# HuiyangYu/TGSFilter

Hardware: AMD Instinct MI355X
Metric: filtered Gbases/sec (end-to-end, excl. gzip I/O) (higher is better)
Workload: dtype u8

## Files before the change

include/tgsf.h:

```cpp
#ifndef TGSF_H
#define TGSF_H

#include <stddef.h>
#include <stdint.h>

#ifdef __cplusplus
extern "C" {
#endif

#define TGSF_ABI_VERSION 3
#define TGSF_MAX_ADAPTERS 32
#define TGSF_MAX_ADAPTER_LEN 8192
#define TGSF_N_DROPINFO 17
#define TGSF_N_QBINS 256
#define TGSF_BIN_WIDTH 100

typedef enum tgsf_status {
    TGSF_OK = 0,
    TGSF_E_INVALID = -1,
    TGSF_E_NO_DEVICE = -2,
    TGSF_E_HIP = -3,
    TGSF_E_CAPACITY = -4,
    TGSF_E_UNSUPPORTED = -5,
    TGSF_E_DATA = -6
} tgsf_status;

typedef struct tgsf_params {
    uint32_t struct_size;
    int32_t  min_len;
    int32_t  max_len;
    float    min_q;
    float    max_q;
    int32_t  bc_len;
    int32_t  head_trim;
    int32_t  tail_trim;
    int32_t  end_len;
    int32_t  end_match_len;
    int32_t  mid_match_len;
    int32_t  extra_len;
    float    end_sim;
    float    mid_sim;
    int32_t  discard;
    int32_t  filter;
    int32_t  only_qc;
    int32_t  min_repeat;
    int32_t  kmer;
    int32_t  qtype;
    int32_t  n_adapters;
    const char* adapters[TGSF_MAX_ADAPTERS];
    int32_t  adapter_len[TGSF_MAX_ADAPTERS];
    uint64_t max_batch_bases;
    uint32_t max_batch_reads;
    uint32_t max_read_len;
    int32_t  no_qual;
    int32_t  reserved;
} tgsf_params;

typedef struct tgsf_batch_in {
    const uint8_t*  seq;
    const uint8_t*  qual;
    const uint64_t* offsets;
    const uint32_t* lengths;
    uint32_t        n_reads;
    uint32_t        reserved;
    uint64_t        n_bytes;
    const uint64_t* qual_offsets;
} tgsf_batch_in;

#define TGSF_RF_LOWQ       0x01u
#define TGSF_RF_AD5P       0x02u
#define TGSF_RF_AD3P       0x04u
#define TGSF_RF_ADMID      0x08u
#define TGSF_RF_DISCARDED  0x10u

typedef struct tgsf_read_result {
    uint64_t sum_q;
    uint32_t flags;
    uint32_t n_frags;
    uint32_t frag_begin;
    uint32_t trimmed;
    int32_t  reserved0;
    int32_t  reserved1;
} tgsf_read_result;

#define TGSF_FF_PASS    0x01u
#define TGSF_FF_REPEAT  0x02u

typedef struct tgsf_fragment {
    uint64_t sum_q;
    uint32_t read;
    int32_t  start;
    int32_t  len;
    uint32_t flags;
} tgsf_fragment;

typedef struct tgsf_batch_out {
    tgsf_read_result* reads;
    tgsf_fragment*    frags;
    uint32_t          frag_capacity;
    uint32_t          n_frags;
} tgsf_batch_out;

#define TGSF_CTR_DROPINFO    0
#define TGSF_CTR_RAW_DIFFQ   17
#define TGSF_CTR_CLEAN_DIFFQ 273
#define TGSF_CTR_ROWS        529
#define TGSF_CTR_END_TABLES  533

enum { TGSF_T_RAW5P_QUAL = 0, TGSF_T_RAW5P_CNT, TGSF_T_RAW3P_QUAL, TGSF_T_RAW3P_CNT,
       TGSF_T_CLEAN5P_QUAL, TGSF_T_CLEAN5P_CNT, TGSF_T_CLEAN3P_QUAL, TGSF_T_CLEAN3P_CNT };
enum { TGSF_B_RAW_QUAL = 0, TGSF_B_RAW_CNT, TGSF_B_CLEAN_QUAL, TGSF_B_CLEAN_CNT };

static inline size_t tgsf_ctr_end_table(int t, int bc_len) {
    return (size_t)TGSF_CTR_END_TABLES + (size_t)t * (size_t)bc_len * 5u;
}
static inline size_t tgsf_ctr_bin_table(int b, int bc_len, uint32_t n_bins) {
    return (size_t)TGSF_CTR_END_TABLES + 8u * (size_t)bc_len * 5u + (size_t)b * (size_t)n_bins * 5u;
}
static inline size_t tgsf_ctr_len(int bc_len, uint32_t n_bins) {
    return tgsf_ctr_bin_table(4, bc_len, n_bins);
}
static inline uint32_t tgsf_n_bins(uint32_t max_read_len) { return max_read_len / TGSF_BIN_WIDTH + 1u; }

typedef struct tgsf_ctx tgsf_ctx;

int tgsf_abi_version(void);

const char* tgsf_backend(void);

int tgsf_prepare_device(int device);

int tgsf_device_location(int device, char* bus_id, int len, int* numa_node);

int tgsf_create(const tgsf_params* params, int device, tgsf_ctx** out_ctx);
void tgsf_destroy(tgsf_ctx* ctx);

int tgsf_submit(tgsf_ctx* ctx, const tgsf_batch_in* in, tgsf_batch_out* out);
int tgsf_submit_async(tgsf_ctx* ctx, const tgsf_batch_in* in, tgsf_batch_out* out);

#define TGSF_MAX_ENQUEUED 64
#define TGSF_NFRAGS_NOT_FINAL 0xFFFFFFFFu
int tgsf_submit_device(tgsf_ctx* ctx, const tgsf_batch_in* in, tgsf_batch_out* out,
                       uint32_t* d_n_frags, void* hip_stream);

int tgsf_wait(tgsf_ctx* ctx);

int tgsf_counters_len(tgsf_ctx* ctx, uint64_t* n_words, int32_t* bc_len, uint32_t* n_bins);
int tgsf_counters(tgsf_ctx* ctx, uint64_t* dst, uint64_t n_words);
int tgsf_counters_used(tgsf_ctx* ctx, uint64_t* dst, uint64_t n_words, uint64_t rows[2]);
int tgsf_counters_merge(tgsf_ctx* dst, tgsf_ctx* src);
int tgsf_counters_device(tgsf_ctx* ctx, void** d_ptr, uint64_t* n_words);
int tgsf_reset_counters(tgsf_ctx* ctx);

#define TGSF_N_STAGES 12
int tgsf_profile(tgsf_ctx* ctx, int enable);
int tgsf_stage_times(tgsf_ctx* ctx, float ms[TGSF_N_STAGES], uint32_t* n_batches);
const char* tgsf_stage_name(int stage);

int tgsf_align_windows(tgsf_ctx* ctx, const uint8_t* seq, uint64_t n_bytes,
                       const uint64_t* win_off, const uint32_t* win_len,
                       const uint8_t* adapter_id, const int32_t* k, uint32_t n,
                       int32_t* res, int32_t* ends);

const char* tgsf_last_error(tgsf_ctx* ctx);

#ifdef __cplusplus
}
#endif
#endif
```

tgsfilter_amd/abi.py:

```python
from __future__ import annotations

import ctypes as C

import numpy as np

ABI_VERSION = 3
MAX_ADAPTERS = 32
MAX_ADAPTER_LEN = 8192
N_DROPINFO = 17
N_QBINS = 256
BIN_WIDTH = 100
N_STAGES = 12

OK, E_INVALID, E_NO_DEVICE, E_HIP, E_CAPACITY, E_UNSUPPORTED, E_DATA = 0, -1, -2, -3, -4, -5, -6

RF_LOWQ, RF_AD5P, RF_AD3P, RF_ADMID, RF_DISCARDED = 0x01, 0x02, 0x04, 0x08, 0x10
FF_PASS, FF_REPEAT = 0x01, 0x02
MAX_ENQUEUED = 64
NFRAGS_NOT_FINAL = 0xFFFFFFFF

CTR_DROPINFO, CTR_RAW_DIFFQ, CTR_CLEAN_DIFFQ, CTR_ROWS, CTR_END_TABLES = 0, 17, 273, 529, 533
(T_RAW5P_QUAL, T_RAW5P_CNT, T_RAW3P_QUAL, T_RAW3P_CNT,
 T_CLEAN5P_QUAL, T_CLEAN5P_CNT, T_CLEAN3P_QUAL, T_CLEAN3P_CNT) = range(8)
B_RAW_QUAL, B_RAW_CNT, B_CLEAN_QUAL, B_CLEAN_CNT = range(4)


class Params(C.Structure):
    _fields_ = [
        ("struct_size", C.c_uint32),
        ("min_len", C.c_int32), ("max_len", C.c_int32),
        ("min_q", C.c_float), ("max_q", C.c_float),
        ("bc_len", C.c_int32), ("head_trim", C.c_int32), ("tail_trim", C.c_int32),
        ("end_len", C.c_int32), ("end_match_len", C.c_int32), ("mid_match_len", C.c_int32),
        ("extra_len", C.c_int32),
        ("end_sim", C.c_float), ("mid_sim", C.c_float),
        ("discard", C.c_int32), ("filter", C.c_int32), ("only_qc", C.c_int32),
        ("min_repeat", C.c_int32), ("kmer", C.c_int32), ("qtype", C.c_int32),
        ("n_adapters", C.c_int32),
        ("adapters", C.c_char_p * MAX_ADAPTERS),
        ("adapter_len", C.c_int32 * MAX_ADAPTERS),
        ("max_batch_bases", C.c_uint64),
        ("max_batch_reads", C.c_uint32),
        ("max_read_len", C.c_uint32),
        ("no_qual", C.c_int32), ("reserved", C.c_int32),
    ]


class BatchIn(C.Structure):
    _fields_ = [
        ("seq", C.c_void_p), ("qual", C.c_void_p), ("offsets", C.c_void_p), ("lengths", C.c_void_p),
        ("n_reads", C.c_uint32), ("reserved", C.c_uint32), ("n_bytes", C.c_uint64),
        ("qual_offsets", C.c_void_p),
    ]


class BatchOut(C.Structure):
    _fields_ = [
        ("reads", C.c_void_p), ("frags", C.c_void_p),
        ("frag_capacity", C.c_uint32), ("n_frags", C.c_uint32),
    ]


READ_RESULT_DTYPE = np.dtype([
    ("sum_q", "<u8"), ("flags", "<u4"), ("n_frags", "<u4"), ("frag_begin", "<u4"),
    ("trimmed", "<u4"), ("reserved0", "<i4"), ("reserved1", "<i4"),
])
FRAGMENT_DTYPE = np.dtype([
    ("sum_q", "<u8"), ("read", "<u4"), ("start", "<i4"), ("len", "<i4"), ("flags", "<u4"),
])
assert READ_RESULT_DTYPE.itemsize == 32 and FRAGMENT_DTYPE.itemsize == 24


def ctr_end_table(t: int, bc_len: int) -> int:
    return CTR_END_TABLES + t * bc_len * 5


def ctr_bin_table(b: int, bc_len: int, n_bins: int) -> int:
    return CTR_END_TABLES + 8 * bc_len * 5 + b * n_bins * 5


def ctr_len(bc_len: int, n_bins: int) -> int:
    return ctr_bin_table(4, bc_len, n_bins)


def n_bins(max_read_len: int) -> int:
    return max_read_len // BIN_WIDTH + 1


_MID_SIM = {"hifi": 0.95, "clr": 0.9, "ont": 0.9}
# ... 35 lines not shown
```

tgsfilter_amd/capi.py:

```python
from __future__ import annotations

import ctypes as C
import os

import numpy as np

from . import abi

_HERE = os.path.dirname(os.path.abspath(__file__))
DEFAULT_LIB = os.path.join(_HERE, "libtgsf.so")
_LIBS = {}

SYMBOLS = [
    "tgsf_abi_version", "tgsf_backend", "tgsf_prepare_device", "tgsf_device_location", "tgsf_create", "tgsf_destroy", "tgsf_submit", "tgsf_submit_async", "tgsf_submit_device",
    "tgsf_wait",
    "tgsf_counters_len", "tgsf_counters", "tgsf_counters_used", "tgsf_counters_merge", "tgsf_counters_device", "tgsf_reset_counters", "tgsf_profile",
    "tgsf_stage_times", "tgsf_stage_name", "tgsf_align_windows", "tgsf_last_error",
]


class TgsfError(RuntimeError):
    def __init__(self, code, msg):
        super().__init__(f"tgsf error {code}: {msg}")
        self.code = code


def load(path: str | None = None):
    explicit = path is not None
    path = path or os.environ.get("TGSF_LIB") or DEFAULT_LIB
    if path in _LIBS:
        if not explicit and not _LIBS[path].tgsf_backend().startswith(b"hip"):
            raise RuntimeError(f"{path} is not the HIP build of libtgsf (there is no CPU fallback; is TGSF_LIB set by accident?)")
        return _LIBS[path]
    if not os.path.exists(path):
        raise FileNotFoundError(
            f"{path} not found: build the HIP extension first (python -c 'import __graft_entry__ as g; g.build()')")
    L = C.CDLL(path)
    vp, u32, u64, i32 = C.c_void_p, C.c_uint32, C.c_uint64, C.c_int32
    L.tgsf_abi_version.restype = C.c_int
    L.tgsf_backend.restype = C.c_char_p
    L.tgsf_prepare_device.argtypes = [C.c_int]
    L.tgsf_device_location.argtypes = [C.c_int, C.c_char_p, C.c_int, C.POINTER(C.c_int)]
    L.tgsf_create.argtypes = [C.POINTER(abi.Params), C.c_int, C.POINTER(vp)]
    L.tgsf_destroy.argtypes = [vp]
    L.tgsf_destroy.restype = None
    L.tgsf_submit.argtypes = [vp, C.POINTER(abi.BatchIn), C.POINTER(abi.BatchOut)]
    L.tgsf_submit_async.argtypes = [vp, C.POINTER(abi.BatchIn), C.POINTER(abi.BatchOut)]
    L.tgsf_submit_device.argtypes = [vp, C.POINTER(abi.BatchIn), C.POINTER(abi.BatchOut), vp, vp]
    L.tgsf_wait.argtypes = [vp]
    L.tgsf_counters_len.argtypes = [vp, C.POINTER(u64), C.POINTER(i32), C.POINTER(u32)]
    L.tgsf_counters.argtypes = [vp, vp, u64]
    L.tgsf_counters_used.argtypes = [vp, vp, u64, vp]
    L.tgsf_counters_merge.argtypes = [vp, vp]
    L.tgsf_counters_device.argtypes = [vp, C.POINTER(vp), C.POINTER(u64)]
    L.tgsf_reset_counters.argtypes = [vp]
    L.tgsf_profile.argtypes = [vp, C.c_int]
    L.tgsf_stage_times.argtypes = [vp, C.POINTER(C.c_float * abi.N_STAGES), C.POINTER(u32)]
    L.tgsf_stage_name.argtypes = [C.c_int]
    L.tgsf_stage_name.restype = C.c_char_p
    L.tgsf_align_windows.argtypes = [vp, vp, u64, vp, vp, vp, vp, u32, vp, vp]
    L.tgsf_last_error.argtypes = [vp]
    L.tgsf_last_error.restype = C.c_char_p
    if L.tgsf_abi_version() != abi.ABI_VERSION:
        raise RuntimeError("libtgsf ABI version mismatch")
    if not explicit and not L.tgsf_backend().startswith(b"hip"):
        raise RuntimeError(f"{path} is the {L.tgsf_backend().decode()!r} build of libtgsf, not the HIP build "
                           "(there is no CPU fallback; is TGSF_LIB set by accident?)")
    _LIBS[path] = L
    return L


class Context:

    def __init__(self, params: abi.Params, device: int = 0, lib_path: str | None = None):
        self.lib = load(lib_path)
        self.params = params
        h = C.c_void_p()
        rc = self.lib.tgsf_create(C.byref(params), device, C.byref(h))
        if rc != 0:
            raise TgsfError(rc, self.lib.tgsf_last_error(None).decode())
        self.h = h
        nw, bc, nb = C.c_uint64(), C.c_int32(), C.c_uint32()
        self._chk(self.lib.tgsf_counters_len(self.h, C.byref(nw), C.byref(bc), C.byref(nb)))
        self.ctr_words, self.bc_len, self.n_bins = nw.value, bc.value, nb.value

    def _chk(self, rc):
        if rc != 0:
            raise TgsfError(rc, self.lib.tgsf_last_error(self.h).decode())

    def close(self):
        if getattr(self, "h", None):
            self.lib.tgsf_destroy(self.h)
            self.h = None

    def __del__(self):
        try:
            self.close()
        except Exception:
            pass

    def submit(self, seq, qual, offsets, lengths=None, frag_capacity=None, qual_offsets=None):
        self.submit_async(seq, qual, offsets, lengths, frag_capacity, qual_offsets)
        return self.wait_result()

    def submit_async(self, seq, qual, offsets, lengths=None, frag_capacity=None, qual_offsets=None):
        seq = np.ascontiguousarray(seq, dtype=np.uint8)
        qual = np.ascontiguousarray(qual, dtype=np.uint8)
        offsets = np.ascontiguousarray(offsets, dtype=np.uint64)
        if lengths is not None:
            lengths = np.ascontiguousarray(lengths, dtype=np.uint32)
            n = len(lengths)
            total = int(lengths.sum())
        else:
            n = len(offsets) - 1
            total = int(offsets[-1] - offsets[0])
        if frag_capacity is None:
            frag_capacity = total // 100 + n + 16
        reads = np.zeros(n, dtype=abi.READ_RESULT_DTYPE)
        frags = np.zeros(frag_capacity, dtype=abi.FRAGMENT_DTYPE)
        if qual_offsets is not None:
            qual_offsets = np.ascontiguousarray(qual_offsets, dtype=np.uint64)
        same = qual is seq or (qual.ctypes.data == seq.ctypes.data)
        bi = abi.BatchIn(seq.ctypes.data, seq.ctypes.data if same else qual.ctypes.data, offsets.ctypes.data,
                         lengths.ctypes.data if lengths is not None else None, n, 0, seq.size,
                         qual_offsets.ctypes.data if qual_offsets is not None else None)
        bo = abi.BatchOut(reads.ctypes.data, frags.ctypes.data, frag_capacity, 0)
        self._pending = (reads, frags, bi, bo, seq, qual, offsets, lengths, qual_offsets)
        rc = self.lib.tgsf_submit_async(self.h, C.byref(bi), C.byref(bo))
        if rc != 0:
            self._pending = None
            self._chk(rc)

    def wait_result(self):
        pend, self._pending = self._pending, None
        if pend is None:
            raise RuntimeError("no batch pending")
        self._chk(self.lib.tgsf_wait(self.h))
        reads, frags, _, bo = pend[:4]
        return reads, frags[:bo.n_frags].copy()

    def submit_device(self, d_seq, d_qual, d_offsets, d_lengths, n_reads, n_bytes, d_reads, d_frags,
                      frag_capacity, d_nfrags=None, stream=None, d_qual_offsets=None):
        bi = abi.BatchIn(d_seq, d_qual, d_offsets, d_lengths, n_reads, 0, n_bytes, d_qual_offsets)
        bo = abi.BatchOut(d_reads, d_frags, frag_capacity, 0)
        self._chk(self.lib.tgsf_submit_device(self.h, C.byref(bi), C.byref(bo), d_nfrags, stream))

    def wait(self):
        self._chk(self.lib.tgsf_wait(self.h))

    def counters(self) -> np.ndarray:
        out = np.zeros(self.ctr_words, dtype=np.uint64)
        self._chk(self.lib.tgsf_counters(self.h, out.ctypes.data, self.ctr_words))
# ... 43 lines not shown
```

tgsfilter_amd/csrc/tgsf_lib.hip:

```cpp
#include <stdarg.h>
#include <stdio.h>
#include <stdlib.h>
#include <string.h>

#include <algorithm>
#include <string>
#include <vector>

#if defined(TGSF_EMUL)
#include "tgsf_kernels.h"
namespace tgsf_emul { thread_local Dim3 threadIdx, blockIdx, blockDim, gridDim; }
typedef void* rt_stream;
typedef int rt_error;
#else
#include <hip/hip_runtime.h>
#include "tgsf_kernels.h"
typedef hipStream_t rt_stream;
#endif

using namespace tgsf;

static thread_local std::string g_create_error;

static const char* knob(const char* name)
{
    static const bool on = [] { const char* e = getenv("TGSF_DEBUG_KNOBS"); return e && e[0] == '1'; }();
    return on ? getenv(name) : nullptr;
}

struct tgsf_ctx {
    tgsf_params params;
    std::vector<std::string> adapters;
    DevParams P;
    DevBatch B;
    int device;
    rt_stream stream;
    rt_stream last_stream;
    bool own_stream;
    std::string error;
    uint64_t cap_bases;
    uint32_t cap_reads, max_read_len, n_bins;
    static constexpr unsigned endtab_grid = 512;
    static constexpr unsigned stats_grid = 768;
    bool flat_scan = true;
    int suffix_filter = 2;
    bool no_hot32 = false;
    uint64_t ctr_words;
    int scratch_cols;
    uint8_t *d_seq, *d_qual;
    uint64_t* d_off;
    uint64_t* d_qoff;
    uint32_t* d_lenin;
    tgsf_read_result* d_out_reads;
    tgsf_fragment* d_out_frags;
    uint32_t* d_out_nfrags;
    std::vector<void*> allocs;
    bool profile;
    float stage_ms[TGSF_N_STAGES];
    uint32_t prof_batches;
#if !defined(TGSF_EMUL)
    static constexpr int kProfRing = 64;
    hipEvent_t ev[kProfRing][TGSF_N_STAGES + 1];
    hipEvent_t ev_aux[kProfRing][3];
    int prof_pending;
    hipStream_t aux;
    hipEvent_t ev_fork, ev_join;
    uint32_t* h_pinned = nullptr;
    static constexpr size_t kStageBytes = 32u << 20;
    uint8_t* stage[2] = {nullptr, nullptr};
    hipEvent_t stage_ev[2] = {nullptr, nullptr};
#endif
    uint32_t h_words_[8];
    uint32_t* h_status;
    uint32_t* pend_nf_p;
    tgsf_batch_out* pend_out = nullptr;
    struct Pending { tgsf_batch_in in; tgsf_read_result* reads; tgsf_fragment* frags; uint32_t fcap; uint32_t* nfrags; rt_stream st; };
    Pending pending[TGSF_MAX_ENQUEUED];
    uint32_t n_pending = 0;
    uint32_t* ovf_ring = nullptr;
    uint32_t* bp_ring = nullptr;
    uint32_t h_ovf[TGSF_MAX_ENQUEUED];
    uint32_t pool_regrown = 0;

};

static int fail(tgsf_ctx* c, int code, const char* fmt, ...)
{
    char buf[512];
    va_list ap;
    va_start(ap, fmt);
    vsnprintf(buf, sizeof buf, fmt, ap);
    va_end(ap);
    if (c) c->error = buf; else g_create_error = buf;
    return code;
}

#if defined(TGSF_EMUL)
#include "tgsf_emul_rt.h"
#else
static int rt_malloc(void** p, size_t n) { return (int)hipMalloc(p, n ? n : 1); }
static void rt_free(void* p) { (void)hipFree(p); }
static int rt_memset(void* p, int v, size_t n, rt_stream s) { return (int)hipMemsetAsync(p, v, n, s); }
static int rt_h2d(void* d, const void* s, size_t n, rt_stream st) { return (int)hipMemcpyAsync(d, s, n, hipMemcpyHostToDevice, st); }
static int rt_d2h(void* d, const void* s, size_t n, rt_stream st) { return (int)hipMemcpyAsync(d, s, n, hipMemcpyDeviceToHost, st); }
static int rt_sync(rt_stream s) { return (int)hipStreamSynchronize(s); }
static const char* rt_errstr(int e) { return hipGetErrorString((hipError_t)e); }
#define TGSF_LAUNCH(kernel, grid, block, stream, ...) hipLaunchKernelGGL(kernel, dim3(grid), dim3(block), 0, (stream), __VA_ARGS__)
#define TGSF_LAUNCH_COOP TGSF_LAUNCH
#define TGSF_LAUNCH_LDS(kernel, grid, block, lds, stream, ...) hipLaunchKernelGGL(kernel, dim3(grid), dim3(block), (lds), (stream), __VA_ARGS__)
static unsigned grid_cap(unsigned g) { return g; }
#endif

template <class T>
static int dev_alloc(tgsf_ctx* c, T** p, size_t count)
{
    void* v = nullptr;
    int e = rt_malloc(&v, count * sizeof(T) + 64);
    if (e) return fail(c, TGSF_E_HIP, "device allocation of %zu bytes failed: %s", count * sizeof(T), rt_errstr(e));
    c->allocs.push_back(v);
    *p = (T*)v;
    return 0;
}

static int build_tables(tgsf_ctx* c)
{
    const tgsf_params& p = c->params;
    DevParams& P = c->P;
    const int A = p.n_adapters;
    std::vector<uint8_t> ad((size_t)kMaxAdapters * kMaxQ, 0);
    const size_t per_ad = (size_t)256 * kPeqW;
    std::vector<uint64_t> fwd((size_t)kMaxAdapters * per_ad, 0), rev((size_t)kMaxAdapters * per_ad, 0),
        top((size_t)kMaxAdapters * 256, 0);
    P.max_nw = 1;
    P.min_Q = 1 << 30;
    for (int a = 0; a < A; a++) {
        const std::string& s = c->adapters[a];
        const int Q = (int)s.size();
        P.Q[a] = Q;
        if (Q > 64 && P.max_nw < 2) P.max_nw = 2;
        if (Q > 128 && P.max_nw < 4) P.max_nw = 4;
        if (Q > 256) P.max_nw = kWideNW;
        if (Q < P.min_Q) P.min_Q = Q;
        int km = Q - p.mid_match_len + 1;
        int ke = Q - p.end_match_len + 1;
        P.k_mid[a] = km > Q - 1 ? Q - 1 : km;
        P.k_end[a] = ke > Q - 1 ? Q - 1 : ke;
        P.w5[a] = p.end_len + (int)((float)Q / p.end_sim);
        P.need_end[a] = P.need_mid[a] = Q + 1;
        for (int m = Q; m >= 0; m--) {
            if (m >= p.end_match_len && (float)m / (float)Q >= p.end_sim) P.need_end[a] = m;
            if (m >= p.mid_match_len && (float)m / (float)Q >= p.mid_sim) P.need_mid[a] = m;
        }
        memcpy(&ad[(size_t)a * kMaxQ], s.data(), (size_t)Q);
        for (int r = 0; r < Q && r < 64 * kPeqW; r++) {
            uint8_t cf = (uint8_t)s[r], cr = (uint8_t)s[Q - 1 - r];
            fwd[(size_t)a * per_ad + (size_t)cf * kPeqW + (r >> 6)] |= 1ull << (r & 63);
            rev[(size_t)a * per_ad + (size_t)cr * kPeqW + (r >> 6)] |= 1ull << (r & 63);
        }
        if (Q <= 64) {
            const int sh = 64 - Q;
            const uint64_t pad = sh ? ((1ull << sh) - 1ull) : 0ull;
            for (int sym = 0; sym < 256; sym++)
                top[(size_t)a * 256 + sym] = (fwd[(size_t)a * per_ad + (size_t)sym * kPeqW] << sh) | pad;
        }
    }
    if (A == 0) P.min_Q = 1 << 30;
    uint8_t* d_ad; uint64_t *d_f, *d_r, *d_t;
    int e;
    if ((e = dev_alloc(c, &d_ad, ad.size()))) return e;
    if ((e = dev_alloc(c, &d_f, fwd.size()))) return e;
    if ((e = dev_alloc(c, &d_r, rev.size()))) return e;
    if ((e = dev_alloc(c, &d_t, top.size()))) return e;
    rt_h2d(d_ad, ad.data(), ad.size(), c->stream);
    rt_h2d(d_f, fwd.data(), fwd.size() * 8, c->stream);
    rt_h2d(d_r, rev.data(), rev.size() * 8, c->stream);
    rt_h2d(d_t, top.data(), top.size() * 8, c->stream);
    rt_sync(c->stream);
    P.adapter = d_ad; P.peq_fwd = d_f; P.peq_rev = d_r; P.peq_top = d_t;
    P.peq_fwd_w = P.peq_rev_w = nullptr;
    if (P.max_nw > 4) {
        const size_t per_w = (size_t)256 * kWideNW;
        std::vector<uint64_t> fw((size_t)A * per_w, 0), rw((size_t)A * per_w, 0);
        for (int a = 0; a < A; a++) {
            const std::string& s = c->adapters[a];
            const int Q = (int)s.size();
            for (int r = 0; r < Q; r++) {
                const uint8_t cf = (uint8_t)s[r], cr = (uint8_t)s[Q - 1 - r];
                fw[(size_t)a * per_w + (size_t)cf * kWideNW + (r >> 6)] |= 1ull << (r & 63);
                rw[(size_t)a * per_w + (size_t)cr * kWideNW + (r >> 6)] |= 1ull << (r & 63);
            }
        }
        uint64_t *d_fw, *d_rw;
        if ((e = dev_alloc(c, &d_fw, fw.size()))) return e;
        if ((e = dev_alloc(c, &d_rw, rw.size()))) return e;
        rt_h2d(d_fw, fw.data(), fw.size() * 8, c->stream);
        rt_h2d(d_rw, rw.data(), rw.size() * 8, c->stream);
        rt_sync(c->stream);
        P.peq_fwd_w = d_fw; P.peq_rev_w = d_rw;
    }
    return 0;
}

extern "C" int tgsf_abi_version(void) { return TGSF_ABI_VERSION; }
extern "C" const char* tgsf_backend(void) { return kTgsfEmul ? "emulation" : "hip:gfx950"; }

#if !defined(TGSF_EMUL)
__global__ void k_noop(int* p) { if (p) *p = 0; }
#endif
#if !defined(TGSF_EMUL)
static void set_wait_mode(int device)
{
    const char* e = getenv("TGSF_SYNC");
    if (!e || strcmp(e, "blocking") != 0) return;
    if (hipSetDevice(device) == hipSuccess) { (void)hipSetDeviceFlags(hipDeviceScheduleBlockingSync); (void)hipGetLastError(); }
}
#endif
extern "C" int tgsf_prepare_device(int device)
{
#if !defined(TGSF_EMUL)
    int ndev = 0;
    if (hipGetDeviceCount(&ndev) != hipSuccess || device < 0 || device >= ndev) return TGSF_E_NO_DEVICE;
    set_wait_mode(device);
    if (hipSetDevice(device) != hipSuccess) return TGSF_E_HIP;
    hipLaunchKernelGGL(k_noop, dim3(1), dim3(64), 0, 0, (int*)nullptr);
    if (hipDeviceSynchronize() != hipSuccess) return TGSF_E_HIP;
    {
        static const char a0[] = "GTTTTCGCATTTATCGTGAAACGCTTTCGCGTTTTTCGTGCGCCGCTTCA";
        static const char a1[] = "TGAAGCGGCGCACGAAAAACGCGAAAGCGTTTCACGATAAATGCGAAAAC";
        tgsf_params p;
        memset(&p, 0, sizeof p);
        p.struct_size = sizeof p;
        p.min_len = 100; p.max_len = 2147483647; p.min_q = 0; p.max_q = 255; p.bc_len = 150;
        p.end_len = 150; p.end_match_len = 4; p.mid_match_len = 35; p.extra_len = 50;
        p.end_sim = 0.75f; p.mid_sim = 0.9f; p.filter = 1; p.qtype = 33; p.kmer = 11;
        p.n_adapters = 2; p.adapters[0] = a0; p.adapters[1] = a1; p.adapter_len[0] = p.adapter_len[1] = 50;
        p.max_batch_bases = 1 << 16; p.max_batch_reads = 16; p.max_read_len = 1 << 14;
        tgsf_ctx* c = nullptr;
        if (tgsf_create(&p, device, &c) == TGSF_OK) {
            std::vector<uint8_t> seq(8192), qual(8192, (uint8_t)'5');
            for (size_t i = 0; i < seq.size(); i++) seq[i] = "ACGT"[(i * 2654435761u >> 13) & 3];
            memcpy(&seq[4096 + 1000], a0, 50);
            const uint64_t off[2] = {0, 4096};
            const uint32_t len[2] = {3000, 4000};
            tgsf_read_result res[2];
            tgsf_fragment fr[64];
            tgsf_batch_in in;
            memset(&in, 0, sizeof in);
            in.seq = seq.data(); in.qual = qual.data(); in.offsets = off; in.lengths = len; in.n_reads = 2; in.n_bytes = seq.size();
            tgsf_batch_out out{res, fr, 64, 0};
            (void)tgsf_submit(c, &in, &out);
            tgsf_destroy(c);
        }
    }
#else
    (void)device;
#endif
    return TGSF_OK;
}

extern "C" int tgsf_device_location(int device, char* bus_id, int len, int* numa_node)
{
    if (numa_node) *numa_node = -1;
    if (bus_id && len > 0) bus_id[0] = 0;
#if !defined(TGSF_EMUL)
    int ndev = 0;
    if (hipGetDeviceCount(&ndev) != hipSuccess || device < 0 || device >= ndev) return TGSF_E_NO_DEVICE;
    char id[64] = {0};
    if (hipDeviceGetPCIBusId(id, (int)sizeof id, device) != hipSuccess) return TGSF_E_HIP;
    for (char* p = id; *p; p++) if (*p >= 'A' && *p <= 'F') *p = (char)(*p - 'A' + 'a');
    if (bus_id && len > 0) { strncpy(bus_id, id, (size_t)len - 1); bus_id[len - 1] = 0; }
    if (numa_node) {
        const std::string path = std::string("/sys/bus/pci/devices/") + id + "/numa_node";
        if (FILE* f = fopen(path.c_str(), "r")) {
            int v = -1;
            if (fscanf(f, "%d", &v) == 1) *numa_node = v;
            fclose(f);
        }
    }
    return TGSF_OK;
#else
    if (bus_id && len > 0) snprintf(bus_id, (size_t)len, "emul:%d", device);
    if (numa_node)
        if (const char* e = knob("TGSF_EMUL_NUMA")) {
            int k = 0;
            for (const char* c = e; *c; k++) {
                if (k == device) { *numa_node = atoi(c); break; }
                while (*c && *c != ',') c++;
                if (*c == ',') c++;
            }
        }
    return TGSF_OK;
#endif
}

extern "C" const char* tgsf_last_error(tgsf_ctx* ctx) { return ctx ? ctx->error.c_str() : g_create_error.c_str(); }

extern "C" void tgsf_destroy(tgsf_ctx* c)
{
    if (!c) return;
    if (c->B.bp_allowed && c->B.bp_state && knob("TGSF_TRACE_BP")) {
        uint32_t w[4] = {0, 0, 0, 0};
        uint64_t pl[4] = {0, 0, 0, 0};
        uint32_t sg[4] = {0, 0, 0, 0};
        if (!rt_d2h(w, c->B.bp_state, sizeof w, c->stream) && !rt_d2h(pl, c->B.plan, sizeof pl, c->stream) && !rt_d2h(sg, c->B.seg_info, sizeof sg, c->stream) && !rt_sync(c->stream))
            fprintf(stderr, "tgsf: clean tables as a by-product of the raw pass: %u batches speculated; the next would%s; the last batch: %llu bases a direct clean pass scans, "
                            "%llu bases its own did, %u work items in that pass\n", w[1], w[0] ? "" : " not", (unsigned long long)pl[2], (unsigned long long)pl[3], sg[2]);
    }
#if !defined(TGSF_EMUL)
    (void)hipSetDevice(c->device);
    (void)hipStreamSynchronize(c->stream);
    for (int k = 0; k < tgsf_ctx::kProfRing; k++) {
        for (int i = 0; i <= TGSF_N_STAGES; i++) if (c->ev[k][i]) (void)hipEventDestroy(c->ev[k][i]);
        for (int i = 0; i < 3; i++) if (c->ev_aux[k][i]) (void)hipEventDestroy(c->ev_aux[k][i]);
    }
    if (c->h_pinned) (void)hipHostFree(c->h_pinned);
    for (int i = 0; i < 2; i++) {
        if (c->stage[i]) (void)hipHostFree(c->stage[i]);
        if (c->stage_ev[i]) (void)hipEventDestroy(c->stage_ev[i]);
    }
    if (c->ev_fork) (void)hipEventDestroy(c->ev_fork);
    if (c->ev_join) (void)hipEventDestroy(c->ev_join);
    if (c->aux) (void)hipStreamDestroy(c->aux);
    if (c->own_stream && c->stream) (void)hipStreamDestroy(c->stream);
#endif
    for (void* p : c->allocs) rt_free(p);
    delete c;
}

extern "C" int tgsf_create(const tgsf_params* p, int device, tgsf_ctx** out)
{
    if (!p || !out) return fail(nullptr, TGSF_E_INVALID, "null argument");
    *out = nullptr;
    if (p->struct_size != sizeof(tgsf_params))
        return fail(nullptr, TGSF_E_INVALID, "tgsf_params.struct_size %u != %zu (ABI mismatch)", p->struct_size, sizeof(tgsf_params));
    if (p->n_adapters < 0 || p->n_adapters > TGSF_MAX_ADAPTERS)
        return fail(nullptr, TGSF_E_INVALID, "n_adapters %d outside [0,%d]", p->n_adapters, TGSF_MAX_ADAPTERS);
    if (p->min_repeat > 0 && (p->kmer < 1 || p->kmer > 32))
        return fail(nullptr, TGSF_E_UNSUPPORTED, "-k %d: the repeat gate supports k-mer sizes 1..32 (the reference's k-mers are 64 bits)", p->kmer);
    if (p->qtype != 33 && p->qtype != 64) return fail(nullptr, TGSF_E_INVALID, "qtype must be 33 or 64");
    if (p->bc_len < 0 || p->bc_len > kMaxBcLenTotal) return fail(nullptr, TGSF_E_INVALID, "bc_len (-e) outside [0,%d]", kMaxBcLenTotal);
    if (p->filter && p->n_adapters > 0) {
        if (!(p->end_sim > 0.f) || !(p->mid_sim > 0.f)) return fail(nullptr, TGSF_E_INVALID, "similarities must be > 0");
        if (p->end_len < 0 || p->extra_len < 0) return fail(nullptr, TGSF_E_INVALID, "end_len / extra_len must be >= 0");
        if (p->end_match_len < 1 || p->mid_match_len < 1)
            return fail(nullptr, TGSF_E_INVALID, "match lengths must be >= 1");
    }
    for (int a = 0; a < p->n_adapters; a++) {
        if (!p->adapters[a] || p->adapter_len[a] < 1 || p->adapter_len[a] > TGSF_MAX_ADAPTER_LEN)
            return fail(nullptr, TGSF_E_UNSUPPORTED, "adapter %d: length %d outside [1,%d]", a, p->adapter_len[a], TGSF_MAX_ADAPTER_LEN);
    }
    if (!p->max_batch_bases || !p->max_batch_reads || !p->max_read_len)
        return fail(nullptr, TGSF_E_INVALID, "max_batch_bases / max_batch_reads / max_read_len must be set");
    if (p->max_read_len > (1u << 28)) return fail(nullptr, TGSF_E_INVALID, "max_read_len above 2^28");

    tgsf_ctx* c = new tgsf_ctx();
    c->params = *p;
    c->device = device;
    c->profile = false;
    c->prof_batches = 0;
    memset(c->stage_ms, 0, sizeof c->stage_ms);
    memset(c->h_words_, 0, sizeof c->h_words_);
    c->h_status = c->h_words_;
    c->pend_nf_p = c->h_words_ + 4;
    for (int a = 0; a < p->n_adapters; a++) {
        c->adapters.emplace_back(p->adapters[a], (size_t)p->adapter_len[a]);
        c->params.adapters[a] = c->adapters.back().data();
    }
    for (int a = 0; a < p->n_adapters; a++) c->params.adapters[a] = c->adapters[a].data();
#if !defined(TGSF_EMUL)
    memset(c->ev, 0, sizeof c->ev);
    memset(c->ev_aux, 0, sizeof c->ev_aux);
    c->aux = nullptr; c->ev_fork = c->ev_join = nullptr;
    int ndev = 0;
    hipError_t he = hipGetDeviceCount(&ndev);
    if (he != hipSuccess || ndev <= 0) {
        delete c;
        return fail(nullptr, TGSF_E_NO_DEVICE, "no HIP device available (%s); libtgsf has no CPU fallback", hipGetErrorString(he));
    }
    if (device < 0 || device >= ndev) { delete c; return fail(nullptr, TGSF_E_NO_DEVICE, "device %d out of range (%d devices)", device, ndev); }
    set_wait_mode(device);
    if ((he = hipSetDevice(device)) != hipSuccess) { delete c; return fail(nullptr, TGSF_E_HIP, "hipSetDevice: %s", hipGetErrorString(he)); }
    if ((he = hipStreamCreateWithFlags(&c->stream, hipStreamNonBlocking)) != hipSuccess) {
        delete c; return fail(nullptr, TGSF_E_HIP, "hipStreamCreate: %s", hipGetErrorString(he));
    }
    c->own_stream = true;
    c->prof_pending = 0;
    {
        uint32_t* pw = nullptr;
        if (hipHostMalloc((void**)&pw, 64, hipHostMallocDefault) == hipSuccess && pw) {
            memset(pw, 0, 64);
            c->h_pinned = pw; c->h_status = pw; c->pend_nf_p = pw + 4;
        }
    }
    {
        int lo = 0, hi = 0;
        (void)hipDeviceGetStreamPriorityRange(&lo, &hi);
        he = hipStreamCreateWithPriority(&c->aux, hipStreamNonBlocking, hi);
    }
    if (he != hipSuccess ||
        (he = hipEventCreateWithFlags(&c->ev_fork, hipEventDisableTiming)) != hipSuccess ||
        (he = hipEventCreateWithFlags(&c->ev_join, hipEventDisableTiming)) != hipSuccess) {
        tgsf_destroy(c); return fail(nullptr, TGSF_E_HIP, "auxiliary stream: %s", hipGetErrorString(he));
    }
#else
    c->stream = nullptr; c->own_stream = false;
#endif
    c->last_stream = c->stream;
#if !defined(TGSF_EMUL)
    if (p->max_batch_bases > (8u << 20)) {
        for (int i = 0; i < 2; i++)
            if (hipHostMalloc((void**)&c->stage[i], tgsf_ctx::kStageBytes, hipHostMallocDefault) != hipSuccess ||
                hipEventCreateWithFlags(&c->stage_ev[i], hipEventDisableTiming) != hipSuccess) {
                tgsf_destroy(c); return fail(nullptr, TGSF_E_HIP, "pinned staging buffers: allocation failed");
            }
    }
#endif
    DevParams& P = c->P;
    memset(&P, 0, sizeof P);
    P.min_len = p->min_len; P.max_len = p->max_len; P.min_q = p->min_q; P.max_q = p->max_q;
    P.bc_len = p->bc_len; P.head_trim = p->head_trim; P.tail_trim = p->tail_trim; P.end_len = p->end_len;
    P.end_match_len = p->end_match_len; P.mid_match_len = p->mid_match_len; P.extra_len = p->extra_len;
    P.end_sim = p->end_sim; P.mid_sim = p->mid_sim; P.discard = p->discard; P.filter = p->filter;
    P.only_qc = p->only_qc; P.qtype = p->qtype; P.n_adapters = p->n_adapters;
    P.no_qual = p->no_qual ? 1 : 0;
    P.min_repeat = p->min_repeat; P.kmer = p->kmer;
    c->cap_bases = p->max_batch_bases;
    c->cap_reads = p->max_batch_reads;
    c->max_read_len = p->max_read_len;
    c->n_bins = tgsf_n_bins(p->max_read_len);
    P.n_bins = c->n_bins;
    c->ctr_words = tgsf_ctr_len(p->bc_len, c->n_bins);
    P.seg_cols = kSegCols;
    if (const char* e = knob("TGSF_NO_HOT32")) c->no_hot32 = atoi(e) > 0;
    if (const char* e = knob("TGSF_SEG_COLS")) { int v = atoi(e); if (v >= 256 && v <= 65536) P.seg_cols = v & ~15; }
    if (const char* e = knob("TGSF_MID_FLAT")) c->flat_scan = atoi(e) > 0;
    if (const char* e = knob("TGSF_MID_FILTER")) { int v = atoi(e); if (v >= 0 && v <= 2) c->suffix_filter = v; }

    int e = build_tables(c);
    DevBatch& B = c->B;
    memset(&B, 0, sizeof B);
    B.flat_pmax = 256; B.flat_pmin = 16; B.flat_f0 = 224;
    if (const char* e = knob("TGSF_FLAT_PMIN")) { int v = atoi(e); if (v >= 1 && v <= (1 << 20)) B.flat_pmin = (uint32_t)v; }
    if (const char* e = knob("TGSF_FLAT_PMAX")) { int v = atoi(e); if (v >= 1 && v <= (1 << 20)) B.flat_pmax = (uint32_t)v; }
    if (const char* e = knob("TGSF_FLAT_F0")) { int v = atoi(e); if (v >= 0 && v <= 256) B.flat_f0 = (uint32_t)v; }
    B.flat_pmin = 1u << flat_log2(B.flat_pmin); B.flat_pmax = 1u << flat_log2(B.flat_pmax);
    if (B.flat_pmax < B.flat_pmin) B.flat_pmax = B.flat_pmin;
    const size_t n = c->cap_reads;
    const int A = p->n_adapters > 0 ? p->n_adapters : 1;
    const uint64_t cap_bytes = c->cap_bases + 16ull * n + 64;
    const int min_len = p->min_len > 0 ? p->min_len : 1;
    uint64_t fcap64 = p->filter ? (c->cap_bases / (uint64_t)min_len + 16) : (uint64_t)n + 16;
    if (fcap64 > c->cap_bases + 16) fcap64 = c->cap_bases + 16;
    if (fcap64 < n + 16 && !p->filter) fcap64 = n + 16;
    B.fcap = (uint32_t)std::min<uint64_t>(fcap64, 0x7FFFFFF0ull);
    B.max_tiles = (c->max_read_len + kTileBases - 1) / kTileBases;
    uint64_t pool = c->cap_bases / 64 + 65536 + (uint64_t)n * 16u * (uint64_t)std::max(p->n_adapters, 1);
    B.pool_cap = (uint32_t)std::min<uint64_t>(pool, 1ull << 28);
    if (const char* e = knob("TGSF_POOL_CAP")) { const long long v = atoll(e); if (v >= 1 && v < (1ll << 28)) B.pool_cap = (uint32_t)v; }
    const size_t nitems = n + (size_t)B.fcap;
    if (!e) e = dev_alloc(c, &c->d_seq, cap_bytes);
    if (!e) e = dev_alloc(c, &c->d_qual, cap_bytes);
    if (!e) e = dev_alloc(c, &c->d_off, n + 1);
    if (!e) e = dev_alloc(c, &c->d_qoff, n + 1);
    if (!e) e = dev_alloc(c, &c->d_lenin, n);
    if (!e) e = dev_alloc(c, &B.len, n);
    if (!e) e = dev_alloc(c, &B.sumq, n);
    if (!e) e = dev_alloc(c, &B.flags, n);
    if (!e) e = dev_alloc(c, &B.clip5, n * A);
    if (!e) e = dev_alloc(c, &B.clip3, n * A);
    if (!e) e = dev_alloc(c, &B.mid_head, n);
    if (!e) e = dev_alloc(c, &B.mid_best, n * A);
    if (!e) e = dev_alloc(c, &B.mid_cnt, n);
    if (!e) e = dev_alloc(c, &B.mid_gate, n * A);
    if (!e) e = dev_alloc(c, &B.pool, (size_t)B.pool_cap);
    if (!e) e = dev_alloc(c, &B.pool_n, 4);
    if (!e) e = dev_alloc(c, &B.seg_cnt, n + 1);
    if (!e) e = dev_alloc(c, &B.chk_cnt, n + 1);
    if (c->cap_bases / 16u + n >= 0xFFFFFFF0ull) c->flat_scan = false;
    if (c->cap_bases / 16u + n >= (1ull << 30) || !c->flat_scan) c->suffix_filter = 0;
    {
        bool any = false;
        for (int a = 0; a < p->n_adapters; a++) any |= c->P.Q[a] > 32 && c->P.Q[a] <= 64 && c->P.k_mid[a] >= 0 && c->P.k_mid[a] <= kSuffixMaxK;
        if (!any || !p->filter) c->suffix_filter = 0;
    }
    if (!e && c->suffix_filter) e = dev_alloc(c, &B.chk_mark, (size_t)4 * (size_t)((c->cap_bases / 16u + n) / 32u + 8u));
    if (c->suffix_filter) {
        B.rc_cap = (uint32_t)std::min<uint64_t>((c->cap_bases / 16u + n) / 25u + 4096u, 1ull << 24);
        if (const char* e2 = knob("TGSF_RECHECK_CAP")) { int v = atoi(e2); if (v >= 0) B.rc_cap = (uint32_t)v; }
        if (!e) e = dev_alloc(c, &B.rc_list, (size_t)B.rc_cap + 1);
        if (!e) e = dev_alloc(c, &B.rc_n, 4);
    }
    if (!e) e = dev_alloc(c, &B.nfr, n + 1);
    if (!e) e = dev_alloc(c, &B.scan_part, n / kScanTile + 2);
    if (!e) e = dev_alloc(c, &B.trimmed, n);
    B.rep_long_cap = (uint32_t)std::min<uint64_t>(c->cap_bases / kRepShare + 16, (uint64_t)B.fcap + 16);
    if (!e) e = dev_alloc(c, &B.rep_next, 2 + (size_t)B.rep_long_cap);
    if (p->min_repeat > 0 && p->kmer >= 12 && p->kmer <= 31) {
        B.rep_tab_log2 = 4;
        while (B.rep_tab_log2 < 40 && (1ull << B.rep_tab_log2) < 2ull * c->max_read_len) B.rep_tab_log2++;
        if (!e) e = dev_alloc(c, &B.rep_tab, (size_t)1 << B.rep_tab_log2);
        if (!e) e = dev_alloc(c, &B.rep_lock, 4);
        if (!e) rt_memset(B.rep_lock, 0, 16, c->stream);
        B.rep_max_plog = kRepMaxPlog;
        if (const char* ev = knob("TGSF_REP_MAX_PLOG")) { int v = atoi(ev); if (v >= 0 && v <= 20) B.rep_max_plog = (uint32_t)v; }
    }
    if (!e) e = dev_alloc(c, &B.tile_hist, 2 * ((size_t)B.max_tiles + 2));
    if (!e) e = dev_alloc(c, &B.tile_cnt, 2 * ((size_t)B.max_tiles + 2));
    if (!e) e = dev_alloc(c, &B.tile_base, 2 * ((size_t)B.max_tiles + 2));
    if (!e) e = dev_alloc(c, &B.tile_fill, 2 * ((size_t)B.max_tiles + 2));
    if (!e) e = dev_alloc(c, &B.seg_info, 4);
    if (!e) e = dev_alloc(c, &B.perm, nitems);
    B.work_cap = (uint32_t)std::min<uint64_t>(2 * (c->cap_bases / kTileBases) + nitems + 16, 0x7FFFFFF0ull);
    if (!e) e = dev_alloc(c, &B.work, 2 * (size_t)B.work_cap);
    if (!e) e = dev_alloc(c, &B.frag_off, (size_t)B.fcap);
    if (!e) e = dev_alloc(c, &B.frag_qoff, (size_t)B.fcap);
    if (!e) e = dev_alloc(c, &B.frag_len, (size_t)B.fcap);
    if (!e) e = dev_alloc(c, &B.frag_sum, (size_t)B.fcap);
    if (!e) e = dev_alloc(c, &B.frag_read, (size_t)B.fcap);
    if (!e) e = dev_alloc(c, &B.frag_start, (size_t)B.fcap);
    if (!e) e = dev_alloc(c, &B.frag_flags, (size_t)B.fcap);
    if (!e) e = dev_alloc(c, &B.raw_tab, 2 * (size_t)c->n_bins * 5);
    if (!e) e = dev_alloc(c, &B.whole, n);
    if (!e) e = dev_alloc(c, &B.plan, 4);
    B.clean_force = p->only_qc ? 1u : 0u;
    B.bp_allowed = (p->filter && !p->only_qc && (p->head_trim > 0 || p->tail_trim > 0) &&
                    p->head_trim >= 0 && p->tail_trim >= 0) ? 1u : 0u;
    static_assert(kTileBases < (1 << 13), "staged bytes of a tile fit the work list's 13 bits");
    if (const char* f = knob("TGSF_CLEAN_TABLES")) {
        if (!strcmp(f, "direct")) { B.clean_force = 1; B.bp_allowed = 0; }
        else if (!strcmp(f, "difference") && !p->only_qc) { B.clean_force = 2; B.bp_allowed = 0; }
        else if (!strcmp(f, "byproduct") && B.bp_allowed) B.clean_force = 3;
    }
    if (B.bp_allowed) {
        if (!e) e = dev_alloc(c, &B.spec, n);
        if (!e) e = dev_alloc(c, &B.spec_sum, n);
        if (!e) e = dev_alloc(c, &B.bp_state, 4);
        if (!e) e = dev_alloc(c, &c->bp_ring, TGSF_MAX_ENQUEUED);
    }
    {
        int maxcols = 1;
        for (int a = 0; a < p->n_adapters; a++) {
            int kmax = std::max(std::max(P.k_end[a], P.k_mid[a]), 0);
            maxcols = std::max(maxcols, P.Q[a] + std::min(P.Q[a], kmax) + 1);
        }
        c->scratch_cols = maxcols;
        int col_words = P.max_nw;
        if (P.max_nw > 4) { col_words = 1; for (int a = 0; a < p->n_adapters; a++) col_words = std::max(col_words, (P.Q[a] + 63) / 64); }
        size_t lane_words = (size_t)(maxcols + 1) * 2 * (size_t)col_words;
        if (P.max_nw > 4) lane_words = std::min<size_t>(lane_words, (1u << 17) + 2 * (size_t)col_words) + 4 * (size_t)col_words + 64;
        B.scratch_wave_words = lane_words * 64;
        B.scratch_mid_wave0 = ((size_t)n * A * 2 + 63) / 64 + 1;
        const size_t waves = B.scratch_mid_wave0 + ((size_t)n * A + 63) / 64 + 1;
        if (!e) e = dev_alloc(c, &B.scratch, waves * B.scratch_wave_words);
    }
    if (!e) e = dev_alloc(c, &B.ctr, (size_t)c->ctr_words);
    if (!e) e = dev_alloc(c, &B.status, 4);
    if (!e) e = dev_alloc(c, &c->ovf_ring, TGSF_MAX_ENQUEUED);
    if (!e) e = dev_alloc(c, &c->d_out_reads, n);
    if (!e) e = dev_alloc(c, &c->d_out_frags, (size_t)B.fcap);
    if (!e) e = dev_alloc(c, &c->d_out_nfrags, 4);
    if (e) {
        g_create_error = c->error;
        tgsf_destroy(c);
        return e;
    }
    rt_memset(B.ctr, 0, c->ctr_words * 8, c->stream);
    rt_memset(B.status, 0, 16, c->stream);
    rt_memset(c->ovf_ring, 0, TGSF_MAX_ENQUEUED * 4, c->stream);
    B.ovf = c->ovf_ring;
    if (B.bp_allowed) {
        const uint32_t init[4] = {1u, 0u, 0u, 0u};
        rt_memset(c->bp_ring, 0, TGSF_MAX_ENQUEUED * 4, c->stream);
        (void)rt_h2d(B.bp_state, init, sizeof init, c->stream);
        B.bp_used = c->bp_ring;
    }
    rt_memset(B.raw_tab, 0, 2 * (size_t)c->n_bins * 5 * 8, c->stream);
    rt_sync(c->stream);
    *out = c;
    return TGSF_OK;
}

static const char* kStageNames[TGSF_N_STAGES] = {
    "prepare+sort", "stats_raw", "gate_reads", "end_tables_raw", "end_windows", "mid_scan",
    "mid_resolve", "regions", "repeat_gate", "stats_clean", "gate_frags+end_tables_clean", "finalize"};

extern "C" const char* tgsf_stage_name(int s) { return (s >= 0 && s < TGSF_N_STAGES) ? kStageNames[s] : ""; }

static unsigned blocks_for(uint64_t n, unsigned block) { return (unsigned)std::max<uint64_t>(1, (n + block - 1) / block); }

#if !defined(TGSF_EMUL)
static int harvest_profile(tgsf_ctx* c, rt_stream st)
{
    if (!c->prof_pending) return TGSF_OK;
    hipError_t he = hipStreamSynchronize(st);
    if (he != hipSuccess) return fail(c, TGSF_E_HIP, "stream synchronize failed: %s", hipGetErrorString(he));
    (void)hipStreamSynchronize(c->aux);
    for (int k = 0; k < c->prof_pending; k++)
        for (int i = 0; i < TGSF_N_STAGES; i++) {
            float ms = 0.f;
            hipError_t e = (i == 3 || i == 4) ? hipEventElapsedTime(&ms, c->ev_aux[k][i - 3], c->ev_aux[k][i - 2])
                                              : hipEventElapsedTime(&ms, c->ev[k][i], c->ev[k][i + 1]);
            if (e == hipSuccess) c->stage_ms[i] += ms;
        }
    c->prof_pending = 0;
    return TGSF_OK;
}
#endif

static void scan_u32(const DevBatch& B, uint32_t* a, uint32_t n, rt_stream st, uint32_t* part = nullptr)
{
    if (!part) part = B.scan_part;
    const unsigned nb = (n + kScanTile - 1) / kScanTile;
    TGSF_LAUNCH_COOP(k_scan_tiles, nb, 256, st, a, n, part);
    TGSF_LAUNCH_COOP(k_scan_top, 1, 64, st, part, (uint32_t)nb, a + n);
    TGSF_LAUNCH_COOP(k_scan_add, nb, 256, st, a, n, (const uint32_t*)part);
}

static int drain_pending(tgsf_ctx* c, bool implicit = false);

static int run_pipeline(tgsf_ctx* c, const tgsf_batch_in* in, tgsf_read_result* d_reads, tgsf_fragment* d_frags,
                        uint32_t out_fcap, uint32_t* d_nfrags, rt_stream st, bool redo = false, uint32_t slot = 0)
{
    if (!redo) {
        if (c->n_pending == TGSF_MAX_ENQUEUED) { int e = drain_pending(c, true); if (e) return e; }
        slot = c->n_pending++;
        tgsf_ctx::Pending& pd = c->pending[slot];
        pd.in = *in; pd.reads = d_reads; pd.frags = d_frags; pd.fcap = out_fcap; pd.nfrags = d_nfrags; pd.st = st;
    }
    const bool profile = c->profile && !redo;
    (void)profile;
    DevBatch B = c->B;
    B.ovf = c->ovf_ring + slot;
    B.bp_used = c->bp_ring + slot;
    B.replay = redo ? 1u : 0u;
    const DevParams& P = c->P;
    B.seq = in->seq; B.qual = in->qual; B.off = in->offsets; B.len_in = in->lengths;
    B.qoff = in->qual_offsets ? in->qual_offsets : in->offsets;
    B.n = in->n_reads; B.n_bytes = in->n_bytes;
    const uint32_t n = B.n;
    const int A = P.n_adapters;
    const unsigned T = 256;
    static_assert(kMidThreads == 256, "k_mid_flat / k_mid_scan1 are launched with T lanes a workgroup");
    c->last_stream = st;
    const unsigned gsmall = grid_cap(std::min(blocks_for(n, T), 2048u));
    const unsigned gstats = grid_cap(c->stats_grid);
    const size_t tl = 2 * ((size_t)B.max_tiles + 2) * 4;
    const unsigned gfold = grid_cap(std::min(blocks_for((uint64_t)P.n_bins * 5, T), 1024u));
    int stage = 0;
#if !defined(TGSF_EMUL)
    if (profile && c->prof_pending == tgsf_ctx::kProfRing) { int e = harvest_profile(c, st); if (e) return e; }
    hipEvent_t* evs = c->ev[profile ? c->prof_pending : 0];
    hipEvent_t* evx = c->ev_aux[profile ? c->prof_pending : 0];
    if (profile) {
        for (int i = 0; i <= TGSF_N_STAGES; i++) if (!evs[i]) (void)hipEventCreate(&evs[i]);
        for (int i = 0; i < 3; i++) if (!evx[i]) (void)hipEventCreate(&evx[i]);
    }
    hipStream_t ax = c->aux;
#define STAGE_MARK() do { if (profile) (void)hipEventRecord(evs[stage], st); stage++; } while (0)
#else
#define STAGE_MARK() do { stage++; } while (0)
#endif
// ... 60 lines not shown
                gflat = grid_cap(blocks_for((uint64_t)S.d0[S.nph] + 128ull * (B.flat_pmax / B.flat_pmin) + 512u, T));
            }
        }
        const uint64_t max_segs = in->n_bytes / (uint64_t)P.seg_cols + 2ull * n + 1;
        const unsigned gseg = blocks_for(max_segs, T);
        const unsigned gmid = gseg;
        rt_stream ms = st;
        (void)ms;
        auto launch_scans = [&](uint32_t mode) {
            DevBatch Bm = B;
            Bm.mid_mode = mode;
            int a = 0;
            while (a < A) {
                if (P.Q[a] > 256) { TGSF_LAUNCH(k_mid_scan_wide, gseg, T, ms, P, Bm, a); a++; continue; }
                if (P.Q[a] > 192) { TGSF_LAUNCH(k_mid_scanw<4>, gseg, T, ms, P, Bm, a); a++; continue; }
                if (P.Q[a] > 128) { TGSF_LAUNCH(k_mid_scanw<3>, gseg, T, ms, P, Bm, a); a++; continue; }
                if (P.Q[a] > 64) { TGSF_LAUNCH(k_mid_scanw<2>, gseg, T, ms, P, Bm, a); a++; continue; }
                auto cls = [&](int x) {
                    if (P.Q[x] <= 32 && !c->no_hot32) return 0;
                    if (flat && mode == 0 && c->suffix_filter && P.Q[x] > 32 && P.k_mid[x] >= 0 && P.k_mid[x] <= kSuffixMaxK) return 2;
                    return 1;
                };
                const int kind = cls(a);
                const bool narrow = kind == 0;
                const int width = narrow ? 2 : 4;
                int na = 0;
                while (a + na < A && na < width && P.Q[a + na] <= 64 && cls(a + na) == kind) na++;
                if (kind == 2) {
                    const unsigned lp = 0;
                    Bm.mark_stride = (uint32_t)((flat_chunks / 32u + 7u) & ~3ull);
                    rt_memset(Bm.chk_mark, 0, (size_t)na * Bm.mark_stride * 4u, ms);
                    rt_memset(Bm.rc_n, 0, 4, ms);
                    if (c->suffix_filter == 1) switch (na) {
                    case 1: TGSF_LAUNCH_LDS((k_mid_flat<1, Hot32, 1>), gflat, T, lp, ms, P, Bm, a, na); break;
                    case 2: TGSF_LAUNCH_LDS((k_mid_flat<2, Hot32, 1>), gflat, T, lp, ms, P, Bm, a, na); break;
                    case 3: TGSF_LAUNCH_LDS((k_mid_flat<3, Hot32, 1>), gflat, T, lp, ms, P, Bm, a, na); break;
                    default: TGSF_LAUNCH_LDS((k_mid_flat<4, Hot32, 1>), gflat, T, lp, ms, P, Bm, a, na); break;
                    }
                    else switch (na) {
                    case 1: TGSF_LAUNCH_LDS((k_mid_flat<1, Hot32, 2>), gflat, T, lp, ms, P, Bm, a, na); break;
                    case 2: TGSF_LAUNCH_LDS((k_mid_flat<2, Hot32, 2>), gflat, T, lp, ms, P, Bm, a, na); break;
                    case 3: TGSF_LAUNCH_LDS((k_mid_flat<3, Hot32, 2>), gflat, T, lp, ms, P, Bm, a, na); break;
                    default: TGSF_LAUNCH_LDS((k_mid_flat<4, Hot32, 2>), gflat, T, lp, ms, P, Bm, a, na); break;
                    }
                    const unsigned grc = grid_cap(blocks_for(flat_chunks / 32u + 1u, (unsigned)kRecheckWords));
                    TGSF_LAUNCH_COOP(k_mid_marks, grc, T, ms, P, Bm, a, na);
                    TGSF_LAUNCH(k_mid_recheck, grid_cap(2048u), T, ms, P, Bm, a, na);
                    a += na;
                    continue;
                }
                if (flat && mode == 0) {
                    const unsigned lp = 0;
                    if (narrow) switch (na) {
                    case 1: TGSF_LAUNCH_LDS((k_mid_flat<1, Hot32>), gflat, T, lp, ms, P, Bm, a, na); break;
                    default: TGSF_LAUNCH_LDS((k_mid_flat<2, Hot32>), gflat, T, lp, ms, P, Bm, a, na); break;
                    }
                    else switch (na) {
                    case 1: TGSF_LAUNCH_LDS((k_mid_flat<1, Hot>), gflat, T, lp, ms, P, Bm, a, na); break;
                    case 2: TGSF_LAUNCH_LDS((k_mid_flat<2, Hot>), gflat, T, lp, ms, P, Bm, a, na); break;
                    case 3: TGSF_LAUNCH_LDS((k_mid_flat<3, Hot>), gflat, T, lp, ms, P, Bm, a, na); break;
                    default: TGSF_LAUNCH_LDS((k_mid_flat<4, Hot>), gflat, T, lp, ms, P, Bm, a, na); break;
                    }
                    a += na;
                    continue;
                }
                if (narrow) switch (na) {
                case 1: TGSF_LAUNCH((k_mid_scan1<1, Hot32>), gmid, T, ms, P, Bm, a, na); break;
                default: TGSF_LAUNCH((k_mid_scan1<2, Hot32>), gmid, T, ms, P, Bm, a, na); break;
                }
                else switch (na) {
                case 1: TGSF_LAUNCH((k_mid_scan1<1, Hot>), gmid, T, ms, P, Bm, a, na); break;
                case 2: TGSF_LAUNCH((k_mid_scan1<2, Hot>), gmid, T, ms, P, Bm, a, na); break;
                case 3: TGSF_LAUNCH((k_mid_scan1<3, Hot>), gmid, T, ms, P, Bm, a, na); break;
                default: TGSF_LAUNCH((k_mid_scan1<4, Hot>), gmid, T, ms, P, Bm, a, na); break;
                }
                a += na;
            }
        };
        launch_scans(0);
        if (redo) {
            const uint64_t cells = max_segs * (uint64_t)A + 1;
            if (cells > 0xFFFFFFF0ull) return fail(c, TGSF_E_CAPACITY, "middle scan: too many (segment, adapter) cells for the position-ordered pass");
            uint32_t *seg_n = nullptr, *part = nullptr;
            if (rt_malloc((void**)&seg_n, (size_t)(cells + 1) * 4 + 64) || rt_malloc((void**)&part, (size_t)(cells / kScanTile + 4) * 4 + 64)) {
                if (seg_n) rt_free(seg_n);
                return fail(c, TGSF_E_CAPACITY, "middle scan: no device memory for the position-ordered pass (%.1f GB)", (double)cells * 4e-9);
            }
            B.seg_n = seg_n;
            int rc = TGSF_OK;
            do {
                rt_memset(seg_n, 0, (size_t)(cells + 1) * 4, ms);
                TGSF_LAUNCH(k_mid_reset, gsmall, T, ms, B, A);
                launch_scans(1);
                scan_u32(B, seg_n, (uint32_t)cells, ms, part);
                uint32_t need = 0;
                int he = rt_d2h(&need, seg_n + cells, 4, ms);
                if (!he) he = rt_sync(ms);
                if (he) { rc = fail(c, TGSF_E_HIP, "middle scan (counting pass) failed: %s", rt_errstr(he)); break; }
                if (need > B.pool_cap) {
                    const uint64_t want = (uint64_t)need + 1024;
                    if (want > 0x7FFFFFF0ull) { rc = fail(c, TGSF_E_CAPACITY, "middle-adapter candidates: %u columns tie their reads' minima, more than one batch can list", need); break; }
                    void* np = nullptr;
                    if (rt_malloc(&np, (size_t)want * sizeof(MidCand) + 64)) {
                        rc = fail(c, TGSF_E_CAPACITY, "middle-adapter candidates: no device memory for %llu slots (%.1f GB)", (unsigned long long)want, (double)want * sizeof(MidCand) * 1e-9);
                        break;
                    }
                    for (void*& q : c->allocs) if (q == (void*)c->B.pool) q = np;
                    rt_free(c->B.pool);
                    c->B.pool = (MidCand*)np; c->B.pool_cap = (uint32_t)want;
                    B.pool = c->B.pool; B.pool_cap = c->B.pool_cap;
                    c->pool_regrown++;
                }
                if (knob("TGSF_TRACE_POOL"))
                    fprintf(stderr, "tgsf: candidate pool overflow (or a read with a long candidate list): %u columns at their reads' minima, pool of %u slots%s; scanning again in position order\n", need, B.pool_cap,
                            c->pool_regrown ? " (grown)" : "");
                rt_memset(B.ovf, 0, 4, ms);
                launch_scans(2);
                TGSF_LAUNCH(k_mid_link, gsmall, T, ms, B, A);
                DevBatch Bm = B;
                Bm.mid_mode = 2;
                if (P.max_nw > 4) TGSF_LAUNCH(k_mid_resolve<kWideNW>, blocks_for((uint64_t)n * A, 64), 64, ms, P, Bm);
                else if (P.max_nw > 2) TGSF_LAUNCH(k_mid_resolve<4>, blocks_for((uint64_t)n * A, 64), 64, ms, P, Bm);
                else TGSF_LAUNCH(k_mid_resolve<2>, blocks_for((uint64_t)n * A, 64), 64, ms, P, Bm);
                const unsigned geach = grid_cap(std::min(blocks_for(need, 64), 65536u));
                if (need) {
                    if (P.max_nw > 4) TGSF_LAUNCH(k_mid_resolve_each<kWideNW>, geach, 64, ms, P, Bm);
                    else if (P.max_nw > 2) TGSF_LAUNCH(k_mid_resolve_each<4>, geach, 64, ms, P, Bm);
                    else TGSF_LAUNCH(k_mid_resolve_each<2>, geach, 64, ms, P, Bm);
                }
                he = rt_sync(ms);
                if (he) rc = fail(c, TGSF_E_HIP, "middle scan (position-ordered pass) failed: %s", rt_errstr(he));
            } while (0);
            rt_free(seg_n);
            rt_free(part);
            B.seg_n = nullptr;
            if (rc) return rc;
        }
    }
    STAGE_MARK();
    if (P.filter && A > 0 && !redo) {
        if (P.max_nw > 4) TGSF_LAUNCH(k_mid_resolve<kWideNW>, blocks_for((uint64_t)n * A, 64), 64, st, P, B);
        else if (P.max_nw > 2) TGSF_LAUNCH(k_mid_resolve<4>, blocks_for((uint64_t)n * A, 64), 64, st, P, B);
        else TGSF_LAUNCH(k_mid_resolve<2>, blocks_for((uint64_t)n * A, 64), 64, st, P, B);
    }
    STAGE_MARK();
#if !defined(TGSF_EMUL)
    (void)hipStreamWaitEvent(st, c->ev_join, 0);
#endif
    TGSF_LAUNCH(k_regions<false>, gsmall, T, st, P, B);
    scan_u32(B, B.nfr, n, st);
    TGSF_LAUNCH(k_regions<true>, gsmall, T, st, P, B);
    STAGE_MARK();
    if (P.min_repeat > 0 && !P.only_qc) {
        rt_memset(B.rep_next, 0, 2 * sizeof(uint32_t), st);
        const int keys_from = 12;
        if (P.kmer < keys_from && P.kmer <= 13) TGSF_LAUNCH(k_repeat, grid_cap(256u), kRepThreads, st, P, B);
        else {
            TGSF_LAUNCH(k_repeat_long, gsmall, T, st, P, B);
            if (P.kmer <= 15) TGSF_LAUNCH(k_repeat_keys<false>, grid_cap(256u), kRepThreads, st, P, B);
            else TGSF_LAUNCH(k_repeat_keys<true>, grid_cap(256u), kRepThreads, st, P, B);
        }
    }
    STAGE_MARK();
    rt_memset(B.tile_hist, 0, tl, st);
    rt_memset(B.tile_fill, 0, tl, st);
    const unsigned gfr = grid_cap(std::min(blocks_for((uint64_t)B.fcap + n, T), 2048u));
    TGSF_LAUNCH(k_clean_plan, gsmall, T, st, P, B);
    if (B.bp_allowed && !redo) TGSF_LAUNCH(k_clean_plan_next, 1, 64, st, B);
    TGSF_LAUNCH(k_fold_raw<true>, gfold, T, st, P, B);
    TGSF_LAUNCH(k_frag_prepare, gfr, T, st, P, B);
    TGSF_LAUNCH_COOP(k_tile_scan, 1, 64, st, B, 2u);
    TGSF_LAUNCH(k_tile_scatter<true>, gfr, T, st, P, B);
    TGSF_LAUNCH(k_build_work<true>, gwork, T, st, P, B);
    TGSF_LAUNCH((k_stats<true, true>), gstats, 64 * kStatsWaves, st, P, B);
    STAGE_MARK();
    TGSF_LAUNCH(k_gate_frags, gfr, T, st, P, B);
    for (uint32_t slab = 0; slab * (uint32_t)kMaxBcLen < (uint32_t)P.bc_len; slab++)
        TGSF_LAUNCH(k_end_tables<true>, grid_cap(c->endtab_grid), 64 * kEndWaves, st, P, B, slab);
    STAGE_MARK();
    TGSF_LAUNCH(k_finalize, gsmall, T, st, B, d_reads, d_frags, out_fcap, d_nfrags);
    STAGE_MARK();
#if !defined(TGSF_EMUL)
    hipError_t he = hipGetLastError();
    if (he != hipSuccess) return fail(c, TGSF_E_HIP, "kernel launch failed: %s", hipGetErrorString(he));
    if (profile) { c->prof_batches++; c->prof_pending++; }
#endif
    return TGSF_OK;
}

static int text_h2d(tgsf_ctx* c, uint8_t* dst, const uint8_t* src, uint64_t n, rt_stream st)
{
#if !defined(TGSF_EMUL)
    hipPointerAttribute_t at;
    const bool known = hipPointerGetAttributes(&at, src) == hipSuccess && at.type != hipMemoryTypeUnregistered;
    (void)hipGetLastError();
    if (!known && c->stage[0] && n > (1u << 20)) {
        int he = 0, k = 0;
        for (uint64_t o = 0; o < n; o += tgsf_ctx::kStageBytes, k ^= 1) {
            const size_t m = (size_t)std::min<uint64_t>(tgsf_ctx::kStageBytes, n - o);
            (void)hipEventSynchronize(c->stage_ev[k]);
            memcpy(c->stage[k], src + o, m);
            he |= (int)hipMemcpyAsync(dst + o, c->stage[k], m, hipMemcpyHostToDevice, st);
            he |= (int)hipEventRecord(c->stage_ev[k], st);
        }
        return he;
    }
#endif
    (void)c;
    return rt_h2d(dst, src, n, st);
}

static int check_batch(tgsf_ctx* c, const tgsf_batch_in* in)
{
    if (!in || !in->seq || (!in->qual && !c->P.no_qual) || !in->offsets) return fail(c, TGSF_E_INVALID, "null batch pointer");
    if (in->n_reads == 0) return fail(c, TGSF_E_INVALID, "empty batch");
    if (in->n_reads > c->cap_reads) return fail(c, TGSF_E_CAPACITY, "batch has %u reads, context was sized for %u", in->n_reads, c->cap_reads);
    if (in->qual_offsets && !in->lengths) return fail(c, TGSF_E_INVALID, "qual_offsets requires explicit lengths");
// ... 190 lines not shown
        const uint64_t r = used[b >> 1];
        if (r) he = rt_d2h(dst + at, c->B.ctr + at, (size_t)r * 5 * 8, c->stream);
    }
    if (!he) he = rt_sync(c->stream);
    if (rows) { rows[0] = used[0]; rows[1] = used[1]; }
    return he ? fail(c, TGSF_E_HIP, "device to host copy failed") : TGSF_OK;
}

extern "C" int tgsf_counters_merge(tgsf_ctx* dst, tgsf_ctx* src)
{
    if (!dst || !src || dst == src) return TGSF_E_INVALID;
    if (dst->ctr_words != src->ctr_words || dst->P.bc_len != src->P.bc_len || dst->device != src->device)
        return fail(dst, TGSF_E_INVALID, "tgsf_counters_merge: the contexts differ in tally layout or device");
    int e = tgsf_wait(src);
    if (e) return fail(dst, e, "%s", src->error.c_str());
    if ((e = tgsf_wait(dst))) return e;
    TGSF_LAUNCH(k_ctr_merge, grid_cap(blocks_for(dst->ctr_words, 256)), 256, dst->stream, dst->B.ctr, (const uint64_t*)src->B.ctr, dst->ctr_words);
    const int he = rt_sync(dst->stream);
    return he ? fail(dst, TGSF_E_HIP, "tgsf_counters_merge failed") : TGSF_OK;
}

extern "C" int tgsf_counters_device(tgsf_ctx* c, void** d_ptr, uint64_t* n_words)
{
    if (!c || !d_ptr) return TGSF_E_INVALID;
    *d_ptr = c->B.ctr;
    if (n_words) *n_words = c->ctr_words;
    return TGSF_OK;
}

extern "C" int tgsf_reset_counters(tgsf_ctx* c)
{
    if (!c) return TGSF_E_INVALID;
    int he = rt_memset(c->B.ctr, 0, c->ctr_words * 8, c->stream);
    if (!he) he = rt_memset(c->B.raw_tab, 0, 2 * (size_t)c->n_bins * 5 * 8, c->stream);
    if (!he) he = rt_sync(c->stream);
    return he ? fail(c, TGSF_E_HIP, "memset failed") : TGSF_OK;
}

extern "C" int tgsf_profile(tgsf_ctx* c, int enable)
{
    if (!c) return TGSF_E_INVALID;
#if !defined(TGSF_EMUL)
    { int e = harvest_profile(c, c->last_stream); if (e) return e; }
#endif
    c->profile = enable != 0;
    memset(c->stage_ms, 0, sizeof c->stage_ms);
    c->prof_batches = 0;
    return TGSF_OK;
}

extern "C" int tgsf_stage_times(tgsf_ctx* c, float ms[TGSF_N_STAGES], uint32_t* n_batches)
{
    if (!c || !ms) return TGSF_E_INVALID;
#if !defined(TGSF_EMUL)
    { int e = harvest_profile(c, c->last_stream); if (e) return e; }
#endif
    memcpy(ms, c->stage_ms, sizeof c->stage_ms);
    if (n_batches) *n_batches = c->prof_batches;
    return TGSF_OK;
}

extern "C" int tgsf_align_windows(tgsf_ctx* c, const uint8_t* seq, uint64_t n_bytes, const uint64_t* win_off,
                                  const uint32_t* win_len, const uint8_t* adapter_id, const int32_t* k, uint32_t n,
                                  int32_t* res, int32_t* ends)
{
    if (!c || !seq || !win_off || !win_len || !adapter_id || !k || !res || !ends) return TGSF_E_INVALID;
    if (!n) return TGSF_OK;
    for (uint32_t i = 0; i < n; i++) {
        if (adapter_id[i] >= c->P.n_adapters) return fail(c, TGSF_E_INVALID, "problem %u: adapter id out of range", i);
        if (win_len[i] == 0 || win_off[i] + win_len[i] > n_bytes) return fail(c, TGSF_E_INVALID, "problem %u: window outside the buffer", i);
        if (k[i] < 0) return fail(c, TGSF_E_INVALID, "problem %u: k < 0", i);
        const int Q = c->P.Q[adapter_id[i]];
        if (Q + std::min(Q, (int)k[i]) + 1 > c->scratch_cols)
            return fail(c, TGSF_E_CAPACITY, "problem %u: k larger than the context's thresholds allow for", i);
    }
    if ((size_t)n > (size_t)c->cap_reads * std::max(c->P.n_adapters, 1) * 2)
        return fail(c, TGSF_E_CAPACITY, "more alignment problems than the context was sized for");
#if !defined(TGSF_EMUL)
    (void)hipSetDevice(c->device);
#endif
    uint8_t *d_seq = nullptr, *d_aid = nullptr; uint64_t* d_off = nullptr; uint32_t* d_len = nullptr;
    int32_t *d_k = nullptr, *d_res = nullptr, *d_ends = nullptr;
    int e = 0;
    e |= rt_malloc((void**)&d_seq, n_bytes + 16);
    e |= rt_malloc((void**)&d_aid, n);
    e |= rt_malloc((void**)&d_off, (size_t)n * 8);
    e |= rt_malloc((void**)&d_len, (size_t)n * 4);
    e |= rt_malloc((void**)&d_k, (size_t)n * 4);
    e |= rt_malloc((void**)&d_res, (size_t)n * 16);
    e |= rt_malloc((void**)&d_ends, (size_t)n * 8);
    rt_stream st = c->stream;
    if (!e) {
        e |= rt_h2d(d_seq, seq, n_bytes, st);
        e |= rt_h2d(d_aid, adapter_id, n, st);
        e |= rt_h2d(d_off, win_off, (size_t)n * 8, st);
        e |= rt_h2d(d_len, win_len, (size_t)n * 4, st);
        e |= rt_h2d(d_k, k, (size_t)n * 4, st);
    }
    if (!e) {
        if (c->P.max_nw > 4)
            TGSF_LAUNCH(k_align_windows<kWideNW>, blocks_for(n, 64), 64, st, c->P, c->B, (const uint8_t*)d_seq, (const uint64_t*)d_off,
                        (const uint32_t*)d_len, (const uint8_t*)d_aid, (const int32_t*)d_k, n, d_res, d_ends);
        else if (c->P.max_nw > 2)
            TGSF_LAUNCH(k_align_windows<4>, blocks_for(n, 64), 64, st, c->P, c->B, (const uint8_t*)d_seq, (const uint64_t*)d_off,
                        (const uint32_t*)d_len, (const uint8_t*)d_aid, (const int32_t*)d_k, n, d_res, d_ends);
        else
            TGSF_LAUNCH(k_align_windows<2>, blocks_for(n, 64), 64, st, c->P, c->B, (const uint8_t*)d_seq, (const uint64_t*)d_off,
                        (const uint32_t*)d_len, (const uint8_t*)d_aid, (const int32_t*)d_k, n, d_res, d_ends);
        e |= rt_d2h(res, d_res, (size_t)n * 16, st);
        e |= rt_d2h(ends, d_ends, (size_t)n * 8, st);
        e |= rt_sync(st);
    }
    rt_free(d_seq); rt_free(d_aid); rt_free(d_off); rt_free(d_len); rt_free(d_k); rt_free(d_res); rt_free(d_ends);
    return e ? fail(c, TGSF_E_HIP, "tgsf_align_windows: device operation failed") : TGSF_OK;
}
```

tgsfilter_amd/host/api.cpp:

```cpp
#include "api.h"
#include "cputime.h"
#include "fatal.h"

#include <dlfcn.h>
#include <unistd.h>

#include <chrono>
#include <cstdio>
#include <cstdlib>
#include <iostream>
#include <string>
#include <thread>

#ifndef TGSF_LIB_REL
#define TGSF_LIB_REL "../libtgsf.so"
#endif
#ifndef TGSF_EXPECT_BACKEND
#define TGSF_EXPECT_BACKEND "hip"
#endif

namespace host {

namespace {
Api g_api;
std::thread g_thread;
std::string g_error;
double g_load_s = 0, g_device_s = 0;
bool g_started = false;

double now_s() { return std::chrono::duration<double>(std::chrono::steady_clock::now().time_since_epoch()).count(); }

std::string lib_path()
{
    if (const char* e = getenv("TGSF_LIB")) return e;
    char exe[4096];
    const ssize_t n = readlink("/proc/self/exe", exe, sizeof exe - 1);
    std::string dir = n > 0 ? std::string(exe, (size_t)n) : std::string(".");
    const size_t slash = dir.rfind('/');
    dir = slash == std::string::npos ? "." : dir.substr(0, slash);
    return dir + "/" + TGSF_LIB_REL;
}

void load(std::vector<int> devices)
{
    CpuScope cpu(CPU_LOADER);
    const double t0 = now_s();
    const std::string path = lib_path();
    void* h = dlopen(path.c_str(), RTLD_NOW | RTLD_LOCAL);
    if (!h) { g_error = std::string("cannot load ") + path + ": " + dlerror() + " (there is no CPU fallback)"; return; }
#define BIND(field, sym) \
    g_api.field = reinterpret_cast<decltype(g_api.field)>(dlsym(h, sym)); \
    if (!g_api.field) { g_error = std::string("symbol ") + sym + " missing in " + path; return; }
    BIND(abi_version, "tgsf_abi_version")
    BIND(backend, "tgsf_backend")
    BIND(prepare_device, "tgsf_prepare_device")
    BIND(create, "tgsf_create")
    BIND(destroy, "tgsf_destroy")
    BIND(submit, "tgsf_submit")
    BIND(wait, "tgsf_wait")
    BIND(counters_len, "tgsf_counters_len")
    BIND(counters, "tgsf_counters")
    BIND(counters_used, "tgsf_counters_used")
    BIND(align_windows, "tgsf_align_windows")
    BIND(last_error, "tgsf_last_error")
    BIND(profile, "tgsf_profile")
    BIND(stage_times, "tgsf_stage_times")
    BIND(stage_name, "tgsf_stage_name")
    BIND(device_location, "tgsf_device_location")
    BIND(counters_merge, "tgsf_counters_merge")
#undef BIND
    if (g_api.abi_version() != TGSF_ABI_VERSION) { g_error = path + ": ABI version mismatch"; return; }
    {
        const char* b = g_api.backend();
        const std::string want = TGSF_EXPECT_BACKEND;
        if (!b || std::string(b).compare(0, want.size(), want) != 0) {
            g_error = path + " is the \"" + (b ? b : "?") + "\" build of the library; this program runs on the \"" + want +
                      "\" build only (there is no CPU fallback; is TGSF_LIB set by accident?)";
            return;
        }
    }
    g_load_s = now_s() - t0;
    std::vector<std::thread> up;
    for (size_t i = 1; i < devices.size(); i++) {
        bool seen = false;
        for (size_t j = 0; j < i; j++) seen = seen || devices[j] == devices[i];
        if (!seen) up.emplace_back([d = devices[i]] { CpuScope c2(CPU_LOADER); (void)g_api.prepare_device(d); });
    }
    if (!devices.empty()) (void)g_api.prepare_device(devices[0]);
    for (std::thread& t : up) t.join();
    g_device_s = now_s() - t0 - g_load_s;
}
}

void lib_start(const std::vector<int>& devices)
{
    g_started = true;
    g_thread = std::thread(load, devices);
}

const Api& lib()
{
    if (!g_started) lib_start({});
    if (g_thread.joinable()) g_thread.join();
    if (!g_error.empty()) {
        std::cerr << "Error: " << g_error << std::endl;
        quit(255);
    }
    return g_api;
}

namespace {
RcclApi g_rccl;
bool g_rccl_ok = false, g_rccl_started = false;
std::thread g_rccl_thread;

void load_rccl()
{
    std::string path = lib_path();
    const size_t slash = path.rfind('/');
    path = (slash == std::string::npos ? std::string(".") : path.substr(0, slash)) + "/libtgsf_rccl.so";
    void* h = dlopen(path.c_str(), RTLD_NOW | RTLD_LOCAL);
    if (!h) return;
#define BIND(field, sym) g_rccl.field = reinterpret_cast<decltype(g_rccl.field)>(dlsym(h, sym)); if (!g_rccl.field) return;
    BIND(unique_id, "tgsf_rccl_unique_id")
    BIND(comm_init, "tgsf_rccl_comm_init")
    BIND(comm_count, "tgsf_rccl_comm_count")
    BIND(comm_destroy, "tgsf_rccl_comm_destroy")
    BIND(allreduce_counters, "tgsf_rccl_allreduce_counters")
    BIND(last_error, "tgsf_rccl_last_error")
#undef BIND
    g_rccl_ok = true;
}
}

void rccl_start()
{
    if (g_rccl_started) return;
    g_rccl_started = true;
    g_rccl_thread = std::thread(load_rccl);
}

const RcclApi* rccl_lib()
{
    rccl_start();
    if (g_rccl_thread.joinable()) g_rccl_thread.join();
    return g_rccl_ok ? &g_rccl : nullptr;
}

void lib_times(double& load_s, double& device_s) { load_s = g_load_s; device_s = g_device_s; }

}
```

tgsfilter_amd/host/api.h:

```cpp
#pragma once
#include <vector>

#include "tgsf.h"
#include "tgsf_rccl.h"

namespace host {

struct Api {
    decltype(&tgsf_abi_version) abi_version;
    decltype(&tgsf_backend) backend;
    decltype(&tgsf_prepare_device) prepare_device;
    decltype(&tgsf_create) create;
    decltype(&tgsf_destroy) destroy;
    decltype(&tgsf_submit) submit;
    decltype(&tgsf_wait) wait;
    decltype(&tgsf_counters_len) counters_len;
    decltype(&tgsf_counters) counters;
    decltype(&tgsf_counters_used) counters_used;
    decltype(&tgsf_align_windows) align_windows;
    decltype(&tgsf_last_error) last_error;
    decltype(&tgsf_profile) profile;
    decltype(&tgsf_stage_times) stage_times;
    decltype(&tgsf_stage_name) stage_name;
    decltype(&tgsf_device_location) device_location;
    decltype(&tgsf_counters_merge) counters_merge;
};

struct RcclApi {
    decltype(&tgsf_rccl_unique_id) unique_id;
    decltype(&tgsf_rccl_comm_init) comm_init;
    decltype(&tgsf_rccl_comm_count) comm_count;
    decltype(&tgsf_rccl_comm_destroy) comm_destroy;
    decltype(&tgsf_rccl_allreduce_counters) allreduce_counters;
    decltype(&tgsf_rccl_last_error) last_error;
};
void rccl_start();
const RcclApi* rccl_lib();

void lib_start(const std::vector<int>& devices);
const Api& lib();
void lib_times(double& load_s, double& device_s);

}
```

tgsfilter_amd/host/prepass.cpp:

```cpp
#include "prepass.h"
#include <chrono>
#include <cstdio>

#include <unistd.h>

#include <algorithm>
#include <cstdlib>
#include <cstring>
#include <iostream>
#include <thread>
#include <unordered_map>
#include <vector>

#include "api.h"
#include "fatal.h"

namespace host {

const char* const kAdapterLib[22] = {
    "ATCTCTCTCTTTTCCTCCTCCTCCGTTGTTGTTGTTGAGAGAGAT",
    "ATCTCTCTCAACAACAACAACGGAGGAGGAGGAAAAGAGAGAGAT",
    "AAAAAAAAAAAAAAAAAATTAACGGAGGAGGAGGA",
    "TCCTCCTCCTCCGTTAATTTTTTTTTTTTTTTTTT",
    "AATGTACTTCGTTCAGTTACGTATTGCT",
    "AGCAATACGTAACTGAACGAAGTACATT",
    "GCAATACGTAACTGAACGAAGT",
    "ACTTCGTTCAGTTACGTATTGC",
    "GTTTTCGCATTTATCGTGAAACGCTTTCGCGTTTTTCGTGCGCCGCTTCA",
    "TGAAGCGGCGCACGAAAAACGCGAAAGCGTTTCACGATAAATGCGAAAAC",
    "GGCGTCTGCTTGGGTGTTTAACCTTTTTGTCAGAGAGGTTCCAAGTCAGAGAGGTTCCT",
    "AGGAACCTCTCTGACTTGGAACCTCTCTGACAAAAAGGTTAAACACCCAAGCAGACGCC",
    "GGAACCTCTCTGACTTGGAACCTCTCTGACAAAAAGGTTAAACACCCAAGCAGACGCCAGCAAT",
    "ATTGCTGGCGTCTGCTTGGGTGTTTAACCTTTTTGTCAGAGAGGTTCCAAGTCAGAGAGGTTCC",
    "TTTTTTTTCCTGTACTTCGTTCAGTTACGTATTGCT",
    "AGCAATACGTAACTGAACGAAGTACAGGAAAAAAAA",
    "GCAATACGTAACTGAACGAAGTACAGG",
    "CCTGTACTTCGTTCAGTTACGTATTGC",
    "ACGTAACTGAACGAAGTACAGG",
    "CCTGTACTTCGTTCAGTTACGT",
    "CTTGCGGGCGGCGGACTCTCCTCTGAAGATAGAGCGACAGGCAAG",
    "CTTGCCTGTCGCTCTATCTTCAGAGGAGAGTCCGCCGCCCGCAAG",
};

std::string rev_comp(const std::string& s)
{
    static char comp[256];
    static bool init = false;
    if (!init) {
        memset(comp, 'N', sizeof comp);
        const char* a = "AGCTagctMRWSYKmrwsyk";
        const char* b = "TCGAtcgaKYWSRMkywsrm";
        for (int i = 0; a[i]; i++) comp[(unsigned char)a[i]] = b[i];
        init = true;
    }
    std::string r;
    r.reserve(s.size());
    for (size_t i = s.size(); i-- > 0;) r += comp[(unsigned char)s[i]];
    return r;
}

static int check_base_content(const std::vector<std::string>& ends, int check_len, int seq_num, float end_bias)
{
    static const struct Col { uint8_t of[256]; Col() { memset(of, 4, sizeof of); of['A'] = of['a'] = 0; of['T'] = of['t'] = 1; of['G'] = of['g'] = 2; of['C'] = of['c'] = 3; } } col;
    std::vector<int> cnt5((size_t)check_len * 5, 0);
    for (const std::string& s : ends) {
        const size_t n = std::min(s.size(), (size_t)check_len);
        for (size_t i = 0; i < n; i++) cnt5[i * 5 + col.of[(unsigned char)s[i]]]++;
    }
    std::vector<int> cnt((size_t)check_len * 4, 0);
    for (int i = 0; i < check_len; i++) for (int j = 0; j < 4; j++) cnt[(size_t)i * 4 + j] = cnt5[(size_t)i * 5 + j];
    const int max_diff = (int)((seq_num * end_bias) / 100);
    int trim = 0;
    for (int i = 1; i < check_len - 1; i++) {
        const int ld = std::min(i, 5), rd = std::min(check_len - i - 1, 5);
        bool left = false, right = false;
        for (int j = 0; j < 4; j++) {
            for (int x = 1; x <= ld; x++)
                if (abs(cnt[(size_t)i * 4 + j] - cnt[(size_t)(i - x) * 4 + j]) > max_diff) { left = true; break; }
            for (int x = 1; x <= rd; x++)
                if (abs(cnt[(size_t)(i + x) * 4 + j] - cnt[(size_t)i * 4 + j]) > max_diff) { right = true; break; }
        }
        if (left && right) trim = i + 1;
    }
    return trim;
}

static double pp_now() { return std::chrono::duration<double>(std::chrono::steady_clock::now().time_since_epoch()).count(); }
static double g_pp_create = 0, g_pp_align = 0; static int g_pp_calls = 0;

static void adapter_search(const Options& o, const std::vector<std::string>& ends, std::string& adapter, float& depth)
{
    adapter.clear(); depth = 0.f;
    float min_sim = o.mid_sim;
    if (min_sim < 0.9) min_sim = 0.9f;
    if (ends.empty()) return;

    tgsf_params p;
    memset(&p, 0, sizeof p);
    p.struct_size = sizeof p;
    p.min_len = 100; p.max_len = 2147483647; p.min_q = 0; p.max_q = 255; p.bc_len = 0;
    p.end_len = 0; p.extra_len = 0; p.end_sim = 0.75f; p.mid_sim = 0.9f; p.filter = 1; p.qtype = 33;
    p.n_adapters = 22;
    int k[22];
    size_t max_q = 0;
    for (int a = 0; a < 22; a++) {
        p.adapters[a] = kAdapterLib[a];
        p.adapter_len[a] = (int)strlen(kAdapterLib[a]);
        k[a] = (int)((1 - min_sim) * p.adapter_len[a]) + 1;
        max_q = std::max(max_q, (size_t)p.adapter_len[a]);
    }
    p.end_match_len = 2; p.mid_match_len = (int)max_q;
    const size_t per_call = 4096;
    p.max_batch_reads = (uint32_t)(per_call * 22 / (22 * 2) + 64);
    p.max_batch_bases = 1 << 20; p.max_read_len = 1 << 16;
    tgsf_ctx* ctx = nullptr;
    const double c0 = pp_now();
    if (lib().create(&p, o.devices.empty() ? o.device : o.devices[0], &ctx) != TGSF_OK) { std::cerr << "Error: " << lib().last_error(nullptr) << std::endl; quit(255); }

    g_pp_create += pp_now() - c0;
    std::unordered_map<int, int> maps;
    std::vector<uint8_t> buf; std::vector<uint64_t> off; std::vector<uint32_t> len; std::vector<uint8_t> aid;
    std::vector<int32_t> kk, res, eds;
    for (size_t b = 0; b < ends.size(); b += per_call) {
        const size_t e = std::min(ends.size(), b + per_call);
        buf.clear(); off.clear(); len.clear(); aid.clear(); kk.clear();
        for (size_t i = b; i < e; i++) {
            const uint64_t o0 = buf.size();
            buf.insert(buf.end(), ends[i].begin(), ends[i].end());
            if (ends[i].empty()) continue;
            for (int a = 0; a < 22; a++) { off.push_back(o0); len.push_back((uint32_t)ends[i].size()); aid.push_back((uint8_t)a); kk.push_back(k[a]); }
        }
        const uint32_t n = (uint32_t)off.size();
        if (!n) continue;
        res.assign((size_t)n * 4, 0); eds.assign((size_t)n * 2, 0);
        const double a0 = pp_now();
        if (lib().align_windows(ctx, buf.data(), buf.size(), off.data(), len.data(), aid.data(), kk.data(), n, res.data(), eds.data()) != TGSF_OK) {
            std::cerr << "Error: " << lib().last_error(ctx) << std::endl; quit(255);
        }
        g_pp_align += pp_now() - a0; g_pp_calls++;
        for (uint32_t i = 0; i < n; i++)
            if (res[(size_t)i * 4 + 1] > 0)
                maps[(int)aid[i]] += res[(size_t)i * 4 + 2] - res[(size_t)i * 4 + 0];
    }
    lib().destroy(ctx);
    std::vector<std::pair<int, int>> vec(maps.begin(), maps.end());
    std::sort(vec.begin(), vec.end(), [](const std::pair<int, int>& a, const std::pair<int, int>& b) { return a.second > b.second; });
    if (vec.empty()) return;
    const int best = vec.front().first;
    const std::string cand = kAdapterLib[best];
    const float mean_dep = (float)maps[best] / (float)cand.size();
    if (mean_dep >= 2 * min_sim) { adapter = cand; depth = mean_dep; }
}

PrepassResult run_prepass(Options& o, const std::function<bool(Rec&)>& next_record)
{
    PrepassResult R;
    const double t0 = pp_now();
    int check_len = std::max(std::max(o.end_len, o.bc_len), 100);
    int min_len = std::max(o.min_len, 2 * check_len);
    const int max_seq = std::max(o.ad_num, o.bc_num);
    std::vector<std::string> ends5, ends3;
    const bool need5 = o.filter && (o.head_trim < 0 || o.adapter_file.empty());
    const bool need3 = o.filter && (o.tail_trim < 0 || o.adapter_file.empty());
    int seq_num = 0, min_qc = 255, max_qc = 0;
    {
        Rec r;
        const bool has_qual = o.in_type != 0;
        while (next_record(r)) {
            const int L = (int)r.len;
            if (L < min_len) continue;
            if (seq_num >= max_seq) break;
            seq_num++;
            if (need5) ends5.emplace_back(r.seq, (size_t)check_len);
            if (need3) ends3.emplace_back(rev_comp(std::string(r.seq + (L - check_len), (size_t)check_len)));
            if (has_qual)
                for (int i = 0; i < check_len; i++) { const char c = r.qual[i]; if (min_qc > c) min_qc = c; if (max_qc < c) max_qc = c; }
        }
    }
    const double t_read = pp_now() - t0;
    if (o.in_type == 1 || o.in_type == 2) {
        if (min_qc >= 33 && min_qc <= 78 && max_qc >= 33 && max_qc <= 127) R.qtype = 33;
        else if (min_qc >= 64 && min_qc <= 108 && max_qc >= 64 && max_qc <= 127) R.qtype = 64;
        else R.qtype = min_qc < 55 ? 33 : 64;
        std::cerr << "INFO: base quality scoring: Phred" << R.qtype << std::endl;
        const int maxq = max_qc - R.qtype;
        if (o.min_q >= 0) {
            if (o.min_q >= maxq) {
                std::cerr << "Warning: max base quality score was: " << maxq << std::endl;
                std::cerr << "INFO: Please reset -q parameter." << std::endl;
                quit(255);
            }
        } else {
            if (maxq > 10 && o.read_type == "clr") o.min_q = 10;
            else if (maxq > 20 && o.read_type == "hifi") o.min_q = 20;
            else if (maxq > 10 && o.read_type == "ont") o.min_q = 10;
            else o.min_q = 0;
        }
    }
    const double t1 = pp_now();
    double t_bc = 0;
    if (o.filter) {
        {
            std::thread t3;
            if (o.tail_trim < 0) t3 = std::thread([&] { R.trim3p = check_base_content(ends3, check_len, seq_num, o.end_bias); });
            if (o.head_trim < 0) R.trim5p = check_base_content(ends5, check_len, seq_num, o.end_bias);
            if (t3.joinable()) t3.join();
        }
        if (o.head_trim < 0 && o.tail_trim < 0 && R.trim5p > o.bc_len) R.trim5p = o.bc_len;
        t_bc = pp_now() - t1;
        if (o.adapter_file.empty()) {
            adapter_search(o, ends5, R.adapter5p, R.depth5p);
            adapter_search(o, ends3, R.adapter3p, R.depth3p);
        }
    }
    if (getenv("TGSF_TIMING"))
        fprintf(stderr, "PREPASS: %d reads looked at in %.3f s | base content %.3f | adapter search %.3f (contexts %.3f, %d alignment calls %.3f)\n",
                seq_num, t_read, t_bc, pp_now() - t1 - t_bc, g_pp_create, g_pp_calls, g_pp_align);
    return R;
}

}
```

tgsfilter_amd/host/run.h:

```cpp
#pragma once
#include <memory>

#include "api.h"
#include "pipeline.h"
#include "prepass.h"
#include "report.h"
#include "shard.h"

namespace host {

int cpu_budget();
[[noreturn]] void leave(int code);
bool detached();

struct Run {
    explicit Run(Options& opts) : o(opts) {}

    int set_up_ranks();
    int check_file_types();
    void open_input();
    void open_output_early();
    void prepass();
    void make_contexts();
    void filter_pass();
    void downsample();
    void sum_tallies();
    void report();
    void timing_lines();

    Options& o;
    RankLink link;
    bool shard_may_use_rccl = false;
    bool sharded = false;
    bool timing = false;
    double t_epoch0 = 0, t_start = 0;
    double t_drain = 0, t_prepass = 0, t_pipe = 0, t_parse = 0, t_gpu = 0, t_write = 0, t_widle = 0, t_first = 0;

    std::string html;
    bool fasta_in = false;
    InputBytes in;
    bool streaming = false;
    size_t chunk_bytes = 64u << 20;
    int scan_threads = 1;
    size_t text_off = 0, text_size = 0;
    const char* text = nullptr;
    std::unique_ptr<RecordIndex> records_p;
    std::unique_ptr<ChunkReader> open_stream();

    std::string out_path;
    MappedSink sink;
    std::atomic<bool> early_stop{false};
    std::thread early;
    void end_early() { if (early.joinable()) { early_stop = true; early.join(); } }
    Output out;
    bool fastq_out = false, run_filter_pass = true;

    PrepassResult pp;
    std::vector<std::string> adapters;

    uint64_t batch_text = 0;
    uint32_t batch_reads = 1u << 16;
    const Api* api = nullptr;
    double t_load = 0, t_dev = 0, t_libwait = 0;
    const RcclApi* R = nullptr;
    struct RcclUp { std::atomic<int> done{0}; int rc = TGSF_OK; std::string err; void* comm = nullptr; };
    std::shared_ptr<RcclUp> rccl_state = std::make_shared<RcclUp>();
    std::thread rccl_up;
    bool use_rccl = false;
    bool ranks_own_gpus = false;
    tgsf_params p;
    std::vector<int> ctx_dev;
    std::vector<tgsf_ctx*> ctxs;
    double t_p0 = 0;

    std::unique_ptr<Channel<std::shared_ptr<Batch>>> to_gpu, to_writer;
    std::vector<int> raw_lens, clean_lens;
    uint64_t raw_bases = 0, clean_bases = 0;
    uint64_t own_raw_bases = 0;
    std::vector<CleanRec> clean_recs;
    BatchStore store;
    std::atomic<uint64_t> stream_text{0};
    std::atomic<double> stream_share{0.0};
    std::mutex gpu_time_m;
    bool numa_bind = false;
    std::vector<int> dev_node;
    std::vector<double> dev_submit_s;
    std::vector<uint64_t> dev_bytes, dev_batches;
    int fill_threads = 1, populate_threads = 1;
    uint64_t fill_min = 1u << 20, stride_bytes = 2ull << 30;
    std::unique_ptr<Pool> pool, populate;
    std::unique_ptr<Reserver> reserver;
    bool release_input = false, release_output = false;
    std::unique_ptr<Channel<std::pair<const char*, uint64_t>>> to_release;
    bool mapped_out = false;
    double t_f0 = 0, t_busy = 0, t_fill_tail = 0, t_close = 0;
    void reader_body();
    void feed(size_t k);
    void bind_to_node_of(size_t k);
    void writer_body();
    void fill_job(const std::shared_ptr<Batch>& b, size_t lo, size_t hi);
    void batch_done(std::shared_ptr<Batch> b);

    std::unique_ptr<MappedSink> dsink;
    std::unique_ptr<Pool> dpop;
    std::unique_ptr<Reserver> dres;
    bool open_dsink(uint64_t capacity, uint64_t speculative);
    uint64_t down_bases = 0, down_job_recs = 0, down_job_bases = 0;
    std::vector<int> down_lens;
    std::vector<uint64_t> down_t;
    double t_dsel = 0, t_dcreate = 0, t_dqc = 0, t_dwrite = 0, t_dclose = 0, t_dsubmit = 0, t_dfirst = 0, d_kept = 0, d_span = 0;
    int n_dsubmit = 0;
    bool d_in_place = false, d_mapped = false;
    std::vector<char> select_kept();
    void second_pass(const std::vector<char>& keep);

    uint64_t nw = 0;
    int32_t bc = 0;
    uint32_t nbins = 0;
    std::vector<uint64_t> t;
    double t_x0 = 0, t_rccl_wait = 0, t_allreduce = 0;
    int rccl_ranks = 0;
    std::string tally_route;
    bool reports() const { return !sharded || link.rank == 0; }
};

std::vector<uint64_t> pack_rows(const std::vector<uint64_t>& v, int32_t bc, uint32_t nbins);
void add_rows(std::vector<uint64_t>& v, const std::vector<uint64_t>& ru, int32_t bc, uint32_t nbins);

}
```

tgsfilter_amd/host/run_contexts.cpp:

```cpp
#include "run.h"

namespace host {

void Run::prepass()
{
    std::unique_ptr<CpuScope> cpu_prepass(new CpuScope(CPU_PREPASS));
    if (sharded && link.rank > 0) {
    } else if (streaming) {
        std::unique_ptr<ChunkReader> cr = open_stream();
        std::shared_ptr<Chunk> ch;
        size_t at = 0;
        bool over = false;
        pp = run_prepass(o, [&](Rec& r) {
            while (!over && (!ch || at >= ch->recs.size())) {
                if (ch && !ch->message.empty()) std::cerr << ch->message << std::endl;
                if (ch && ch->last) { over = true; break; }
                ch = cr->next(o.in_file);
                at = 0;
                if (!ch) over = true;
            }
            if (over) return false;
            r = ch->recs[at++];
            return true;
        });
    } else if (sharded && link.world > 1) {
        RecordIndex whole(in.data(), in.size(), !fasta_in, std::max(scan_threads, std::min(8, cpu_budget() / 2)), 1u << 14);
        RecordIndex::Cursor cur(whole);
        pp = run_prepass(o, [&](Rec& r) { return cur.next(r); });
    } else {
        RecordIndex::Cursor cur(*records_p);
        pp = run_prepass(o, [&](Rec& r) { return cur.next(r); });
    }
    if (sharded) {
        BlobOut b;
        if (link.rank == 0) { b.pod(pp.qtype); b.pod(pp.trim5p); b.pod(pp.trim3p); b.pod(pp.depth5p); b.pod(pp.depth3p); b.pod(o.min_q); b.str(pp.adapter5p); b.str(pp.adapter3p); }
        link.bcast(b.s);
        BlobIn r(b.s);
        r.pod(pp.qtype); r.pod(pp.trim5p); r.pod(pp.trim3p); r.pod(pp.depth5p); r.pod(pp.depth3p); r.pod(o.min_q); r.str(pp.adapter5p); r.str(pp.adapter3p);
    }
    cpu_prepass.reset();
    t_prepass = now_s() - t_start;
    if (o.filter) {
        if (o.head_trim < 0) o.head_trim = pp.trim5p;
        if (o.tail_trim < 0) o.tail_trim = pp.trim3p;
        std::cerr << "INFO: trim 5' end length: " << o.head_trim << std::endl;
        std::cerr << "INFO: trim 3' end length: " << o.tail_trim << std::endl;
        std::cerr << "INFO: min output reads length: " << o.min_len << std::endl;
        if (!fasta_in) std::cerr << "INFO: min Phred average quality score: " << o.min_q << std::endl;
        auto add = [&](const std::string& a) { if (std::find(adapters.begin(), adapters.end(), a) == adapters.end()) adapters.push_back(a); };
        if (!o.adapter_file.empty()) {
            InputBytes af;
            if (af.open(o.adapter_file)) {
                const int ft = file_type(o.adapter_file);
                FastxReader rd(af.data(), af.size(), ft == 1);
                Record r;
                while (rd.next(r)) { add(std::string(r.seq)); add(rev_comp(std::string(r.seq))); }
            }
            int num = 0;
            for (const std::string& a : adapters) std::cerr << "INFO: input adapter " << ++num << " :" << a << std::endl;
        } else {
            std::string a5 = pp.adapter5p, a3 = pp.adapter3p;
            float d5 = pp.depth5p, d3 = pp.depth3p;
            if (d5 > 5 * d3) { a3.clear(); d3 = 0; } else if (d3 > 5 * d5) { a5.clear(); d5 = 0; }
            std::cerr << "INFO: 5' adapter: " << a5 << std::endl;
            std::cerr << "INFO: 3' adapter: " << a3 << std::endl;
            std::cerr << "INFO: mean depth of 5' adapter: " << d5 << std::endl;
            std::cerr << "INFO: mean depth of 3' adapter: " << d3 << std::endl;
            if (o.only_adapters) leave(0);
            if (!a5.empty()) { add(a5); add(rev_comp(a5)); }
            if (!a3.empty()) { add(a3); add(rev_comp(a3)); }
            if (a5.empty() && a3.empty()) {
                if (o.read_type == "hifi" || o.read_type == "clr") {
                    add(kAdapterLib[0]); add(kAdapterLib[1]);
                    std::cerr << "INFO: set PacBio blunt adapter to trim: " << kAdapterLib[0] << std::endl;
                } else if (o.read_type == "ont") {
                    add(kAdapterLib[8]); add(kAdapterLib[9]);
                    std::cerr << "INFO: set NanoPore rapid adapter to trim: " << kAdapterLib[8] << std::endl;
                }
            }
        }
    }
}

void Run::make_contexts()
{
    batch_text = streaming ? std::min<uint64_t>(256ull << 20, chunk_bytes)
                                    : std::min<uint64_t>(256ull << 20, std::max<uint64_t>(text_size / 8 + 4096, 1 << 16));
    if (const char* e = knob("TGSF_BATCH_BYTES")) { const long long v = atoll(e); if (v > 0) batch_text = (uint64_t)v; }
    batch_reads = 1u << 16;
    {
        uint64_t per_read = 0, cols = 0, words = 1;
        for (const std::string& a : adapters) {
            const int Q = (int)a.size();
            const int kmax = std::max(0, std::min(Q - 1, std::max(Q - o.end_match_len + 1, Q - o.mid_match_len + 1)));
            cols = std::max<uint64_t>(cols, (uint64_t)(Q + kmax + 2));
            words = std::max<uint64_t>(words, Q > 256 ? (uint64_t)(Q + 63) / 64 : Q > 128 ? 4 : Q > 64 ? 2 : 1);
        }
        per_read = cols * 2 * words * 8;
        if (words > 4) per_read = std::min<uint64_t>(per_read, (1ull << 20) + 16 * words) + 32 * words + 512;
        per_read *= 3 * std::max<size_t>(adapters.size(), 1);
        if (per_read) batch_reads = (uint32_t)std::min<uint64_t>(batch_reads, std::max<uint64_t>(256, (4ull << 30) / per_read));
    }
    fastq_out = o.out_type == 1;
    run_filter_pass = o.filter || o.only_qc;
    {
        const char* w = getenv("TGSF_WRITER");
        const bool may_map = !o.only_qc && !o.out_gz && !o.downsample && run_filter_pass && !o.out_file.empty() &&
                             !(w && !strcmp(w, "writev"));
        if (may_map && !sink.is_open()) sink.open(out_path, streaming ? std::max<uint64_t>(64ull << 30, 64ull * in.size())
                                                                      : 4 * (uint64_t)text_size + (1ull << 30));
        Options oo = o;
        oo.out_file = out_path;
        if (!o.only_qc && !sink.is_open() && !out.open(oo)) leave(1);
    }
    api = &lib();
    const Api& L = *api;
    lib_times(t_load, t_dev);
    t_libwait = now_s() - t_start - t_prepass;
    if (sharded) {
        const char* ex = getenv("TGSF_SHARD_EXCHANGE");
        if (shard_may_use_rccl) R = rccl_lib();
        char bus[64] = {0};
        int node = -1;
        if (L.device_location(o.device, bus, (int)sizeof bus, &node) != TGSF_OK) snprintf(bus, sizeof bus, "device%d", o.device);
        BlobOut mine;
        mine.str(bus);
        mine.pod<int>(R ? 1 : 0);
        const std::vector<std::string> all = link.gather(mine.s);
        std::string verdict(2, '0');
        if (link.rank == 0) {
            std::vector<std::string> seen;
            bool ok = R != nullptr, own = true;
            for (const std::string& a : all) {
                BlobIn in2(a);
                std::string b2; int have = 0;
                in2.str(b2); in2.pod(have);
                own = own && std::find(seen.begin(), seen.end(), b2) == seen.end();
                ok = ok && have;
                seen.push_back(b2);
            }
            ok = ok && own;
            verdict[0] = own ? '1' : '0';
            if (ok) {
                char id[TGSF_RCCL_ID_BYTES];
                if (R->unique_id(id) == TGSF_OK) { verdict[1] = '1'; verdict.append(id, sizeof id); }
                else if (ex && !strcmp(ex, "rccl")) die(std::string("TGSF_SHARD_EXCHANGE=rccl: ") + R->last_error());
            } else if (ex && !strcmp(ex, "rccl")) die("TGSF_SHARD_EXCHANGE=rccl: ranks share a GPU, or libtgsf_rccl.so does not load on every rank");
        }
        link.bcast(verdict);
        ranks_own_gpus = verdict.size() >= 2 && verdict[0] == '1';
        use_rccl = verdict.size() == 2 + TGSF_RCCL_ID_BYTES && verdict[1] == '1';
        if (use_rccl)
            rccl_up = std::thread([R = R, up = rccl_state, verdict, device = o.device, rank = link.rank, world = link.world] {
                if (const char* e = knob("TGSF_RCCL_STALL_S")) usleep((useconds_t)(atof(e) * 1e6));
                up->rc = R->comm_init(device, verdict.data() + 2, rank, world, &up->comm);
                if (up->rc != TGSF_OK) up->err = R->last_error();
                up->done.store(1, std::memory_order_release);
            });
    }
    memset(&p, 0, sizeof p);
    p.struct_size = sizeof p;
    p.min_len = o.min_len; p.max_len = o.max_len; p.min_q = o.min_q < 0 ? 0.f : o.min_q; p.max_q = o.max_q;
    p.bc_len = o.bc_len; p.head_trim = o.head_trim < 0 ? 0 : o.head_trim; p.tail_trim = o.tail_trim < 0 ? 0 : o.tail_trim;
    p.end_len = o.end_len; p.end_match_len = o.end_match_len; p.mid_match_len = o.mid_match_len; p.extra_len = o.extra_len;
    p.end_sim = o.end_sim; p.mid_sim = o.mid_sim; p.discard = o.discard; p.filter = o.filter; p.only_qc = o.only_qc;
    p.min_repeat = o.min_repeat; p.kmer = o.kmer; p.qtype = pp.qtype ? pp.qtype : 33;
    p.no_qual = fasta_in ? 1 : 0;
    if (adapters.size() > TGSF_MAX_ADAPTERS) die("more than " + std::to_string(TGSF_MAX_ADAPTERS) + " adapter sequences");
    p.n_adapters = (int)adapters.size();
    for (size_t a = 0; a < adapters.size(); a++) { p.adapters[a] = adapters[a].data(); p.adapter_len[a] = (int)adapters[a].size(); }
    p.max_batch_reads = batch_reads;
    if (streaming) p.max_read_len = 1u << 26;
    else if (sharded) {
        if (in.size() <= (1ull << 30)) { records_p->wait_complete(); p.max_read_len = (uint32_t)std::max<uint64_t>(link.max_u64(records_p->longest()), 1024); }
        else p.max_read_len = (uint32_t)std::min<uint64_t>(std::max<uint64_t>(in.size() / 2, 1024), 1u << 26);
    }
    else if (records_p->complete()) p.max_read_len = std::max<uint32_t>(records_p->longest(), 1024);
    else p.max_read_len = (uint32_t)std::min<uint64_t>(std::max<uint64_t>(in.size() / 2, 1024), 1u << 26);
    p.max_batch_bases = std::max<uint64_t>(batch_text, 2ull * p.max_read_len + (1u << 16)) + (1 << 20);
    int per_dev = (streaming || text_size > (64u << 20)) ? 3 : 1;
    if (const char* e = getenv("TGSF_CTX_PER_DEVICE")) { const int v = atoi(e); if (v >= 1 && v <= 8) per_dev = v; }
    for (int d : o.devices) for (int k = 0; k < per_dev; k++) ctx_dev.push_back(d);
    ctxs.assign(ctx_dev.size(), nullptr);
    t_p0 = now_s();
}

}
```

tgsfilter_amd/host/run_pipeline.cpp:

```cpp
#include "run.h"

#include <sched.h>

namespace host {

void Run::reader_body()
{
    CpuScope cpu(CPU_BATCHER);
    if (!run_filter_pass) { for (size_t d = 0; d < ctxs.size(); d++) to_gpu->put(nullptr); return; }
    std::unique_ptr<RecordIndex::Cursor> rd;
    if (!streaming) rd.reset(new RecordIndex::Cursor(*records_p));
    std::unique_ptr<ChunkReader> cr;
    if (streaming) cr = open_stream();
    std::shared_ptr<Chunk> ch;
    size_t ch_at = 0;
    bool over = false;
    Rec r;
    auto fresh = [&] { return store.get(); };
    std::shared_ptr<Batch> b = fresh();
    const double t0 = now_s();
    double waited = 0;
    uint64_t next_id = 0;
    auto flush = [&] {
        if (b->recs.empty()) return;
// ... 13 lines not shown
            ch_at = 0;
            if (!ch) { over = true; break; }
            stream_text.store(cr->text_bytes());
            stream_share.store(cr->consumed());
        }
        if (over) return false;
        r = ch->recs[ch_at++];
        return true;
    };
    auto bad_cut = [&](size_t at) {
        die("--ranks / --shard: the input cannot be cut near byte " + std::to_string(at) + " the way one sequential reader would read it "
            "(lines the reader skips, or a malformed record, near there): run it without --ranks / --shard");
    };
    const char* last_end = nullptr;
    while (next_record()) {
        const size_t L = r.len;
        if (L > p.max_read_len) die("read longer than the supported maximum");
        const char* rec_end = (fasta_in ? r.seq : r.qual) + L;
        if (sharded && !last_end && link.rank > 0 && r.name != text + 1) bad_cut(text_off);
        last_end = rec_end;
        if (!b->recs.empty() && ((uint64_t)(rec_end - b->base) > batch_text || b->recs.size() >= batch_reads)) flush();
        if (b->recs.empty()) { b->base = r.name; b->hold = ch; }
        b->off.push_back((uint64_t)(r.seq - b->base));
        b->qoff.push_back(fasta_in ? b->off.back() : (uint64_t)(r.qual - b->base));
        b->len.push_back((uint32_t)L); b->recs.push_back(r);
        b->span = (uint64_t)(rec_end - b->base);
        if (b->span > p.max_batch_bases) die("record larger than a batch");
        b->bases += L;
        raw_bases += L; raw_lens.push_back((int)L);
    }
    if (sharded && link.rank + 1 < link.world) {
        const char* e = last_end ? last_end : text;
        const char* const end = text + text_size;
        if (e < end && *e == '\r') e++;
        if (e < end && *e == '\n') e++;
        if (e != end || !records_p->end_message().empty()) bad_cut(text_off + text_size);
    }
    flush();
    for (size_t d = 0; d < ctxs.size(); d++) to_gpu->put(nullptr);
    t_parse = now_s() - t0 - waited;
    std::sort(raw_lens.begin(), raw_lens.end());
}

void Run::bind_to_node_of(size_t k)
{
    const Api& L = *api;
    int node = -1;
    char bus[64];
    if (L.device_location(ctx_dev[k], bus, (int)sizeof bus, &node) == TGSF_OK && node >= 0) {
        const char* sysfs = knob("TGSF_SYSFS_NODES");
        std::ifstream f(std::string(sysfs ? sysfs : "/sys/devices/system/node") + "/node" + std::to_string(node) + "/cpulist");
        std::string list;
        cpu_set_t set;
        CPU_ZERO(&set);
        int n_set = 0;
        if (f && std::getline(f, list)) {
            size_t i = 0;
            while (i < list.size()) {
                const int a = atoi(list.c_str() + i);
                int b = a;
                size_t j = list.find_first_of(",-", i);
                if (j != std::string::npos && list[j] == '-') { b = atoi(list.c_str() + j + 1); j = list.find(',', j); }
                for (int c2 = a; c2 <= b && c2 < CPU_SETSIZE; c2++) { CPU_SET(c2, &set); n_set++; }
                i = j == std::string::npos ? list.size() : j + 1;
            }
        }
        cpu_set_t allowed;
        if (n_set > 0 && sched_getaffinity(0, sizeof allowed, &allowed) == 0) {
            n_set = 0;
            for (int c2 = 0; c2 < CPU_SETSIZE; c2++) {
                if (CPU_ISSET(c2, &set) && !CPU_ISSET(c2, &allowed)) CPU_CLR(c2, &set);
                if (CPU_ISSET(c2, &set)) n_set++;
            }
        }
        if (n_set > 0 && sched_setaffinity(0, sizeof set, &set) == 0) dev_node[k] = node;
    }
}

void Run::feed(size_t k)
{
    CpuScope cpu(CPU_FEEDER);
    const Api& L = *api;
    if (numa_bind) bind_to_node_of(k);
    if (L.create(&p, ctx_dev[k], &ctxs[k]) != TGSF_OK) die(L.last_error(nullptr));
    tgsf_ctx* fctx = ctxs[k];
    if (timing) (void)L.profile(fctx, 1);
    for (;;) {
        std::shared_ptr<Batch> b = to_gpu->get();
        if (!b) break;
        const double g0 = now_s();
        if (b->res.size() < b->recs.size()) b->res.resize(b->recs.size());
        const size_t fneed = (size_t)(b->bases / (uint64_t)std::max(p.min_len, 1)) + b->recs.size() + 16;
        if (b->frags.size() < fneed) b->frags.resize(fneed);
        const uint8_t* btext = reinterpret_cast<const uint8_t*>(b->base);
        tgsf_batch_in bi;
        memset(&bi, 0, sizeof bi);
        bi.seq = btext; bi.qual = btext;
        bi.offsets = b->off.data(); bi.qual_offsets = b->qoff.data(); bi.lengths = b->len.data();
        bi.n_reads = (uint32_t)b->recs.size(); bi.n_bytes = b->span;
        tgsf_batch_out bo{b->res.data(), b->frags.data(), (uint32_t)b->frags.size(), 0};
        if (L.submit(fctx, &bi, &bo) != TGSF_OK) die(L.last_error(fctx));
        { std::lock_guard<std::mutex> l(gpu_time_m); t_gpu += now_s() - g0; if (t_first == 0) t_first = now_s() - t_p0; }
        dev_submit_s[k] += now_s() - g0; dev_bytes[k] += b->span; dev_batches[k]++;
        b->n_frags = bo.n_frags;
        to_writer->put(std::move(b));
    }
    to_writer->put(nullptr);
}

void Run::batch_done(std::shared_ptr<Batch> b)
{
    if (b->out_bytes && release_output) to_release->put({b->dst, b->out_bytes});
    if (release_input) to_release->put({b->base, b->span});
    store.put(std::move(b));
}

void Run::filter_pass()
{
    to_gpu.reset(new Channel<std::shared_ptr<Batch>>(2 + ctxs.size()));
    to_writer.reset(new Channel<std::shared_ptr<Batch>>(256));
    if (!run_filter_pass) {
        RecordIndex::Cursor rd(*records_p);
        Rec r;
        while (rd.next(r)) {
            clean_recs.push_back({std::string_view(r.name, r.name_len), 1, r.seq, r.qual, r.len});
            clean_bases += r.len;
        }
    }

    std::thread reader([this] { reader_body(); });

    numa_bind = o.devices.size() > 1 || (link.world > 1 && ranks_own_gpus);
    if (const char* e = getenv("TGSF_NUMA")) numa_bind = atoi(e) > 0;
    dev_node.assign(ctx_dev.size(), -1);
    dev_submit_s.assign(ctx_dev.size(), 0.0);
    dev_bytes.assign(ctx_dev.size(), 0);
    dev_batches.assign(ctx_dev.size(), 0);
    std::vector<std::thread> feeders;
    for (size_t k = 0; k < ctxs.size(); k++) feeders.emplace_back([this, k] { feed(k); });

    fill_threads = std::max(1, std::min(o.n_thread, 16));
    fill_min = 1u << 20;
    if (const char* e = knob("TGSF_FILL_MIN_BYTES")) { const long long v = atoll(e); if (v > 0) fill_min = (uint64_t)v; }
    pool.reset(new Pool(sink.is_open() ? fill_threads : 1));
    populate_threads = std::max(1, std::min(o.n_thread, 32));
    if (const char* e = knob("TGSF_POPULATE_THREADS")) { const int v = atoi(e); if (v >= 1 && v <= 64) populate_threads = v; }
    populate.reset(new Pool(sink.is_open() ? populate_threads : 0, CPU_POPULATE));
    stride_bytes = streaming ? (128ull << 20) : (2ull << 30);
    if (const char* e = knob("TGSF_STRIDE_BYTES")) { const long long v = atoll(e); if (v > 0) stride_bytes = (uint64_t)v; }
    end_early();
    reserver.reset(new Reserver(sink, *populate, stride_bytes, false));
    if (sink.is_open())
        reserver->start((!streaming && text_size > (256u << 20)) ? (uint64_t)text_size / 4 : 0);
    {
        uint64_t early_min = 1ull << 30;
        if (const char* e = knob("TGSF_DOWN_EARLY_MIN")) early_min = strtoull(e, nullptr, 10);
        if (o.downsample && !streaming && in.mapped() && (uint64_t)text_size >= early_min) {
            uint64_t spec = (uint64_t)text_size / 4;
            if (o.genome_size > 0 && o.desired_depth > 0) spec = std::min<uint64_t>(spec, (2 * o.genome_size * (uint64_t)o.desired_depth) / (uint64_t)link.world + (uint64_t)text_size / 64);
            open_dsink(4 * (uint64_t)text_size + (1ull << 30), spec);
        }
    }
    const bool sync_exit = !detached();
    release_input = sync_exit && !streaming && in.mapped() && !o.downsample;
    release_output = sync_exit || streaming;
    const uint64_t release_piece = 16u << 20;
    to_release.reset(new Channel<std::pair<const char*, uint64_t>>(1 << 16));
// ... 28 lines not shown
```

tgsfilter_amd/host/run_report.cpp:

```cpp
#include "run.h"

#include <sys/stat.h>

namespace host {

std::vector<uint64_t> pack_rows(const std::vector<uint64_t>& v, int32_t bc2, uint32_t nb2)
{
    const size_t head = tgsf_ctr_bin_table(0, bc2, nb2);
    std::vector<uint64_t> out(v.begin(), v.begin() + (long)head);
    for (int b = 0; b < 4; b++) {
        const size_t at = tgsf_ctr_bin_table(b, bc2, nb2), n = (size_t)std::min<uint64_t>(v[TGSF_CTR_ROWS + (b >> 1)], nb2) * 5;
        out.insert(out.end(), v.begin() + (long)at, v.begin() + (long)(at + n));
    }
    return out;
}

void add_rows(std::vector<uint64_t>& v, const std::vector<uint64_t>& ru, int32_t bc2, uint32_t nb2)
{
    const size_t head = tgsf_ctr_bin_table(0, bc2, nb2);
    if (ru.size() < head) die("a rank of the job sent a tally vector of another layout");
    uint64_t rows[4];
    for (int q = 0; q < 4; q++) rows[q] = std::max(v[TGSF_CTR_ROWS + q], ru[TGSF_CTR_ROWS + q]);
    for (size_t i = 0; i < head; i++) v[i] += ru[i];
    size_t from = head;
// ... 161 lines not shown
        const uint64_t* d = &t[TGSF_CTR_DROPINFO];
        std::cerr << "INFO: " << raw_lens.size() << " reads with a total of " << raw_bases << " bases were input." << std::endl;
        if (!o.only_qc) {
            std::cerr << "INFO: " << d[0] << " reads were discarded with " << d[1] << " bases due to low quality." << std::endl;
            std::cerr << "INFO: " << d[2] << " reads have adapter at 5', 3' and middle." << std::endl;
            std::cerr << "INFO: " << d[3] << " reads have adapter at 5' and middle." << std::endl;
            std::cerr << "INFO: " << d[4] << " reads have adapter at 3' and middle." << std::endl;
            std::cerr << "INFO: " << d[5] << " reads have adapter at 5' and 3' end." << std::endl;
            std::cerr << "INFO: " << d[6] << " reads only have adapter at middle." << std::endl;
            std::cerr << "INFO: " << d[7] << " reads only have adapter at 5' end." << std::endl;
            std::cerr << "INFO: " << d[8] << " reads only have adapter at 3' end." << std::endl;
            std::cerr << "INFO: " << d[9] << " reads didn't have any adapter." << std::endl;
            std::cerr << "INFO: " << d[10] << " bases were trimmed due to the adapter or base content bias." << std::endl;
            std::cerr << "INFO: " << d[11] << " reads were discarded with " << d[12] << " bases due to the short length." << std::endl;
            std::cerr << "INFO: " << d[13] << " reads were discarded with " << d[14] << " bases due to low quality after split." << std::endl;
            if (o.min_repeat > 0)
                std::cerr << "INFO: " << d[15] << " reads were discarded with " << d[16] << " bases due to short repeat length." << std::endl;
            std::cerr << "INFO: " << clean_num << " reads with a total of " << clean_bases << " bases after filtering." << std::endl;
            if (!o.downsample && !o.out_file.empty()) {
                if (!sharded) std::cerr << "INFO: Filtered reads were written to: " << o.out_file << "." << std::endl;
                else std::cerr << "INFO: Filtered reads were written to: " << o.out_file << ".part0 ... " << o.out_file << ".part" << link.world - 1
                               << " (" << link.world << " parts; concatenated in this order they are the reads in input order)." << std::endl;
            }
        }
    }
    if (reports() && sharded && !o.out_file.empty() && !o.only_qc && !o.only_adapters) {
        const std::string list = o.out_file + ".parts";
        std::vector<std::string> earlier;
        {
            std::ifstream f(list);
            std::string line;
            if (f && std::getline(f, line) && line == "# tgsfilter parts, in order")
                while (std::getline(f, line)) if (!line.empty()) earlier.push_back(line);
        }
        std::vector<std::string> mine;
        for (int k = 0; k < link.world; k++) mine.push_back(o.out_file + ".part" + std::to_string(k));
        for (const std::string& e : earlier) {
            if (std::find(mine.begin(), mine.end(), e) != mine.end()) continue;
            const std::string stem = o.out_file + ".part";
            if (e.compare(0, stem.size(), stem) != 0 || e.size() == stem.size() || e.find_first_not_of("0123456789", stem.size()) != std::string::npos) continue;
            struct stat st;
            if (lstat(e.c_str(), &st) == 0 && S_ISREG(st.st_mode) && unlink(e.c_str()) == 0)
                std::cerr << "Warning: " << e << ", a part of an earlier job with more ranks, was removed." << std::endl;
        }
        for (int k = link.world; k < link.world + 1024; k++) {
            const std::string other = o.out_file + ".part" + std::to_string(k);
            struct stat st;
            if (lstat(other.c_str(), &st) != 0) { if (k >= link.world + 64) break; else continue; }
            std::cerr << "Warning: " << other << " exists and is not a part of this job (nor of an earlier one this tool listed): `cat " << o.out_file
                      << ".part*` would take it in -- the parts of this job are listed in " << list << "." << std::endl;
        }
        std::ofstream f(list, std::ios::trunc);
        f << "# tgsfilter parts, in order\n";
        for (const std::string& m : mine) f << m << "\n";
    }
    if (o.downsample && reports()) {
        if (down_lens.empty()) die("no reads to downsample");
        std::sort(down_lens.begin(), down_lens.end());
        side_stats(bc, down_lens, down_bases, tables(down_t, false), clean);
        clean.tab[8] = limit_decimals(std::round(clean.mean_qual * 1000) / 1000.0, 2);
        if (!o.filter)
            std::cerr << "INFO: " << (sharded ? down_job_recs : clean_recs.size()) << " reads with a total of " << (sharded ? down_job_bases : clean_bases) << " bases were input." << std::endl;
        std::cerr << "INFO: " << down_lens.size() << " reads with a total of " << down_bases << " bases after downsampling." << std::endl;
        if (!o.out_file.empty()) {
            if (!sharded) std::cerr << "INFO: Downsampled reads were written to: " << o.out_file << "." << std::endl;
            else std::cerr << "INFO: Downsampled reads were written to: " << o.out_file << ".part0 ... " << o.out_file << ".part" << link.world - 1
                           << " (" << link.world << " parts; concatenated in this order they are the reads in input order)." << std::endl;
        }
    }
    std::string qc = fasta_in ? "0" : "1";
    qc += o.only_qc ? "0" : ((!o.filter && o.downsample) ? "1" : "2");
    if (reports()) {
        std::ofstream ofs(html);
        write_report(ofs, qc, raw, clean);
        ofs.close();
        std::cerr << "INFO: Quality control report was written to: " << html << "." << std::endl;
    }
}

void Run::timing_lines()
{
    const Api& L = *api;
    if (timing) {
        fprintf(stderr, "POOL: %zu jobs, busy %.3f, freeing job state %.3f, longest job %.3f, first job at %.3f, last job done at %.3f (pipeline start = 0, planner done at %.3f)\n",
                pool->jobs_, t_busy, pool->destroy_, pool->longest_, pool->first_ - t_p0, pool->last_ - t_p0, t_f0 - t_p0);
        fprintf(stderr, "TIMING: total %.3f s | index+prepass %.3f | waiting for the library %.3f (load %.3f + device %.3f, beside the pre-pass) | "
                        "pipeline %.3f (batching %.3f, tgsf_submit summed over %zu feeders %.3f, plan+write %.3f, planner waiting %.3f, "
                        "first batch filtered after %.3f, fill tail %.3f, closing the output %.3f; stages overlap) | stats+report %.3f | %s (fallocate %.3f, mapping the reserved pages %.3f, fill threads busy %.3f summed)\n",
                now_s() - t_start, t_prepass, t_libwait, t_load, t_dev, t_pipe, t_parse, ctxs.size(), t_gpu, t_write, t_widle, t_first,
                t_fill_tail, t_close, now_s() - t_p0 - t_pipe, mapped_out ? "output: fallocate + mapped fill" : "output: writev", sink.t_falloc, reserver->t_populate_wait, t_busy);
        fprintf(stderr, "RESERVE: planner waited %.3f s for pages of the output file\n", t_drain);
    }
    if (timing) {
        float tot[TGSF_N_STAGES] = {0};
        uint32_t nb = 0;
        for (tgsf_ctx* c : ctxs) {
            float ms[TGSF_N_STAGES]; uint32_t n1 = 0;
            if (c && L.stage_times(c, ms, &n1) == TGSF_OK) { nb += n1; for (int i = 0; i < TGSF_N_STAGES; i++) tot[i] += ms[i]; }
        }
        double sum = 0;
        for (int i = 0; i < TGSF_N_STAGES; i++) sum += tot[i];
        char piece[256];
        snprintf(piece, sizeof piece, "GPU: kernels %.3f s summed over %zu contexts and %u batches (upper bound of the busy time: contexts overlap) = %.4f of the run |", sum * 1e-3, ctxs.size(), nb,
                 sum * 1e-3 / std::max(1e-9, now_s() - t_start));
        std::string line = piece;
        for (int i = 0; i < TGSF_N_STAGES; i++) if (tot[i] > 0) { snprintf(piece, sizeof piece, " %s %.1f ms", L.stage_name(i), tot[i]); line += piece; }
        line += "\n";
        fputs(line.c_str(), stderr);
    }
    if (timing) {
        for (size_t di = 0; di < o.devices.size(); di++) {
            if (std::find(o.devices.begin(), o.devices.begin() + (long)di, o.devices[di]) != o.devices.begin() + (long)di) continue;
            double sub = 0; uint64_t by = 0, nb2 = 0; int nf2 = 0, node = -1;
            for (size_t k = 0; k < ctx_dev.size(); k++)
                if (ctx_dev[k] == o.devices[di]) { sub += dev_submit_s[k]; by += dev_bytes[k]; nb2 += dev_batches[k]; nf2++; node = std::max(node, dev_node[k]); }
            fprintf(stderr, "DEVICE %d: %llu batches, %.2f GB of text through %d feeders, tgsf_submit %.3f s summed = %.1f GB/s per feeder, %.1f GB/s for the device over the pipeline's %.3f s%s\n",
                    o.devices[di], (unsigned long long)nb2, by * 1e-9, nf2, sub, sub > 0 ? by * 1e-9 / sub : 0.0, t_pipe > 0 ? by * 1e-9 / t_pipe : 0.0, t_pipe,
                    node >= 0 ? (" (feeders bound to NUMA node " + std::to_string(node) + ")").c_str() : "");
        }
    }
    if (timing) {
        const double proc = process_cpu_s();
        double own = 0;
        std::string line;
        char piece[160];
        for (int s = 0; s < CPU_N; s++) {
            double v = (double)cpu_ns()[s].load() * 1e-9;
            if (s == CPU_MAIN) v += (double)thread_cpu_ns() * 1e-9 - (double)cpu_ns()[CPU_PREPASS].load() * 1e-9;
            own += v;
            if (v >= 0.0005) { snprintf(piece, sizeof piece, "%s %s %.3f", line.empty() ? "" : ",", cpu_stage_name(s), v); line += piece; }
        }
        snprintf(piece, sizeof piece, "CPU: %.3f s of CPU time (user + system) for %.3f Gbases = %.4f CPU-s per Gbase |", proc, (double)own_raw_bases * 1e-9,
                 own_raw_bases ? proc / ((double)own_raw_bases * 1e-9) : 0.0);
        std::string head = piece;
        snprintf(piece, sizeof piece, " | threads of the runtime and others %.3f\n", proc - own);
        fputs((head + line + piece).c_str(), stderr);
    }
    if (timing && o.downsample)
        fprintf(stderr, "DOWN: selection %.3f | QC pass over the kept reads (%s, %.2f GB of them in %.2f GB of text): context %.3f, batches + submits %.3f (its own thread; %d submits %.3f, the first %.3f) | writing them %.3f (%s) | closing the output %.3f\n",
                t_dsel, d_in_place ? "read in place" : "packed", d_kept * 1e-9, d_span * 1e-9, t_dcreate, t_dqc, n_dsubmit, t_dsubmit, t_dfirst, t_dwrite, d_mapped ? "fallocate + threads into a mapping" : "writev", t_dclose);
    if (timing) {
        struct timespec ts; clock_gettime(CLOCK_REALTIME, &ts);
        fprintf(stderr, "CLOCK: main entered at %.6f, leaving at %.6f (epoch seconds)\n", t_epoch0, (double)ts.tv_sec + ts.tv_nsec * 1e-9);
    }
}

}
```

tgsfilter_amd/host/run_setup.cpp:

```cpp
#include "run.h"

#include <sched.h>
#include <sys/stat.h>

namespace host {

int Run::set_up_ranks()
{
    if (o.ranks >= 1 && o.shard_world > 0) { std::cerr << "Error: --ranks starts the ranks itself; --shard is for a rank started by another launcher" << std::endl; return 1; }
    if (o.ranks >= 1 || o.shard_world >= 1) {
        const int world = o.ranks >= 1 ? o.ranks : o.shard_world;
        const char* why = nullptr;
        if (o.out_file.empty() && !o.only_qc && !o.only_adapters) why = "every rank writes a part file of its own: -o is needed";
        else if (file_type(o.in_file) == 2 || (o.in_file.size() > 3 && o.in_file.compare(o.in_file.size() - 3, 3, ".gz") == 0))
            why = "the ranks take byte ranges of a plain FASTQ / FASTA text";
        if (why) { std::cerr << "Error: --ranks / --shard: " << why << std::endl; return 1; }
        if (world > 1024) { std::cerr << "Error: --ranks " << world << std::endl; return 1; }
        {
            std::vector<int> dv;
            for (int r = 0; r < world && o.ranks >= 1; r++) dv.push_back(o.devices.empty() ? r : o.devices[(size_t)r % o.devices.size()]);
            std::sort(dv.begin(), dv.end());
            shard_may_use_rccl = o.ranks < 1 || std::adjacent_find(dv.begin(), dv.end()) == dv.end();
            const char* ex = getenv("TGSF_SHARD_EXCHANGE");
            if (ex && !strcmp(ex, "socket")) shard_may_use_rccl = false;
        }
        if (o.ranks >= 1) {
            fork_ranks(world, link);
            o.device = o.devices.empty() ? link.rank : o.devices[(size_t)link.rank % o.devices.size()];
        } else {
            if (o.rendezvous.empty()) { std::cerr << "Error: --shard needs --rendezvous <path>: where the ranks of the job meet (a unix socket)" << std::endl; return 1; }
            setenv("HSA_ENABLE_IPC_MODE_LEGACY", "0", 0);
            link.rendezvous(o.shard_rank, world, o.rendezvous);
        }
        o.devices.assign(1, o.device);
        o.n_thread = std::max(2, std::min(o.n_thread, std::max(o.n_thread / world, cpu_budget() / world)));
    }
    sharded = o.ranks >= 1 || o.shard_world >= 1;
    return 0;
}

int Run::check_file_types()
{
    o.in_type = file_type(o.in_file);
    const std::string prefix = file_prefix(o.in_file);
    html = prefix + ".html";
    if (!o.out_file.empty() && !o.only_qc) {
        html = file_prefix(o.out_file) + ".html";
        o.out_type = file_type(o.out_file);
        if (file_extension(o.out_file) == "gz") o.out_gz = true;
    } else {
        o.out_type = o.fasta_out ? 0 : (o.in_type == 2 ? 1 : o.in_type);
    }
    if (o.in_type == 3 || o.out_type == 3) {
        std::cerr << "Error: The file name suffix should be '.[fastq|fq|fasta|fa][.gz] or .[sam|bam]'" << std::endl;
        if (o.in_type == 3) std::cerr << "Error: Please check your input file name: " << o.in_file << std::endl;
        else std::cerr << "Error: Please check your output file name: " << o.out_file << std::endl;
        return 1;
    }
    if (o.in_type == 0 && o.out_type == 1) { std::cerr << "Error: Fasta format input file can't output fastq format file" << std::endl; return 1; }
    fasta_in = o.in_type == 0;
    return 0;
}

std::unique_ptr<ChunkReader> Run::open_stream()
{
    std::string err;
    std::unique_ptr<TextSource> src = open_text(in.data(), in.size(), o.in_type == 2, err);
    if (!src) { std::cerr << "Error: " << err << " (" << o.in_file << ")" << std::endl; fflush(nullptr); _exit(255); }
    return std::unique_ptr<ChunkReader>(new ChunkReader(std::move(src), !fasta_in, chunk_bytes, 20));
}

void Run::open_input()
{
    if (o.devices.empty()) o.devices.push_back(o.device);
    lib_start(o.devices);
    if (sharded && shard_may_use_rccl) rccl_start();

    const bool coded = o.in_type == 2 || (o.in_file.size() > 3 && o.in_file.compare(o.in_file.size() - 3, 3, ".gz") == 0);
    uint64_t stream_min = 256ull << 20;
    if (const char* e = knob("TGSF_STREAM_MIN_BYTES")) stream_min = strtoull(e, nullptr, 10);
    if (coded && !o.downsample) {
        if (!in.open_raw(o.in_file)) leave(1);
        streaming = in.size() >= stream_min;
    }
    if (!streaming && !in.open(o.in_file, o.in_type == 2)) leave(1);
    chunk_bytes = [] { const char* e = knob("TGSF_CHUNK_BYTES"); return e ? (size_t)strtoull(e, nullptr, 10) : (size_t)(64u << 20); }();
    const int budget = std::max(1, cpu_budget() / link.world);
    scan_threads = std::max(1, std::min({o.n_thread, 32, std::max(2, budget / 2)}));
    text_off = 0; text_size = in.size();
    if (sharded) {
        if (streaming || (in.size() > 0 && !in.mapped())) die("--ranks / --shard: the input is not a plain text file");
        const size_t lo = find_record_start(in.data(), in.size(), (size_t)((unsigned __int128)in.size() * (unsigned)link.rank / (unsigned)link.world), !fasta_in);
        const size_t hi = link.rank + 1 == link.world ? in.size()
                        : find_record_start(in.data(), in.size(), (size_t)((unsigned __int128)in.size() * (unsigned)(link.rank + 1) / (unsigned)link.world), !fasta_in);
        text_off = lo; text_size = hi > lo ? hi - lo : 0;
    }
    text = in.data() + text_off;
    if (!streaming) records_p.reset(new RecordIndex(text, text_size, !fasta_in, scan_threads));
}

void Run::open_output_early()
{
    out_path = sharded && !o.out_file.empty() ? o.out_file + ".part" + std::to_string(link.rank) : o.out_file;
    {
        const char* w = getenv("TGSF_WRITER");
        uint64_t early_min = 256ull << 20;
        if (const char* e = knob("TGSF_EARLY_OPEN_MIN")) early_min = strtoull(e, nullptr, 10);
        const bool may_map_early = !o.only_qc && !o.out_gz && !o.downsample && (o.filter || o.only_qc) && !o.out_file.empty() &&
                                   !(w && !strcmp(w, "writev")) && !o.only_adapters && !streaming && in.mapped() &&
                                   (uint64_t)text_size >= early_min;
        if (may_map_early && sink.open(out_path, 4 * (uint64_t)text_size + (1ull << 30), true))
            early = std::thread([this] {
                CpuScope cpu(CPU_FALLOCATE);
                const uint64_t limit = (uint64_t)text_size / 4;
                while (!early_stop.load() && sink.reserved() < limit)
                    if (!sink.reserve_to(std::min<uint64_t>(limit, sink.reserved() + (256u << 20)), false)) break;
            });
    }
}

}
```

Measured before the change: 6.670.

## Reserve device contexts ahead of time and carve allocations from one block

Adds tgsf_reserve/tgsf_release_reserved so that streams, events, pinned buffers and one large device block per context are allocated during the pre-pass, using upper-bound parameters. tgsf_create can then take a reserved resource set instead of calling the allocator many times. Per-context allocations are carved from a single block, and table build is split from table upload. The aim is to keep context creation latency out of the critical path, at the cost of possibly over-allocating memory from the upper-bound estimate and some added complexity.

New measurement: 6.675, median of 2. Within noise of the previous version (+0.1%).

```diff
diff --git a/include/tgsf.h b/include/tgsf.h
--- a/include/tgsf.h
+++ b/include/tgsf.h
@@ -8,7 +8,7 @@
 extern "C" {
 #endif
 
-#define TGSF_ABI_VERSION 3
+#define TGSF_ABI_VERSION 4
 #define TGSF_MAX_ADAPTERS 32
 #define TGSF_MAX_ADAPTER_LEN 8192
 #define TGSF_N_DROPINFO 17
@@ -135,6 +135,10 @@
 int tgsf_create(const tgsf_params* params, int device, tgsf_ctx** out_ctx);
 void tgsf_destroy(tgsf_ctx* ctx);
 
+int tgsf_reserve(const tgsf_params* upper, int device, int n_contexts);
+int tgsf_release_reserved(int device);
+int tgsf_alloc_stats(uint64_t out[5]);
+
 int tgsf_submit(tgsf_ctx* ctx, const tgsf_batch_in* in, tgsf_batch_out* out);
 int tgsf_submit_async(tgsf_ctx* ctx, const tgsf_batch_in* in, tgsf_batch_out* out);
 
diff --git a/tgsfilter_amd/abi.py b/tgsfilter_amd/abi.py
--- a/tgsfilter_amd/abi.py
+++ b/tgsfilter_amd/abi.py
@@ -4,7 +4,7 @@
 
 import numpy as np
 
-ABI_VERSION = 3
+ABI_VERSION = 4
 MAX_ADAPTERS = 32
 MAX_ADAPTER_LEN = 8192
 N_DROPINFO = 17
diff --git a/tgsfilter_amd/capi.py b/tgsfilter_amd/capi.py
--- a/tgsfilter_amd/capi.py
+++ b/tgsfilter_amd/capi.py
@@ -12,7 +12,7 @@
 _LIBS = {}
 
 SYMBOLS = [
-    "tgsf_abi_version", "tgsf_backend", "tgsf_prepare_device", "tgsf_device_location", "tgsf_create", "tgsf_destroy", "tgsf_submit", "tgsf_submit_async", "tgsf_submit_device",
+    "tgsf_abi_version", "tgsf_backend", "tgsf_prepare_device", "tgsf_device_location", "tgsf_create", "tgsf_destroy", "tgsf_reserve", "tgsf_release_reserved", "tgsf_alloc_stats", "tgsf_submit", "tgsf_submit_async", "tgsf_submit_device",
     "tgsf_wait",
     "tgsf_counters_len", "tgsf_counters", "tgsf_counters_used", "tgsf_counters_merge", "tgsf_counters_device", "tgsf_reset_counters", "tgsf_profile",
     "tgsf_stage_times", "tgsf_stage_name", "tgsf_align_windows", "tgsf_last_error",
@@ -44,6 +44,9 @@
     L.tgsf_create.argtypes = [C.POINTER(abi.Params), C.c_int, C.POINTER(vp)]
     L.tgsf_destroy.argtypes = [vp]
     L.tgsf_destroy.restype = None
+    L.tgsf_reserve.argtypes = [C.POINTER(abi.Params), C.c_int, C.c_int]
+    L.tgsf_release_reserved.argtypes = [C.c_int]
+    L.tgsf_alloc_stats.argtypes = [C.POINTER(u64 * 5)]
     L.tgsf_submit.argtypes = [vp, C.POINTER(abi.BatchIn), C.POINTER(abi.BatchOut)]
     L.tgsf_submit_async.argtypes = [vp, C.POINTER(abi.BatchIn), C.POINTER(abi.BatchOut)]
     L.tgsf_submit_device.argtypes = [vp, C.POINTER(abi.BatchIn), C.POINTER(abi.BatchOut), vp, vp]
@@ -68,6 +71,24 @@
                            "(there is no CPU fallback; is TGSF_LIB set by accident?)")
     _LIBS[path] = L
     return L
+
+
+def reserve(upper: abi.Params, device: int = 0, n_contexts: int = 1, lib_path: str | None = None):
+    L = load(lib_path)
+    rc = L.tgsf_reserve(C.byref(upper), device, n_contexts)
+    if rc != 0:
+        raise TgsfError(rc, L.tgsf_last_error(None).decode())
+
+
+def release_reserved(device: int = 0, lib_path: str | None = None) -> int:
+    return int(load(lib_path).tgsf_release_reserved(device))
+
+
+def alloc_stats(lib_path: str | None = None) -> dict:
+    out = (C.c_uint64 * 5)()
+    load(lib_path).tgsf_alloc_stats(C.byref(out))
+    return {"allocations_made": int(out[0]), "allocations_live": int(out[1]), "contexts_created": int(out[2]), "reserved_held": int(out[3]),
+            "contexts_from_reserve": int(out[4])}
 
 
 class Context:
diff --git a/tgsfilter_amd/csrc/tgsf_lib.hip b/tgsfilter_amd/csrc/tgsf_lib.hip
--- a/tgsfilter_amd/csrc/tgsf_lib.hip
+++ b/tgsfilter_amd/csrc/tgsf_lib.hip
@@ -4,6 +4,9 @@
 #include <string.h>
 
 #include <algorithm>
+#include <atomic>
+#include <map>
+#include <mutex>
 #include <string>
 #include <vector>
 
@@ -54,7 +57,11 @@
     tgsf_read_result* d_out_reads;
     tgsf_fragment* d_out_frags;
     uint32_t* d_out_nfrags;
-    std::vector<void*> allocs;
+    struct ctx_resources* res = nullptr;
+    void* pool_own = nullptr;
+    uint8_t* aw_buf = nullptr;
+    size_t aw_cap = 0;
+    struct host_tables* tab = nullptr;
     bool profile;
     float stage_ms[TGSF_N_STAGES];
     uint32_t prof_batches;
@@ -111,26 +118,125 @@
 static unsigned grid_cap(unsigned g) { return g; }
 #endif
 
-template <class T>
-static int dev_alloc(tgsf_ctx* c, T** p, size_t count)
-{
-    void* v = nullptr;
-    int e = rt_malloc(&v, count * sizeof(T) + 64);
-    if (e) return fail(c, TGSF_E_HIP, "device allocation of %zu bytes failed: %s", count * sizeof(T), rt_errstr(e));
-    c->allocs.push_back(v);
-    *p = (T*)v;
+static std::atomic<uint64_t> g_allocs_made{0}, g_allocs_live{0}, g_ctx_created{0}, g_ctx_from_reserve{0};
+static int dev_malloc(void** p, size_t n)
+{
+    const int e = rt_malloc(p, n);
+    if (e) return e;
+    g_allocs_made++; g_allocs_live++;
+#if defined(TGSF_EMUL)
+    if (const char* fill = knob("TGSF_EMUL_FILL")) memset(*p, (int)strtol(fill, nullptr, 0), n ? n : 1);
+#endif
     return 0;
 }
-
-static int build_tables(tgsf_ctx* c)
+static void dev_free(void* p)
+{
+    if (!p) return;
+    rt_free(p);
+    g_allocs_live--;
+}
+
+struct ctx_resources {
+    int device = 0;
+    void* block = nullptr;
+    size_t bytes = 0;
+    bool staging = false;
+    uint8_t* pinned = nullptr;
+#if !defined(TGSF_EMUL)
+    static constexpr size_t kStageBytes = tgsf_ctx::kStageBytes;
+    hipStream_t stream = nullptr, aux = nullptr;
+    hipEvent_t ev_fork = nullptr, ev_join = nullptr, stage_ev[2] = {nullptr, nullptr};
+#endif
+};
+
+static void res_release(ctx_resources* r)
+{
+    if (!r) return;
+#if !defined(TGSF_EMUL)
+    (void)hipSetDevice(r->device);
+    if (r->pinned) (void)hipHostFree(r->pinned);
+    for (int i = 0; i < 2; i++) if (r->stage_ev[i]) (void)hipEventDestroy(r->stage_ev[i]);
+    if (r->ev_fork) (void)hipEventDestroy(r->ev_fork);
+    if (r->ev_join) (void)hipEventDestroy(r->ev_join);
+    if (r->aux) (void)hipStreamDestroy(r->aux);
+    if (r->stream) (void)hipStreamDestroy(r->stream);
+#endif
+    dev_free(r->block);
+    delete r;
+}
+
+static ctx_resources* res_acquire(int device, size_t bytes, bool staging, int* code, std::string* err)
+{
+    ctx_resources* r = new ctx_resources();
+    r->device = device; r->staging = staging;
+    char buf[256];
+#define RES_FAIL(c, ...) do { snprintf(buf, sizeof buf, __VA_ARGS__); *err = buf; *code = (c); res_release(r); return nullptr; } while (0)
+#if !defined(TGSF_EMUL)
+    hipError_t he;
+    if ((he = hipSetDevice(device)) != hipSuccess) RES_FAIL(TGSF_E_HIP, "hipSetDevice: %s", hipGetErrorString(he));
+    if ((he = hipStreamCreateWithFlags(&r->stream, hipStreamNonBlocking)) != hipSuccess) RES_FAIL(TGSF_E_HIP, "hipStreamCreate: %s", hipGetErrorString(he));
+    {
+        const size_t pb = 256 + (staging ? 2 * ctx_resources::kStageBytes : 0);
+        if (hipHostMalloc((void**)&r->pinned, pb, hipHostMallocDefault) != hipSuccess || !r->pinned) {
+            r->pinned = nullptr;
+            (void)hipGetLastError();
+            if (staging) RES_FAIL(TGSF_E_HIP, "pinned staging buffers: allocation failed");
+        } else memset(r->pinned, 0, 64);
+    }
+    {
+        int lo = 0, hi = 0;
+        (void)hipDeviceGetStreamPriorityRange(&lo, &hi);
+        he = hipStreamCreateWithPriority(&r->aux, hipStreamNonBlocking, hi);
+    }
+    if (he != hipSuccess ||
+        (he = hipEventCreateWithFlags(&r->ev_fork, hipEventDisableTiming)) != hipSuccess ||
+        (he = hipEventCreateWithFlags(&r->ev_join, hipEventDisableTiming)) != hipSuccess)
+        RES_FAIL(TGSF_E_HIP, "auxiliary stream: %s", hipGetErrorString(he));
+    for (int i = 0; i < 2 && staging; i++)
+        if (hipEventCreateWithFlags(&r->stage_ev[i], hipEventDisableTiming) != hipSuccess) RES_FAIL(TGSF_E_HIP, "pinned staging buffers: allocation failed");
+#endif
+    {
+        const int e = dev_malloc(&r->block, bytes);
+        if (e) RES_FAIL(TGSF_E_HIP, "device allocation of %zu bytes failed: %s", bytes, rt_errstr(e));
+        r->bytes = bytes;
+    }
+#undef RES_FAIL
+    return r;
+}
+
+static std::mutex g_reserve_m;
+static std::map<int, std::vector<ctx_resources*>> g_reserved;
+
+struct Carver {
+    uintptr_t base;
+    size_t off = 0;
+    template <class T> void take(T** p, size_t count)
+    {
+        off = (off + 255) & ~(size_t)255;
+        *p = (T*)(base + off);
+        off += count * sizeof(T) + 64;
+    }
+};
+
+struct host_tables {
+    std::vector<uint8_t> ad;
+    std::vector<uint64_t> fwd, rev, top, fw, rw;
+    uint8_t* d_ad = nullptr;
+    uint64_t *d_f = nullptr, *d_r = nullptr, *d_t = nullptr, *d_fw = nullptr, *d_rw = nullptr;
+};
+
+static void build_tables(tgsf_ctx* c)
 {
     const tgsf_params& p = c->params;
     DevParams& P = c->P;
     const int A = p.n_adapters;
-    std::vector<uint8_t> ad((size_t)kMaxAdapters * kMaxQ, 0);
+    host_tables& H = *c->tab;
+    std::vector<uint8_t>& ad = H.ad;
+    std::vector<uint64_t>&fwd = H.fwd, &rev = H.rev, &top = H.top;
+    ad.assign((size_t)kMaxAdapters * kMaxQ, 0);
     const size_t per_ad = (size_t)256 * kPeqW;
-    std::vector<uint64_t> fwd((size_t)kMaxAdapters * per_ad, 0), rev((size_t)kMaxAdapters * per_ad, 0),
-        top((size_t)kMaxAdapters * 256, 0);
+    fwd.assign((size_t)kMaxAdapters * per_ad, 0); rev.assign((size_t)kMaxAdapters * per_ad, 0);
+    top.assign((size_t)kMaxAdapters * 256, 0);
     P.max_nw = 1;
     P.min_Q = 1 << 30;
     for (int a = 0; a < A; a++) {
@@ -165,40 +271,36 @@
         }
     }
     if (A == 0) P.min_Q = 1 << 30;
-    uint8_t* d_ad; uint64_t *d_f, *d_r, *d_t;
-    int e;
-    if ((e = dev_alloc(c, &d_ad, ad.size()))) return e;
-    if ((e = dev_alloc(c, &d_f, fwd.size()))) return e;
-    if ((e = dev_alloc(c, &d_r, rev.size()))) return e;
-    if ((e = dev_alloc(c, &d_t, top.size()))) return e;
-    rt_h2d(d_ad, ad.data(), ad.size(), c->stream);
-    rt_h2d(d_f, fwd.data(), fwd.size() * 8, c->stream);
-    rt_h2d(d_r, rev.data(), rev.size() * 8, c->stream);
-    rt_h2d(d_t, top.data(), top.size() * 8, c->stream);
-    rt_sync(c->stream);
-    P.adapter = d_ad; P.peq_fwd = d_f; P.peq_rev = d_r; P.peq_top = d_t;
-    P.peq_fwd_w = P.peq_rev_w = nullptr;
     if (P.max_nw > 4) {
         const size_t per_w = (size_t)256 * kWideNW;
-        std::vector<uint64_t> fw((size_t)A * per_w, 0), rw((size_t)A * per_w, 0);
+        H.fw.assign((size_t)A * per_w, 0); H.rw.assign((size_t)A * per_w, 0);
         for (int a = 0; a < A; a++) {
             const std::string& s = c->adapters[a];
             const int Q = (int)s.size();
             for (int r = 0; r < Q; r++) {
                 const uint8_t cf = (uint8_t)s[r], cr = (uint8_t)s[Q - 1 - r];
-                fw[(size_t)a * per_w + (size_t)cf * kWideNW + (r >> 6)] |= 1ull << (r & 63);
-                rw[(size_t)a * per_w + (size_t)cr * kWideNW + (r >> 6)] |= 1ull << (r & 63);
+                H.fw[(size_t)a * per_w + (size_t)cf * kWideNW + (r >> 6)] |= 1ull << (r & 63);
+                H.rw[(size_t)a * per_w + (size_t)cr * kWideNW + (r >> 6)] |= 1ull << (r & 63);
             }
         }
-        uint64_t *d_fw, *d_rw;
-        if ((e = dev_alloc(c, &d_fw, fw.size()))) return e;
-        if ((e = dev_alloc(c, &d_rw, rw.size()))) return e;
-        rt_h2d(d_fw, fw.data(), fw.size() * 8, c->stream);
-        rt_h2d(d_rw, rw.data(), rw.size() * 8, c->stream);
-        rt_sync(c->stream);
-        P.peq_fwd_w = d_fw; P.peq_rev_w = d_rw;
-    }
-    return 0;
+    }
+}
+
+static void upload_tables(tgsf_ctx* c)
+{
+    host_tables& H = *c->tab;
+    DevParams& P = c->P;
+    rt_h2d(H.d_ad, H.ad.data(), H.ad.size(), c->stream);
+    rt_h2d(H.d_f, H.fwd.data(), H.fwd.size() * 8, c->stream);
+    rt_h2d(H.d_r, H.rev.data(), H.rev.size() * 8, c->stream);
+    rt_h2d(H.d_t, H.top.data(), H.top.size() * 8, c->stream);
+    P.adapter = H.d_ad; P.peq_fwd = H.d_f; P.peq_rev = H.d_r; P.peq_top = H.d_t;
+    P.peq_fwd_w = P.peq_rev_w = nullptr;
+    if (P.max_nw > 4) {
+        rt_h2d(H.d_fw, H.fw.data(), H.fw.size() * 8, c->stream);
+        rt_h2d(H.d_rw, H.rw.data(), H.rw.size() * 8, c->stream);
+        P.peq_fwd_w = H.d_fw; P.peq_rev_w = H.d_rw;
+    }
 }
 
 extern "C" int tgsf_abi_version(void) { return TGSF_ABI_VERSION; }
@@ -298,7 +400,7 @@
 extern "C" void tgsf_destroy(tgsf_ctx* c)
 {
     if (!c) return;
-    if (c->B.bp_allowed && c->B.bp_state && knob("TGSF_TRACE_BP")) {
+    if (c->res && c->B.bp_allowed && c->B.bp_state && knob("TGSF_TRACE_BP")) {
         uint32_t w[4] = {0, 0, 0, 0};
         uint64_t pl[4] = {0, 0, 0, 0};
         uint32_t sg[4] = {0, 0, 0, 0};
@@ -308,29 +410,22 @@
     }
 #if !defined(TGSF_EMUL)
     (void)hipSetDevice(c->device);
-    (void)hipStreamSynchronize(c->stream);
+    if (c->stream) (void)hipStreamSynchronize(c->stream);
     for (int k = 0; k < tgsf_ctx::kProfRing; k++) {
         for (int i = 0; i <= TGSF_N_STAGES; i++) if (c->ev[k][i]) (void)hipEventDestroy(c->ev[k][i]);
         for (int i = 0; i < 3; i++) if (c->ev_aux[k][i]) (void)hipEventDestroy(c->ev_aux[k][i]);
     }
-    if (c->h_pinned) (void)hipHostFree(c->h_pinned);
-    for (int i = 0; i < 2; i++) {
-        if (c->stage[i]) (void)hipHostFree(c->stage[i]);
-        if (c->stage_ev[i]) (void)hipEventDestroy(c->stage_ev[i]);
-    }
-    if (c->ev_fork) (void)hipEventDestroy(c->ev_fork);
-    if (c->ev_join) (void)hipEventDestroy(c->ev_join);
-    if (c->aux) (void)hipStreamDestroy(c->aux);
-    if (c->own_stream && c->stream) (void)hipStreamDestroy(c->stream);
-#endif
-    for (void* p : c->allocs) rt_free(p);
+#endif
+    res_release(c->res);
+    dev_free(c->pool_own);
+    dev_free(c->aw_buf);
+    delete c->tab;
     delete c;
 }
 
-extern "C" int tgsf_create(const tgsf_params* p, int device, tgsf_ctx** out)
-{
-    if (!p || !out) return fail(nullptr, TGSF_E_INVALID, "null argument");
-    *out = nullptr;
+static int check_params(const tgsf_params* p)
+{
+    if (!p) return fail(nullptr, TGSF_E_INVALID, "null argument");
     if (p->struct_size != sizeof(tgsf_params))
         return fail(nullptr, TGSF_E_INVALID, "tgsf_params.struct_size %u != %zu (ABI mismatch)", p->struct_size, sizeof(tgsf_params));
     if (p->n_adapters < 0 || p->n_adapters > TGSF_MAX_ADAPTERS)
@@ -353,6 +448,11 @@
         return fail(nullptr, TGSF_E_INVALID, "max_batch_bases / max_batch_reads / max_read_len must be set");
     if (p->max_read_len > (1u << 28)) return fail(nullptr, TGSF_E_INVALID, "max_read_len above 2^28");
 
+    return TGSF_OK;
+}
+
+static tgsf_ctx* new_host_ctx(const tgsf_params* p, int device)
+{
     tgsf_ctx* c = new tgsf_ctx();
     c->params = *p;
     c->device = device;
@@ -362,59 +462,15 @@
     memset(c->h_words_, 0, sizeof c->h_words_);
     c->h_status = c->h_words_;
     c->pend_nf_p = c->h_words_ + 4;
-    for (int a = 0; a < p->n_adapters; a++) {
-        c->adapters.emplace_back(p->adapters[a], (size_t)p->adapter_len[a]);
-        c->params.adapters[a] = c->adapters.back().data();
-    }
+    for (int a = 0; a < p->n_adapters; a++) c->adapters.emplace_back(p->adapters[a], (size_t)p->adapter_len[a]);
     for (int a = 0; a < p->n_adapters; a++) c->params.adapters[a] = c->adapters[a].data();
 #if !defined(TGSF_EMUL)
     memset(c->ev, 0, sizeof c->ev);
     memset(c->ev_aux, 0, sizeof c->ev_aux);
     c->aux = nullptr; c->ev_fork = c->ev_join = nullptr;
-    int ndev = 0;
-    hipError_t he = hipGetDeviceCount(&ndev);
-    if (he != hipSuccess || ndev <= 0) {
-        delete c;
-        return fail(nullptr, TGSF_E_NO_DEVICE, "no HIP device available (%s); libtgsf has no CPU fallback", hipGetErrorString(he));
-    }
-    if (device < 0 || device >= ndev) { delete c; return fail(nullptr, TGSF_E_NO_DEVICE, "device %d out of range (%d devices)", device, ndev); }
-    set_wait_mode(device);
-    if ((he = hipSetDevice(device)) != hipSuccess) { delete c; return fail(nullptr, TGSF_E_HIP, "hipSetDevice: %s", hipGetErrorString(he)); }
-    if ((he = hipStreamCreateWithFlags(&c->stream, hipStreamNonBlocking)) != hipSuccess) {
-        delete c; return fail(nullptr, TGSF_E_HIP, "hipStreamCreate: %s", hipGetErrorString(he));
-    }
-    c->own_stream = true;
     c->prof_pending = 0;
-    {
-        uint32_t* pw = nullptr;
-        if (hipHostMalloc((void**)&pw, 64, hipHostMallocDefault) == hipSuccess && pw) {
-            memset(pw, 0, 64);
-            c->h_pinned = pw; c->h_status = pw; c->pend_nf_p = pw + 4;
-        }
-    }
-    {
-        int lo = 0, hi = 0;
-        (void)hipDeviceGetStreamPriorityRange(&lo, &hi);
-        he = hipStreamCreateWithPriority(&c->aux, hipStreamNonBlocking, hi);
-    }
-    if (he != hipSuccess ||
-        (he = hipEventCreateWithFlags(&c->ev_fork, hipEventDisableTiming)) != hipSuccess ||
-        (he = hipEventCreateWithFlags(&c->ev_join, hipEventDisableTiming)) != hipSuccess) {
-        tgsf_destroy(c); return fail(nullptr, TGSF_E_HIP, "auxiliary stream: %s", hipGetErrorString(he));
-    }
-#else
+#endif
     c->stream = nullptr; c->own_stream = false;
-#endif
-    c->last_stream = c->stream;
-#if !defined(TGSF_EMUL)
-    if (p->max_batch_bases > (8u << 20)) {
-        for (int i = 0; i < 2; i++)
-            if (hipHostMalloc((void**)&c->stage[i], tgsf_ctx::kStageBytes, hipHostMallocDefault) != hipSuccess ||
-                hipEventCreateWithFlags(&c->stage_ev[i], hipEventDisableTiming) != hipSuccess) {
-                tgsf_destroy(c); return fail(nullptr, TGSF_E_HIP, "pinned staging buffers: allocation failed");
-            }
-    }
-#endif
     DevParams& P = c->P;
     memset(&P, 0, sizeof P);
     P.min_len = p->min_len; P.max_len = p->max_len; P.min_q = p->min_q; P.max_q = p->max_q;
@@ -436,7 +492,24 @@
     if (const char* e = knob("TGSF_MID_FLAT")) c->flat_scan = atoi(e) > 0;
     if (const char* e = knob("TGSF_MID_FILTER")) { int v = atoi(e); if (v >= 0 && v <= 2) c->suffix_filter = v; }
 
-    int e = build_tables(c);
+    c->tab = new host_tables();
+    build_tables(c);
+    return c;
+}
+
+static size_t lay_out(tgsf_ctx* c, uint8_t* base, bool all)
+{
+    const tgsf_params* p = &c->params;
+    DevParams& P = c->P;
+    Carver K{(uintptr_t)base};
+    {
+        host_tables& H = *c->tab;
+        K.take(&H.d_ad, H.ad.size());
+        K.take(&H.d_f, H.fwd.size());
+        K.take(&H.d_r, H.rev.size());
+        K.take(&H.d_t, H.top.size());
+        if (P.max_nw > 4) { K.take(&H.d_fw, H.fw.size()); K.take(&H.d_rw, H.rw.size()); }
+    }
     DevBatch& B = c->B;
     memset(&B, 0, sizeof B);
     B.flat_pmax = 256; B.flat_pmin = 16; B.flat_f0 = 224;
@@ -458,24 +531,24 @@
     B.pool_cap = (uint32_t)std::min<uint64_t>(pool, 1ull << 28);
     if (const char* e = knob("TGSF_POOL_CAP")) { const long long v = atoll(e); if (v >= 1 && v < (1ll << 28)) B.pool_cap = (uint32_t)v; }
     const size_t nitems = n + (size_t)B.fcap;
-    if (!e) e = dev_alloc(c, &c->d_seq, cap_bytes);
-    if (!e) e = dev_alloc(c, &c->d_qual, cap_bytes);
-    if (!e) e = dev_alloc(c, &c->d_off, n + 1);
-    if (!e) e = dev_alloc(c, &c->d_qoff, n + 1);
-    if (!e) e = dev_alloc(c, &c->d_lenin, n);
-    if (!e) e = dev_alloc(c, &B.len, n);
-    if (!e) e = dev_alloc(c, &B.sumq, n);
-    if (!e) e = dev_alloc(c, &B.flags, n);
-    if (!e) e = dev_alloc(c, &B.clip5, n * A);
-    if (!e) e = dev_alloc(c, &B.clip3, n * A);
-    if (!e) e = dev_alloc(c, &B.mid_head, n);
-    if (!e) e = dev_alloc(c, &B.mid_best, n * A);
-    if (!e) e = dev_alloc(c, &B.mid_cnt, n);
-    if (!e) e = dev_alloc(c, &B.mid_gate, n * A);
-    if (!e) e = dev_alloc(c, &B.pool, (size_t)B.pool_cap);
-    if (!e) e = dev_alloc(c, &B.pool_n, 4);
-    if (!e) e = dev_alloc(c, &B.seg_cnt, n + 1);
-    if (!e) e = dev_alloc(c, &B.chk_cnt, n + 1);
+    K.take(&c->d_seq, cap_bytes);
+    K.take(&c->d_qual, cap_bytes);
+    K.take(&c->d_off, n + 1);
+    K.take(&c->d_qoff, n + 1);
+    K.take(&c->d_lenin, n);
+    K.take(&B.len, n);
+    K.take(&B.sumq, n);
+    K.take(&B.flags, n);
+    K.take(&B.clip5, n * A);
+    K.take(&B.clip3, n * A);
+    K.take(&B.mid_head, n);
+    K.take(&B.mid_best, n * A);
+    K.take(&B.mid_cnt, n);
+    K.take(&B.mid_gate, n * A);
+    K.take(&B.pool, (size_t)B.pool_cap);
+    K.take(&B.pool_n, 4);
+    K.take(&B.seg_cnt, n + 1);
+    K.take(&B.chk_cnt, n + 1);
     if (c->cap_bases / 16u + n >= 0xFFFFFFF0ull) c->flat_scan = false;
     if (c->cap_bases / 16u + n >= (1ull << 30) || !c->flat_scan) c->suffix_filter = 0;
     {
@@ -483,45 +556,44 @@
         for (int a = 0; a < p->n_adapters; a++) any |= c->P.Q[a] > 32 && c->P.Q[a] <= 64 && c->P.k_mid[a] >= 0 && c->P.k_mid[a] <= kSuffixMaxK;
         if (!any || !p->filter) c->suffix_filter = 0;
     }
-    if (!e && c->suffix_filter) e = dev_alloc(c, &B.chk_mark, (size_t)4 * (size_t)((c->cap_bases / 16u + n) / 32u + 8u));
-    if (c->suffix_filter) {
+    if (c->suffix_filter || all) K.take(&B.chk_mark, (size_t)4 * (size_t)((c->cap_bases / 16u + n) / 32u + 8u));
+    if (c->suffix_filter || all) {
         B.rc_cap = (uint32_t)std::min<uint64_t>((c->cap_bases / 16u + n) / 25u + 4096u, 1ull << 24);
         if (const char* e2 = knob("TGSF_RECHECK_CAP")) { int v = atoi(e2); if (v >= 0) B.rc_cap = (uint32_t)v; }
-        if (!e) e = dev_alloc(c, &B.rc_list, (size_t)B.rc_cap + 1);
-        if (!e) e = dev_alloc(c, &B.rc_n, 4);
-    }
-    if (!e) e = dev_alloc(c, &B.nfr, n + 1);
-    if (!e) e = dev_alloc(c, &B.scan_part, n / kScanTile + 2);
-    if (!e) e = dev_alloc(c, &B.trimmed, n);
+        K.take(&B.rc_list, (size_t)B.rc_cap + 1);
+        K.take(&B.rc_n, 4);
+    }
+    K.take(&B.nfr, n + 1);
+    K.take(&B.scan_part, n / kScanTile + 2);
+    K.take(&B.trimmed, n);
     B.rep_long_cap = (uint32_t)std::min<uint64_t>(c->cap_bases / kRepShare + 16, (uint64_t)B.fcap + 16);
-    if (!e) e = dev_alloc(c, &B.rep_next, 2 + (size_t)B.rep_long_cap);
+    K.take(&B.rep_next, 2 + (size_t)B.rep_long_cap);
     if (p->min_repeat > 0 && p->kmer >= 12 && p->kmer <= 31) {
         B.rep_tab_log2 = 4;
         while (B.rep_tab_log2 < 40 && (1ull << B.rep_tab_log2) < 2ull * c->max_read_len) B.rep_tab_log2++;
-        if (!e) e = dev_alloc(c, &B.rep_tab, (size_t)1 << B.rep_tab_log2);
-        if (!e) e = dev_alloc(c, &B.rep_lock, 4);
-        if (!e) rt_memset(B.rep_lock, 0, 16, c->stream);
+        K.take(&B.rep_tab, (size_t)1 << B.rep_tab_log2);
+        K.take(&B.rep_lock, 4);
         B.rep_max_plog = kRepMaxPlog;
         if (const char* ev = knob("TGSF_REP_MAX_PLOG")) { int v = atoi(ev); if (v >= 0 && v <= 20) B.rep_max_plog = (uint32_t)v; }
     }
-    if (!e) e = dev_alloc(c, &B.tile_hist, 2 * ((size_t)B.max_tiles + 2));
-    if (!e) e = dev_alloc(c, &B.tile_cnt, 2 * ((size_t)B.max_tiles + 2));
-    if (!e) e = dev_alloc(c, &B.tile_base, 2 * ((size_t)B.max_tiles + 2));
-    if (!e) e = dev_alloc(c, &B.tile_fill, 2 * ((size_t)B.max_tiles + 2));
-    if (!e) e = dev_alloc(c, &B.seg_info, 4);
-    if (!e) e = dev_alloc(c, &B.perm, nitems);
+    K.take(&B.tile_hist, 2 * ((size_t)B.max_tiles + 2));
+    K.take(&B.tile_cnt, 2 * ((size_t)B.max_tiles + 2));
+    K.take(&B.tile_base, 2 * ((size_t)B.max_tiles + 2));
+    K.take(&B.tile_fill, 2 * ((size_t)B.max_tiles + 2));
+    K.take(&B.seg_info, 4);
+    K.take(&B.perm, nitems);
     B.work_cap = (uint32_t)std::min<uint64_t>(2 * (c->cap_bases / kTileBases) + nitems + 16, 0x7FFFFFF0ull);
-    if (!e) e = dev_alloc(c, &B.work, 2 * (size_t)B.work_cap);
-    if (!e) e = dev_alloc(c, &B.frag_off, (size_t)B.fcap);
-    if (!e) e = dev_alloc(c, &B.frag_qoff, (size_t)B.fcap);
-    if (!e) e = dev_alloc(c, &B.frag_len, (size_t)B.fcap);
-    if (!e) e = dev_alloc(c, &B.frag_sum, (size_t)B.fcap);
-    if (!e) e = dev_alloc(c, &B.frag_read, (size_t)B.fcap);
-    if (!e) e = dev_alloc(c, &B.frag_start, (size_t)B.fcap);
-    if (!e) e = dev_alloc(c, &B.frag_flags, (size_t)B.fcap);
-    if (!e) e = dev_alloc(c, &B.raw_tab, 2 * (size_t)c->n_bins * 5);
-    if (!e) e = dev_alloc(c, &B.whole, n);
-    if (!e) e = dev_alloc(c, &B.plan, 4);
+    K.take(&B.work, 2 * (size_t)B.work_cap);
+    K.take(&B.frag_off, (size_t)B.fcap);
+    K.take(&B.frag_qoff, (size_t)B.fcap);
+    K.take(&B.frag_len, (size_t)B.fcap);
+    K.take(&B.frag_sum, (size_t)B.fcap);
+    K.take(&B.frag_read, (size_t)B.fcap);
+    K.take(&B.frag_start, (size_t)B.fcap);
+    K.take(&B.frag_flags, (size_t)B.fcap);
+    K.take(&B.raw_tab, 2 * (size_t)c->n_bins * 5);
+    K.take(&B.whole, n);
+    K.take(&B.plan, 4);
     B.clean_force = p->only_qc ? 1u : 0u;
     B.bp_allowed = (p->filter && !p->only_qc && (p->head_trim > 0 || p->tail_trim > 0) &&
                     p->head_trim >= 0 && p->tail_trim >= 0) ? 1u : 0u;
@@ -531,11 +603,11 @@
         else if (!strcmp(f, "difference") && !p->only_qc) { B.clean_force = 2; B.bp_allowed = 0; }
         else if (!strcmp(f, "byproduct") && B.bp_allowed) B.clean_force = 3;
     }
-    if (B.bp_allowed) {
-        if (!e) e = dev_alloc(c, &B.spec, n);
-        if (!e) e = dev_alloc(c, &B.spec_sum, n);
-        if (!e) e = dev_alloc(c, &B.bp_state, 4);
-        if (!e) e = dev_alloc(c, &c->bp_ring, TGSF_MAX_ENQUEUED);
+    if (B.bp_allowed || all) {
+        K.take(&B.spec, n);
+        K.take(&B.spec_sum, n);
+        K.take(&B.bp_state, 4);
+        K.take(&c->bp_ring, TGSF_MAX_ENQUEUED);
     }
     {
         int maxcols = 1;
@@ -551,19 +623,77 @@
         B.scratch_wave_words = lane_words * 64;
         B.scratch_mid_wave0 = ((size_t)n * A * 2 + 63) / 64 + 1;
         const size_t waves = B.scratch_mid_wave0 + ((size_t)n * A + 63) / 64 + 1;
-        if (!e) e = dev_alloc(c, &B.scratch, waves * B.scratch_wave_words);
-    }
-    if (!e) e = dev_alloc(c, &B.ctr, (size_t)c->ctr_words);
-    if (!e) e = dev_alloc(c, &B.status, 4);
-    if (!e) e = dev_alloc(c, &c->ovf_ring, TGSF_MAX_ENQUEUED);
-    if (!e) e = dev_alloc(c, &c->d_out_reads, n);
-    if (!e) e = dev_alloc(c, &c->d_out_frags, (size_t)B.fcap);
-    if (!e) e = dev_alloc(c, &c->d_out_nfrags, 4);
-    if (e) {
-        g_create_error = c->error;
-        tgsf_destroy(c);
-        return e;
-    }
+        K.take(&B.scratch, waves * B.scratch_wave_words);
+    }
+    K.take(&B.ctr, (size_t)c->ctr_words);
+    K.take(&B.status, 4);
+    K.take(&c->ovf_ring, TGSF_MAX_ENQUEUED);
+    K.take(&c->d_out_reads, n);
+    K.take(&c->d_out_frags, (size_t)B.fcap);
+    K.take(&c->d_out_nfrags, 4);
+    return K.off;
+}
+
+static bool wants_staging(const tgsf_params* p) { return !kTgsfEmul && p->max_batch_bases > (8u << 20); }
+
+extern "C" int tgsf_create(const tgsf_params* p, int device, tgsf_ctx** out)
+{
+    if (!out) return fail(nullptr, TGSF_E_INVALID, "null argument");
+    *out = nullptr;
+    if (const int bad = check_params(p)) return bad;
+#if !defined(TGSF_EMUL)
+    {
+        int ndev = 0;
+        hipError_t he = hipGetDeviceCount(&ndev);
+        if (he != hipSuccess || ndev <= 0)
+            return fail(nullptr, TGSF_E_NO_DEVICE, "no HIP device available (%s); libtgsf has no CPU fallback", hipGetErrorString(he));
+        if (device < 0 || device >= ndev) return fail(nullptr, TGSF_E_NO_DEVICE, "device %d out of range (%d devices)", device, ndev);
+        set_wait_mode(device);
+        if ((he = hipSetDevice(device)) != hipSuccess) return fail(nullptr, TGSF_E_HIP, "hipSetDevice: %s", hipGetErrorString(he));
+    }
+#endif
+    tgsf_ctx* c = new_host_ctx(p, device);
+    const size_t total = lay_out(c, nullptr, false);
+    const bool staging = wants_staging(p);
+    {
+        std::lock_guard<std::mutex> g(g_reserve_m);
+        auto it = g_reserved.find(device);
+        if (it != g_reserved.end())
+            for (size_t i = 0; i < it->second.size(); i++)
+                if (it->second[i]->bytes >= total && it->second[i]->staging == staging) {
+                    c->res = it->second[i];
+                    it->second.erase(it->second.begin() + (long)i);
+                    g_ctx_from_reserve++;
+                    break;
+                }
+    }
+    if (!c->res) {
+        int code = TGSF_E_HIP;
+        std::string err;
+        c->res = res_acquire(device, total, staging, &code, &err);
+        if (!c->res) { tgsf_destroy(c); return fail(nullptr, code, "%s", err.c_str()); }
+    }
+#if !defined(TGSF_EMUL)
+    {
+        ctx_resources& r = *c->res;
+        c->stream = r.stream; c->own_stream = true;
+        c->aux = r.aux; c->ev_fork = r.ev_fork; c->ev_join = r.ev_join;
+        if (r.pinned) {
+            c->h_pinned = (uint32_t*)r.pinned;
+            memset(r.pinned, 0, 64);
+            c->h_status = c->h_pinned; c->pend_nf_p = c->h_pinned + 4;
+        }
+        for (int i = 0; i < 2 && staging; i++) {
+            c->stage[i] = r.pinned + 256 + (size_t)i * tgsf_ctx::kStageBytes;
+            c->stage_ev[i] = r.stage_ev[i];
+        }
+    }
+#endif
+    c->last_stream = c->stream;
+    (void)lay_out(c, (uint8_t*)c->res->block, false);
+    upload_tables(c);
+    DevBatch& B = c->B;
+    if (B.rep_lock) rt_memset(B.rep_lock, 0, 16, c->stream);
     rt_memset(B.ctr, 0, c->ctr_words * 8, c->stream);
     rt_memset(B.status, 0, 16, c->stream);
     rt_memset(c->ovf_ring, 0, TGSF_MAX_ENQUEUED * 4, c->stream);
@@ -575,8 +705,64 @@
         B.bp_used = c->bp_ring;
     }
     rt_memset(B.raw_tab, 0, 2 * (size_t)c->n_bins * 5 * 8, c->stream);
-    rt_sync(c->stream);
+    const int se = rt_sync(c->stream);
+    delete c->tab;
+    c->tab = nullptr;
+    if (se) { tgsf_destroy(c); return fail(nullptr, TGSF_E_HIP, "tgsf_create: device set-up failed: %s", rt_errstr(se)); }
+    g_ctx_created++;
     *out = c;
+    return TGSF_OK;
+}
+
+extern "C" int tgsf_reserve(const tgsf_params* upper, int device, int n_contexts)
+{
+    if (n_contexts < 0) return fail(nullptr, TGSF_E_INVALID, "tgsf_reserve: n_contexts < 0");
+    if (const int bad = check_params(upper)) return bad;
+#if !defined(TGSF_EMUL)
+    {
+        int ndev = 0;
+        if (hipGetDeviceCount(&ndev) != hipSuccess || device < 0 || device >= ndev) return fail(nullptr, TGSF_E_NO_DEVICE, "tgsf_reserve: no HIP device %d", device);
+        set_wait_mode(device);
+        if (hipSetDevice(device) != hipSuccess) return fail(nullptr, TGSF_E_HIP, "tgsf_reserve: hipSetDevice failed");
+    }
+#endif
+    size_t total;
+    {
+        tgsf_ctx* c = new_host_ctx(upper, device);
+        total = lay_out(c, nullptr, true);
+        delete c->tab;
+        delete c;
+    }
+    for (int i = 0; i < n_contexts; i++) {
+        int code = TGSF_E_HIP;
+        std::string err;
+        ctx_resources* r = res_acquire(device, total, wants_staging(upper), &code, &err);
+        if (!r) return fail(nullptr, code, "tgsf_reserve: %s", err.c_str());
+        std::lock_guard<std::mutex> g(g_reserve_m);
+        g_reserved[device].push_back(r);
+    }
+    return TGSF_OK;
+}
+
+extern "C" int tgsf_release_reserved(int device)
+{
+    std::vector<ctx_resources*> mine;
+    {
+        std::lock_guard<std::mutex> g(g_reserve_m);
+        auto it = g_reserved.find(device);
+        if (it != g_reserved.end()) { mine.swap(it->second); g_reserved.erase(it); }
+    }
+    for (ctx_resources* r : mine) res_release(r);
+    return (int)mine.size();
+}
+
+extern "C" int tgsf_alloc_stats(uint64_t out[5])
+{
+    if (!out) return TGSF_E_INVALID;
+    out[0] = g_allocs_made.load(); out[1] = g_allocs_live.load(); out[2] = g_ctx_created.load(); out[4] = g_ctx_from_reserve.load();
+    std::lock_guard<std::mutex> g(g_reserve_m);
+    out[3] = 0;
+    for (const auto& kv : g_reserved) out[3] += kv.second.size();
     return TGSF_OK;
 }
 
@@ -803,8 +989,8 @@
             const uint64_t cells = max_segs * (uint64_t)A + 1;
             if (cells > 0xFFFFFFF0ull) return fail(c, TGSF_E_CAPACITY, "middle scan: too many (segment, adapter) cells for the position-ordered pass");
             uint32_t *seg_n = nullptr, *part = nullptr;
-            if (rt_malloc((void**)&seg_n, (size_t)(cells + 1) * 4 + 64) || rt_malloc((void**)&part, (size_t)(cells / kScanTile + 4) * 4 + 64)) {
-                if (seg_n) rt_free(seg_n);
+            if (dev_malloc((void**)&seg_n, (size_t)(cells + 1) * 4 + 64) || dev_malloc((void**)&part, (size_t)(cells / kScanTile + 4) * 4 + 64)) {
+                dev_free(seg_n);
                 return fail(c, TGSF_E_CAPACITY, "middle scan: no device memory for the position-ordered pass (%.1f GB)", (double)cells * 4e-9);
             }
             B.seg_n = seg_n;
@@ -822,12 +1008,12 @@
                     const uint64_t want = (uint64_t)need + 1024;
                     if (want > 0x7FFFFFF0ull) { rc = fail(c, TGSF_E_CAPACITY, "middle-adapter candidates: %u columns tie their reads' minima, more than one batch can list", need); break; }
                     void* np = nullptr;
-                    if (rt_malloc(&np, (size_t)want * sizeof(MidCand) + 64)) {
+                    if (dev_malloc(&np, (size_t)want * sizeof(MidCand) + 64)) {
                         rc = fail(c, TGSF_E_CAPACITY, "middle-adapter candidates: no device memory for %llu slots (%.1f GB)", (unsigned long long)want, (double)want * sizeof(MidCand) * 1e-9);
                         break;
                     }
-                    for (void*& q : c->allocs) if (q == (void*)c->B.pool) q = np;
-                    rt_free(c->B.pool);
+                    dev_free(c->pool_own);
+                    c->pool_own = np;
                     c->B.pool = (MidCand*)np; c->B.pool_cap = (uint32_t)want;
                     B.pool = c->B.pool; B.pool_cap = c->B.pool_cap;
                     c->pool_regrown++;
@@ -852,8 +1038,8 @@
                 he = rt_sync(ms);
                 if (he) rc = fail(c, TGSF_E_HIP, "middle scan (position-ordered pass) failed: %s", rt_errstr(he));
             } while (0);
-            rt_free(seg_n);
-            rt_free(part);
+            dev_free(seg_n);
+            dev_free(part);
             B.seg_n = nullptr;
             if (rc) return rc;
         }
@@ -1210,15 +1396,27 @@
     uint8_t *d_seq = nullptr, *d_aid = nullptr; uint64_t* d_off = nullptr; uint32_t* d_len = nullptr;
     int32_t *d_k = nullptr, *d_res = nullptr, *d_ends = nullptr;
     int e = 0;
-    e |= rt_malloc((void**)&d_seq, n_bytes + 16);
-    e |= rt_malloc((void**)&d_aid, n);
-    e |= rt_malloc((void**)&d_off, (size_t)n * 8);
-    e |= rt_malloc((void**)&d_len, (size_t)n * 4);
-    e |= rt_malloc((void**)&d_k, (size_t)n * 4);
-    e |= rt_malloc((void**)&d_res, (size_t)n * 16);
-    e |= rt_malloc((void**)&d_ends, (size_t)n * 8);
+    {
+        Carver K{0};
+        K.take(&d_seq, (size_t)n_bytes + 16); K.take(&d_aid, n); K.take(&d_off, n); K.take(&d_len, n);
+        K.take(&d_k, n); K.take(&d_res, (size_t)n * 4); K.take(&d_ends, (size_t)n * 2);
+        if (K.off > c->aw_cap) {
+            (void)rt_sync(c->stream);
+            dev_free(c->aw_buf);
+            c->aw_buf = nullptr; c->aw_cap = 0;
+            void* nb = nullptr;
+            e = dev_malloc(&nb, K.off);
+            if (!e) { c->aw_buf = (uint8_t*)nb; c->aw_cap = K.off; }
+        }
+        if (!e) {
+            Carver R{(uintptr_t)c->aw_buf};
+            R.take(&d_seq, (size_t)n_bytes + 16); R.take(&d_aid, n); R.take(&d_off, n); R.take(&d_len, n);
+            R.take(&d_k, n); R.take(&d_res, (size_t)n * 4); R.take(&d_ends, (size_t)n * 2);
+        }
+    }
     rt_stream st = c->stream;
     if (!e) {
+        e |= rt_memset(d_seq + n_bytes, 0, 16, st);
         e |= rt_h2d(d_seq, seq, n_bytes, st);
         e |= rt_h2d(d_aid, adapter_id, n, st);
         e |= rt_h2d(d_off, win_off, (size_t)n * 8, st);
@@ -1239,6 +1437,5 @@
         e |= rt_d2h(ends, d_ends, (size_t)n * 8, st);
         e |= rt_sync(st);
     }
-    rt_free(d_seq); rt_free(d_aid); rt_free(d_off); rt_free(d_len); rt_free(d_k); rt_free(d_res); rt_free(d_ends);
     return e ? fail(c, TGSF_E_HIP, "tgsf_align_windows: device operation failed") : TGSF_OK;
 }
diff --git a/tgsfilter_amd/host/api.cpp b/tgsfilter_amd/host/api.cpp
--- a/tgsfilter_amd/host/api.cpp
+++ b/tgsfilter_amd/host/api.cpp
@@ -6,9 +6,11 @@
 #include <unistd.h>
 
 #include <chrono>
+#include <condition_variable>
 #include <cstdio>
 #include <cstdlib>
 #include <iostream>
+#include <mutex>
 #include <string>
 #include <thread>
 
@@ -25,8 +27,18 @@
 Api g_api;
 std::thread g_thread;
 std::string g_error;
-double g_load_s = 0, g_device_s = 0;
+double g_load_s = 0, g_device_s = 0, g_reserve_s = 0;
 bool g_started = false;
+std::thread g_reserve_thread;
+std::mutex g_stage_m;
+std::condition_variable g_stage_cv;
+int g_stage = 0;
+
+void set_stage(int st)
+{
+    { std::lock_guard<std::mutex> l(g_stage_m); g_stage = st; }
+    g_stage_cv.notify_all();
+}
 
 double now_s() { return std::chrono::duration<double>(std::chrono::steady_clock::now().time_since_epoch()).count(); }
 
@@ -41,7 +53,15 @@
     return dir + "/" + TGSF_LIB_REL;
 }
 
+void bind_and_warm(std::vector<int> devices);
+
 void load(std::vector<int> devices)
+{
+    bind_and_warm(std::move(devices));
+    if (!g_error.empty()) set_stage(-1);
+}
+
+void bind_and_warm(std::vector<int> devices)
 {
     CpuScope cpu(CPU_LOADER);
     const double t0 = now_s();
@@ -56,6 +76,9 @@
     BIND(prepare_device, "tgsf_prepare_device")
     BIND(create, "tgsf_create")
     BIND(destroy, "tgsf_destroy")
+    BIND(reserve, "tgsf_reserve")
+    BIND(release_reserved, "tgsf_release_reserved")
+    BIND(alloc_stats, "tgsf_alloc_stats")
     BIND(submit, "tgsf_submit")
     BIND(wait, "tgsf_wait")
     BIND(counters_len, "tgsf_counters_len")
@@ -80,6 +103,7 @@
         }
     }
     g_load_s = now_s() - t0;
+    set_stage(1);
     std::vector<std::thread> up;
     for (size_t i = 1; i < devices.size(); i++) {
         bool seen = false;
@@ -101,12 +125,41 @@
 const Api& lib()
 {
     if (!g_started) lib_start({});
-    if (g_thread.joinable()) g_thread.join();
-    if (!g_error.empty()) {
+    int st;
+    {
+        std::unique_lock<std::mutex> l(g_stage_m);
+        g_stage_cv.wait(l, [] { return g_stage != 0; });
+        st = g_stage;
+    }
+    if (st < 0) {
         std::cerr << "Error: " << g_error << std::endl;
         quit(255);
     }
     return g_api;
+}
+
+const Api& lib_warm()
+{
+    const Api& a = lib();
+    if (g_thread.joinable()) g_thread.join();
+    if (g_reserve_thread.joinable()) g_reserve_thread.join();
+    return a;
+}
+
+void lib_reserve_start(std::function<void(const Api&)> job)
+{
+    if (!g_started) lib_start({});
+    g_reserve_thread = std::thread([job = std::move(job)] {
+        CpuScope cpu(CPU_LOADER);
+        {
+            std::unique_lock<std::mutex> l(g_stage_m);
+            g_stage_cv.wait(l, [] { return g_stage != 0; });
+            if (g_stage < 0) return;
+        }
+        const double t0 = now_s();
+        job(g_api);
+        g_reserve_s = now_s() - t0;
+    });
 }
 
 namespace {
@@ -148,5 +201,6 @@
 }
 
 void lib_times(double& load_s, double& device_s) { load_s = g_load_s; device_s = g_device_s; }
-
-}
+double lib_reserve_s() { return g_reserve_s; }
+
+}
diff --git a/tgsfilter_amd/host/api.h b/tgsfilter_amd/host/api.h
--- a/tgsfilter_amd/host/api.h
+++ b/tgsfilter_amd/host/api.h
@@ -1,4 +1,5 @@
 #pragma once
+#include <functional>
 #include <vector>
 
 #include "tgsf.h"
@@ -12,6 +13,9 @@
     decltype(&tgsf_prepare_device) prepare_device;
     decltype(&tgsf_create) create;
     decltype(&tgsf_destroy) destroy;
+    decltype(&tgsf_reserve) reserve;
+    decltype(&tgsf_release_reserved) release_reserved;
+    decltype(&tgsf_alloc_stats) alloc_stats;
     decltype(&tgsf_submit) submit;
     decltype(&tgsf_wait) wait;
     decltype(&tgsf_counters_len) counters_len;
@@ -39,6 +43,9 @@
 
 void lib_start(const std::vector<int>& devices);
 const Api& lib();
+const Api& lib_warm();
+void lib_reserve_start(std::function<void(const Api&)> job);
 void lib_times(double& load_s, double& device_s);
+double lib_reserve_s();
 
 }
diff --git a/tgsfilter_amd/host/prepass.cpp b/tgsfilter_amd/host/prepass.cpp
--- a/tgsfilter_amd/host/prepass.cpp
+++ b/tgsfilter_amd/host/prepass.cpp
@@ -86,9 +86,9 @@
 }
 
 static double pp_now() { return std::chrono::duration<double>(std::chrono::steady_clock::now().time_since_epoch()).count(); }
-static double g_pp_create = 0, g_pp_align = 0; static int g_pp_calls = 0;
-
-static void adapter_search(const Options& o, const std::vector<std::string>& ends, std::string& adapter, float& depth)
+struct SearchTimes { double lib_wait = 0, create = 0, align = 0; int calls = 0; };
+
+static void adapter_search(const Options& o, const std::vector<std::string>& ends, std::string& adapter, float& depth, SearchTimes& T)
 {
     adapter.clear(); depth = 0.f;
     float min_sim = o.mid_sim;
@@ -114,10 +114,12 @@
     p.max_batch_reads = (uint32_t)(per_call * 22 / (22 * 2) + 64);
     p.max_batch_bases = 1 << 20; p.max_read_len = 1 << 16;
     tgsf_ctx* ctx = nullptr;
+    const double w0 = pp_now();
+    const Api& L = lib();
     const double c0 = pp_now();
-    if (lib().create(&p, o.devices.empty() ? o.device : o.devices[0], &ctx) != TGSF_OK) { std::cerr << "Error: " << lib().last_error(nullptr) << std::endl; quit(255); }
-
-    g_pp_create += pp_now() - c0;
+    T.lib_wait += c0 - w0;
+    if (L.create(&p, o.devices.empty() ? o.device : o.devices[0], &ctx) != TGSF_OK) { std::cerr << "Error: " << L.last_error(nullptr) << std::endl; quit(255); }
+    T.create += pp_now() - c0;
     std::unordered_map<int, int> maps;
     std::vector<uint8_t> buf; std::vector<uint64_t> off; std::vector<uint32_t> len; std::vector<uint8_t> aid;
     std::vector<int32_t> kk, res, eds;
@@ -134,15 +136,15 @@
         if (!n) continue;
         res.assign((size_t)n * 4, 0); eds.assign((size_t)n * 2, 0);
         const double a0 = pp_now();
-        if (lib().align_windows(ctx, buf.data(), buf.size(), off.data(), len.data(), aid.data(), kk.data(), n, res.data(), eds.data()) != TGSF_OK) {
-            std::cerr << "Error: " << lib().last_error(ctx) << std::endl; quit(255);
-        }
-        g_pp_align += pp_now() - a0; g_pp_calls++;
+        if (L.align_windows(ctx, buf.data(), buf.size(), off.data(), len.data(), aid.data(), kk.data(), n, res.data(), eds.data()) != TGSF_OK) {
+            std::cerr << "Error: " << L.last_error(ctx) << std::endl; quit(255);
+        }
+        T.align += pp_now() - a0; T.calls++;
         for (uint32_t i = 0; i < n; i++)
             if (res[(size_t)i * 4 + 1] > 0)
                 maps[(int)aid[i]] += res[(size_t)i * 4 + 2] - res[(size_t)i * 4 + 0];
     }
-    lib().destroy(ctx);
+    L.destroy(ctx);
     std::vector<std::pair<int, int>> vec(maps.begin(), maps.end());
     std::sort(vec.begin(), vec.end(), [](const std::pair<int, int>& a, const std::pair<int, int>& b) { return a.second > b.second; });
     if (vec.empty()) return;
@@ -199,6 +201,7 @@
     }
     const double t1 = pp_now();
     double t_bc = 0;
+    SearchTimes T5, T3;
     if (o.filter) {
         {
             std::thread t3;
@@ -209,13 +212,15 @@
         if (o.head_trim < 0 && o.tail_trim < 0 && R.trim5p > o.bc_len) R.trim5p = o.bc_len;
         t_bc = pp_now() - t1;
         if (o.adapter_file.empty()) {
-            adapter_search(o, ends5, R.adapter5p, R.depth5p);
-            adapter_search(o, ends3, R.adapter3p, R.depth3p);
+            std::thread t3([&] { adapter_search(o, ends3, R.adapter3p, R.depth3p, T3); });
+            adapter_search(o, ends5, R.adapter5p, R.depth5p, T5);
+            t3.join();
         }
     }
     if (getenv("TGSF_TIMING"))
-        fprintf(stderr, "PREPASS: %d reads looked at in %.3f s | base content %.3f | adapter search %.3f (contexts %.3f, %d alignment calls %.3f)\n",
-                seq_num, t_read, t_bc, pp_now() - t1 - t_bc, g_pp_create, g_pp_calls, g_pp_align);
+        fprintf(stderr, "PREPASS: %d reads looked at in %.3f s | base content %.3f | adapter search %.3f (contexts %.3f, %d alignment calls %.3f) | "
+                        "the two ends side by side: waited for the library %.3f, contexts and alignment calls summed over both\n",
+                seq_num, t_read, t_bc, pp_now() - t1 - t_bc, T5.create + T3.create, T5.calls + T3.calls, T5.align + T3.align, T5.lib_wait + T3.lib_wait);
     return R;
 }
 
diff --git a/tgsfilter_amd/host/run.h b/tgsfilter_amd/host/run.h
--- a/tgsfilter_amd/host/run.h
+++ b/tgsfilter_amd/host/run.h
@@ -60,6 +60,15 @@
 
     uint64_t batch_text = 0;
     uint32_t batch_reads = 1u << 16;
+    uint64_t batch_text_bytes() const;
+    uint32_t batch_reads_for(const std::vector<std::string>& ads) const;
+    int contexts_per_device() const;
+    void fill_params(tgsf_params& q, const std::vector<std::string>& ads, uint32_t max_read_len) const;
+    void reserve_contexts();
+    std::vector<std::string> upper_adapters;
+    tgsf_params upper;
+    std::atomic<size_t> n_created{0};
+    std::atomic<uint64_t> create_ns{0};
     const Api* api = nullptr;
     double t_load = 0, t_dev = 0, t_libwait = 0;
     const RcclApi* R = nullptr;
diff --git a/tgsfilter_amd/host/run_contexts.cpp b/tgsfilter_amd/host/run_contexts.cpp
--- a/tgsfilter_amd/host/run_contexts.cpp
+++ b/tgsfilter_amd/host/run_contexts.cpp
@@ -82,25 +82,86 @@
     }
 }
 
+uint64_t Run::batch_text_bytes() const
+{
+    uint64_t bt = streaming ? std::min<uint64_t>(256ull << 20, chunk_bytes)
+                            : std::min<uint64_t>(256ull << 20, std::max<uint64_t>(text_size / 8 + 4096, 1 << 16));
+    if (const char* e = knob("TGSF_BATCH_BYTES")) { const long long v = atoll(e); if (v > 0) bt = (uint64_t)v; }
+    return bt;
+}
+
+uint32_t Run::batch_reads_for(const std::vector<std::string>& ads) const
+{
+    uint32_t br = 1u << 16;
+    uint64_t per_read = 0, cols = 0, words = 1;
+    for (const std::string& a : ads) {
+        const int Q = (int)a.size();
+        const int kmax = std::max(0, std::min(Q - 1, std::max(Q - o.end_match_len + 1, Q - o.mid_match_len + 1)));
+        cols = std::max<uint64_t>(cols, (uint64_t)(Q + kmax + 2));
+        words = std::max<uint64_t>(words, Q > 256 ? (uint64_t)(Q + 63) / 64 : Q > 128 ? 4 : Q > 64 ? 2 : 1);
+    }
+    per_read = cols * 2 * words * 8;
+    if (words > 4) per_read = std::min<uint64_t>(per_read, (1ull << 20) + 16 * words) + 32 * words + 512;
+    per_read *= 3 * std::max<size_t>(ads.size(), 1);
+    if (per_read) br = (uint32_t)std::min<uint64_t>(br, std::max<uint64_t>(256, (4ull << 30) / per_read));
+    return br;
+}
+
+int Run::contexts_per_device() const
+{
+    int per_dev = (streaming || text_size > (64u << 20)) ? 3 : 1;
+    if (const char* e = getenv("TGSF_CTX_PER_DEVICE")) { const int v = atoi(e); if (v >= 1 && v <= 8) per_dev = v; }
+    return per_dev;
+}
+
+void Run::fill_params(tgsf_params& q, const std::vector<std::string>& ads, uint32_t max_read_len) const
+{
+    memset(&q, 0, sizeof q);
+    q.struct_size = sizeof q;
+    q.min_len = o.min_len; q.max_len = o.max_len; q.min_q = o.min_q < 0 ? 0.f : o.min_q; q.max_q = o.max_q;
+    q.bc_len = o.bc_len; q.head_trim = o.head_trim < 0 ? 0 : o.head_trim; q.tail_trim = o.tail_trim < 0 ? 0 : o.tail_trim;
+    q.end_len = o.end_len; q.end_match_len = o.end_match_len; q.mid_match_len = o.mid_match_len; q.extra_len = o.extra_len;
+    q.end_sim = o.end_sim; q.mid_sim = o.mid_sim; q.discard = o.discard; q.filter = o.filter; q.only_qc = o.only_qc;
+    q.min_repeat = o.min_repeat; q.kmer = o.kmer; q.qtype = pp.qtype ? pp.qtype : 33;
+    q.no_qual = fasta_in ? 1 : 0;
+    q.n_adapters = (int)ads.size();
+    for (size_t a = 0; a < ads.size(); a++) { q.adapters[a] = ads[a].data(); q.adapter_len[a] = (int)ads[a].size(); }
+    q.max_batch_reads = batch_reads_for(ads);
+    q.max_read_len = max_read_len;
+    q.max_batch_bases = std::max<uint64_t>(batch_text_bytes(), 2ull * q.max_read_len + (1u << 16)) + (1 << 20);
+}
+
+void Run::reserve_contexts()
+{
+    if (!(o.filter || o.only_qc) || o.only_adapters) return;
+    if (const char* e = knob("TGSF_RESERVE")) if (atoi(e) == 0) return;
+    if (o.filter && !o.adapter_file.empty()) {
+        InputBytes af;
+        if (af.open(o.adapter_file)) {
+            FastxReader rd(af.data(), af.size(), file_type(o.adapter_file) == 1);
+            Record r;
+            auto add = [&](const std::string& a) { if (std::find(upper_adapters.begin(), upper_adapters.end(), a) == upper_adapters.end()) upper_adapters.push_back(a); };
+            while (rd.next(r)) { add(std::string(r.seq)); add(rev_comp(std::string(r.seq))); }
+        }
+    } else if (o.filter) {
+        size_t longest = 0;
+        for (size_t a = 1; a < sizeof kAdapterLib / sizeof kAdapterLib[0]; a++) if (strlen(kAdapterLib[a]) > strlen(kAdapterLib[longest])) longest = a;
+        upper_adapters.assign(4, kAdapterLib[longest]);
+    }
+    if (upper_adapters.size() > TGSF_MAX_ADAPTERS) return;
+    for (const std::string& a : upper_adapters) if (a.empty() || a.size() > TGSF_MAX_ADAPTER_LEN) return;
+    const uint32_t max_read_len = streaming ? 1u << 26 : (uint32_t)std::min<uint64_t>(std::max<uint64_t>(in.size() / 2, 1024), 1u << 26);
+    fill_params(upper, upper_adapters, max_read_len);
+    const int per_dev = contexts_per_device();
+    lib_reserve_start([this, per_dev](const Api& L) {
+        for (int d : o.devices) (void)L.reserve(&upper, d, per_dev);
+    });
+}
+
 void Run::make_contexts()
 {
-    batch_text = streaming ? std::min<uint64_t>(256ull << 20, chunk_bytes)
-                                    : std::min<uint64_t>(256ull << 20, std::max<uint64_t>(text_size / 8 + 4096, 1 << 16));
-    if (const char* e = knob("TGSF_BATCH_BYTES")) { const long long v = atoll(e); if (v > 0) batch_text = (uint64_t)v; }
-    batch_reads = 1u << 16;
-    {
-        uint64_t per_read = 0, cols = 0, words = 1;
-        for (const std::string& a : adapters) {
-            const int Q = (int)a.size();
-            const int kmax = std::max(0, std::min(Q - 1, std::max(Q - o.end_match_len + 1, Q - o.mid_match_len + 1)));
-            cols = std::max<uint64_t>(cols, (uint64_t)(Q + kmax + 2));
-            words = std::max<uint64_t>(words, Q > 256 ? (uint64_t)(Q + 63) / 64 : Q > 128 ? 4 : Q > 64 ? 2 : 1);
-        }
-        per_read = cols * 2 * words * 8;
-        if (words > 4) per_read = std::min<uint64_t>(per_read, (1ull << 20) + 16 * words) + 32 * words + 512;
-        per_read *= 3 * std::max<size_t>(adapters.size(), 1);
-        if (per_read) batch_reads = (uint32_t)std::min<uint64_t>(batch_reads, std::max<uint64_t>(256, (4ull << 30) / per_read));
-    }
+    batch_text = batch_text_bytes();
+    batch_reads = batch_reads_for(adapters);
     fastq_out = o.out_type == 1;
     run_filter_pass = o.filter || o.only_qc;
     {
@@ -113,7 +174,7 @@
         oo.out_file = out_path;
         if (!o.only_qc && !sink.is_open() && !out.open(oo)) leave(1);
     }
-    api = &lib();
+    api = &lib_warm();
     const Api& L = *api;
     lib_times(t_load, t_dev);
     t_libwait = now_s() - t_start - t_prepass;
@@ -158,28 +219,17 @@
                 up->done.store(1, std::memory_order_release);
             });
     }
-    memset(&p, 0, sizeof p);
-    p.struct_size = sizeof p;
-    p.min_len = o.min_len; p.max_len = o.max_len; p.min_q = o.min_q < 0 ? 0.f : o.min_q; p.max_q = o.max_q;
-    p.bc_len = o.bc_len; p.head_trim = o.head_trim < 0 ? 0 : o.head_trim; p.tail_trim = o.tail_trim < 0 ? 0 : o.tail_trim;
-    p.end_len = o.end_len; p.end_match_len = o.end_match_len; p.mid_match_len = o.mid_match_len; p.extra_len = o.extra_len;
-    p.end_sim = o.end_sim; p.mid_sim = o.mid_sim; p.discard = o.discard; p.filter = o.filter; p.only_qc = o.only_qc;
-    p.min_repeat = o.min_repeat; p.kmer = o.kmer; p.qtype = pp.qtype ? pp.qtype : 33;
-    p.no_qual = fasta_in ? 1 : 0;
     if (adapters.size() > TGSF_MAX_ADAPTERS) die("more than " + std::to_string(TGSF_MAX_ADAPTERS) + " adapter sequences");
-    p.n_adapters = (int)adapters.size();
-    for (size_t a = 0; a < adapters.size(); a++) { p.adapters[a] = adapters[a].data(); p.adapter_len[a] = (int)adapters[a].size(); }
-    p.max_batch_reads = batch_reads;
-    if (streaming) p.max_read_len = 1u << 26;
+    uint32_t max_read_len;
+    if (streaming) max_read_len = 1u << 26;
     else if (sharded) {
-        if (in.size() <= (1ull << 30)) { records_p->wait_complete(); p.max_read_len = (uint32_t)std::max<uint64_t>(link.max_u64(records_p->longest()), 1024); }
-        else p.max_read_len = (uint32_t)std::min<uint64_t>(std::max<uint64_t>(in.size() / 2, 1024), 1u << 26);
-    }
-    else if (records_p->complete()) p.max_read_len = std::max<uint32_t>(records_p->longest(), 1024);
-    else p.max_read_len = (uint32_t)std::min<uint64_t>(std::max<uint64_t>(in.size() / 2, 1024), 1u << 26);
-    p.max_batch_bases = std::max<uint64_t>(batch_text, 2ull * p.max_read_len + (1u << 16)) + (1 << 20);
-    int per_dev = (streaming || text_size > (64u << 20)) ? 3 : 1;
-    if (const char* e = getenv("TGSF_CTX_PER_DEVICE")) { const int v = atoi(e); if (v >= 1 && v <= 8) per_dev = v; }
+        if (in.size() <= (1ull << 30)) { records_p->wait_complete(); max_read_len = (uint32_t)std::max<uint64_t>(link.max_u64(records_p->longest()), 1024); }
+        else max_read_len = (uint32_t)std::min<uint64_t>(std::max<uint64_t>(in.size() / 2, 1024), 1u << 26);
+    }
+    else if (records_p->complete()) max_read_len = std::max<uint32_t>(records_p->longest(), 1024);
+    else max_read_len = (uint32_t)std::min<uint64_t>(std::max<uint64_t>(in.size() / 2, 1024), 1u << 26);
+    fill_params(p, adapters, max_read_len);
+    const int per_dev = contexts_per_device();
     for (int d : o.devices) for (int k = 0; k < per_dev; k++) ctx_dev.push_back(d);
     ctxs.assign(ctx_dev.size(), nullptr);
     t_p0 = now_s();
diff --git a/tgsfilter_amd/host/run_pipeline.cpp b/tgsfilter_amd/host/run_pipeline.cpp
--- a/tgsfilter_amd/host/run_pipeline.cpp
+++ b/tgsfilter_amd/host/run_pipeline.cpp
@@ -119,7 +119,12 @@
     CpuScope cpu(CPU_FEEDER);
     const Api& L = *api;
     if (numa_bind) bind_to_node_of(k);
-    if (L.create(&p, ctx_dev[k], &ctxs[k]) != TGSF_OK) die(L.last_error(nullptr));
+    {
+        const double c0 = now_s();
+        if (L.create(&p, ctx_dev[k], &ctxs[k]) != TGSF_OK) die(L.last_error(nullptr));
+        create_ns.fetch_add((uint64_t)((now_s() - c0) * 1e9));
+        if (n_created.fetch_add(1) + 1 == ctxs.size()) for (int d : o.devices) (void)L.release_reserved(d);
+    }
     tgsf_ctx* fctx = ctxs[k];
     if (timing) (void)L.profile(fctx, 1);
     for (;;) {
diff --git a/tgsfilter_amd/host/run_report.cpp b/tgsfilter_amd/host/run_report.cpp
--- a/tgsfilter_amd/host/run_report.cpp
+++ b/tgsfilter_amd/host/run_report.cpp
@@ -267,13 +267,17 @@
 {
     const Api& L = *api;
     if (timing) {
+        uint64_t astats[5] = {0, 0, 0, 0, 0};
+        (void)L.alloc_stats(astats);
         fprintf(stderr, "POOL: %zu jobs, busy %.3f, freeing job state %.3f, longest job %.3f, first job at %.3f, last job done at %.3f (pipeline start = 0, planner done at %.3f)\n",
                 pool->jobs_, t_busy, pool->destroy_, pool->longest_, pool->first_ - t_p0, pool->last_ - t_p0, t_f0 - t_p0);
         fprintf(stderr, "TIMING: total %.3f s | index+prepass %.3f | waiting for the library %.3f (load %.3f + device %.3f, beside the pre-pass) | "
                         "pipeline %.3f (batching %.3f, tgsf_submit summed over %zu feeders %.3f, plan+write %.3f, planner waiting %.3f, "
-                        "first batch filtered after %.3f, fill tail %.3f, closing the output %.3f; stages overlap) | stats+report %.3f | %s (fallocate %.3f, mapping the reserved pages %.3f, fill threads busy %.3f summed)\n",
+                        "first batch filtered after %.3f, fill tail %.3f, closing the output %.3f; stages overlap) | stats+report %.3f | %s (fallocate %.3f, mapping the reserved pages %.3f, fill threads busy %.3f summed) | "
+                        "contexts: %llu created (%llu from blocks reserved ahead), %llu device allocations made, tgsf_create in the feeder threads %.3f summed, reserving them ahead took %.3f beside the pre-pass\n",
                 now_s() - t_start, t_prepass, t_libwait, t_load, t_dev, t_pipe, t_parse, ctxs.size(), t_gpu, t_write, t_widle, t_first,
-                t_fill_tail, t_close, now_s() - t_p0 - t_pipe, mapped_out ? "output: fallocate + mapped fill" : "output: writev", sink.t_falloc, reserver->t_populate_wait, t_busy);
+                t_fill_tail, t_close, now_s() - t_p0 - t_pipe, mapped_out ? "output: fallocate + mapped fill" : "output: writev", sink.t_falloc, reserver->t_populate_wait, t_busy,
+                (unsigned long long)astats[2], (unsigned long long)astats[4], (unsigned long long)astats[0], (double)create_ns.load() * 1e-9, lib_reserve_s());
         fprintf(stderr, "RESERVE: planner waited %.3f s for pages of the output file\n", t_drain);
     }
     if (timing) {
diff --git a/tgsfilter_amd/host/run_setup.cpp b/tgsfilter_amd/host/run_setup.cpp
--- a/tgsfilter_amd/host/run_setup.cpp
+++ b/tgsfilter_amd/host/run_setup.cpp
@@ -97,6 +97,7 @@
     }
     text = in.data() + text_off;
     if (!streaming) records_p.reset(new RecordIndex(text, text_size, !fasta_in, scan_threads));
+    reserve_contexts();
 }
 
 void Run::open_output_early()
```
